# gregspangenberg/shoulder

Measured on AMD Instinct MI355X. Metric: humerus meshes/s end-to-end (all 4 landmarks), higher is better.
Workload: dtype f64 geometry + bf16 UNet

## Files before the change

shoulder_amd/csrc/k_groove.h:

```cpp
#pragma once
#include "k_stages.h"

namespace sh {

#define SH_GSLOTS (SH_GROOVE_NROWS * SH_MAXPEAK)

__global__ void k_groove_rows(const double* __restrict__ itr_cs , const double* __restrict__ prox_zs,
                              const double* __restrict__ canal_axis_ct, int row0,
                              double* __restrict__ xraw, double* __restrict__ ptheta, int* __restrict__ npk,
                              double* __restrict__ r0, int* __restrict__ err, int B) {
  __shared__ double s_bufA[SH_MPROX], s_bufB[SH_MPROX];
  double* const s_r = s_bufA; double* const s_filt = s_bufA;
  double* const s_neg = s_bufB; double* const s_roll = s_bufB;
  __shared__ int s_cand[SH_PEAK_CAP];
  __shared__ Peak s_pk[SH_PEAK_CAP];
  __shared__ int s_pass[SH_PEAK_CAP];
  __shared__ int s_ncand;
  const int M = SH_MPROX;
  const int gid = blockIdx.x, lane = threadIdx.x;
  const int b = gid / SH_GROOVE_NROWS, i = gid % SH_GROOVE_NROWS;
  const double* row = itr_cs + ((size_t)b * SH_NPROX + row0 + i) * 2 * M;
  const double* zs = prox_zs + (size_t)b * SH_NPROX + row0;
  for (int k = lane; k < M; k += 64) s_r[k] = row[M + k];
  if (lane == 0) s_ncand = 0;
  __syncthreads();
  double acc = 0.0;
  if (lane < 32) {
    const int leaf = lane >> 3, k = lane & 7;
    acc = s_r[128 * leaf + k];
    for (int q = 1; q < 16; ++q) acc += s_r[128 * leaf + 8 * q + k];
  }
  acc = acc + __shfl_down(acc, 1);
  acc = acc + __shfl_down(acc, 2);
  acc = acc + __shfl_down(acc, 4);
  acc = acc + __shfl_down(acc, 8);
  acc = acc + __shfl_down(acc, 16);
  const double mean = __shfl(acc, 0) / (double)M;
  for (int k = lane; k < M; k += 64) s_neg[k] = -1.0 * (s_r[k] - mean);
  __syncthreads();
  for (int k = 5 + lane; k < M - 5; k += 64) s_filt[k] = savgol10_1_at(s_neg, k);
  if (lane == 0) savgol10_1_edges(s_neg, M, s_filt);
  __syncthreads();
  double bv = 1e300;
  int bi = 0x7fffffff;
  for (int k = lane; k < M; k += 64) if (s_filt[k] < bv) { bv = s_filt[k]; bi = k; }
  for (int off = 32; off > 0; off >>= 1) {
    double ov = __shfl_down(bv, off);
    int oi = __shfl_down(bi, off);
    if (ov < bv || (ov == bv && oi < bi)) { bv = ov; bi = oi; }
  }
  const int amin = __shfl(bi, 0);
  double* r0row = r0 + (size_t)gid * M;
  for (int k = lane; k < M; k += 64) r0row[k] = -s_neg[k];
  __syncthreads();
  for (int k = lane; k < M; k += 64) { int src = k + amin; if (src >= M) src -= M; s_roll[k] = s_filt[src]; }
  __syncthreads();
  for (int k = 1 + lane; k < M - 1; k += 64)
    if (s_roll[k - 1] < s_roll[k]) {
      int resume;
      int pk = local_maximum_at(s_roll, M, k, &resume);
      if (pk >= 0) { int s = atomicAdd(&s_ncand, 1); if (s < SH_PEAK_CAP) s_cand[s] = pk; }
    }
  __syncthreads();
  int nc = s_ncand < SH_PEAK_CAP ? s_ncand : SH_PEAK_CAP;
  if (lane == 0)
    for (int a = 1; a < nc; ++a) { int v = s_cand[a]; int q = a - 1; while (q >= 0 && s_cand[q] > v) { s_cand[q + 1] = s_cand[q]; --q; } s_cand[q + 1] = v; }
  __syncthreads();
  static_assert(SH_MPROX == 512, "8 samples per lane");
  __shared__ int s_lb[SH_PEAK_CAP], s_rb[SH_PEAK_CAP];
  __shared__ double s_lmin[SH_PEAK_CAP], s_rmin[SH_PEAK_CAP];
  {
    double xr[8];
#pragma unroll
    for (int q = 0; q < 8; ++q) xr[q] = s_roll[8 * lane + q];
    for (int cnd = 0; cnd < nc; ++cnd) {
      const int pk = s_cand[cnd];
      const double v = s_roll[pk];
      int L = -1, R = M;
#pragma unroll
      for (int q = 0; q < 8; ++q) { const int k = 8 * lane + q; if (k < pk && xr[q] > v) L = k; }
#pragma unroll
      for (int q = 7; q >= 0; --q) { const int k = 8 * lane + q; if (k > pk && xr[q] > v) R = k; }
      for (int off = 32; off > 0; off >>= 1) { L = max(L, __shfl_xor(L, off)); R = min(R, __shfl_xor(R, off)); }
      double lm = v, rm = v;
#pragma unroll
      for (int q = 0; q < 8; ++q) {
        const int k = 8 * lane + q;
        if (k > L && k <= pk) lm = fmin(lm, xr[q]);
        if (k >= pk && k < R) rm = fmin(rm, xr[q]);
      }
      for (int off = 32; off > 0; off >>= 1) { lm = fmin(lm, __shfl_xor(lm, off)); rm = fmin(rm, __shfl_xor(rm, off)); }
      int lb = -1, rb = M;
#pragma unroll
      for (int q = 0; q < 8; ++q) { const int k = 8 * lane + q; if (k > L && k <= pk && xr[q] == lm) lb = k; }
#pragma unroll
      for (int q = 7; q >= 0; --q) { const int k = 8 * lane + q; if (k >= pk && k < R && xr[q] == rm) rb = k; }
      for (int off = 32; off > 0; off >>= 1) { lb = max(lb, __shfl_xor(lb, off)); rb = min(rb, __shfl_xor(rb, off)); }
      if (lane == 0) { s_lb[cnd] = lb; s_rb[cnd] = rb; s_lmin[cnd] = lm; s_rmin[cnd] = rm; }
    }
  }
  __syncthreads();
  if (lane < nc) {
    const double* x = s_roll;
    const int pk = s_cand[lane], lb = s_lb[lane], rb = s_rb[lane];
    const double left_min = s_lmin[lane], right_min = s_rmin[lane];
    bool ok = x[pk] >= -10.0;
    const double prom = x[pk] - (left_min > right_min ? left_min : right_min);
    ok = ok && prom >= 0.6;
    if (ok) {
      const double h = x[pk] - prom * 0.5;
      int k = pk;
      while (lb < k && h < x[k]) --k;
      double lip = (double)k;
      if (x[k] < h) lip += (h - x[k]) / (x[k + 1] - x[k]);
      k = pk;
      while (k < rb && h < x[k]) ++k;
      double rip = (double)k;
      if (x[k] < h) rip -= (h - x[k]) / (x[k - 1] - x[k]);
      const double w = rip - lip;
      ok = w >= 0.1;
      if (ok) { s_pk[lane].idx = pk; s_pk[lane].prominence = prom; s_pk[lane].width = w; s_pk[lane].width_height = h; }
    }
    s_pass[lane] = ok ? 1 : 0;
  }
  __syncthreads();
  __shared__ int s_np;
  __shared__ double s_th[SH_MAXPEAK], s_d[SH_MAXPEAK][SH_MAXPEAK];
  __shared__ int s_pidx[SH_MAXPEAK];
  if (lane == 0) {
    int np_ = 0;
    for (int a = 0; a < nc; ++a) if (s_pass[a]) s_pk[np_++] = s_pk[a];
    if (np_ > SH_MAXPEAK) {
      bool keep[SH_PEAK_CAP];
      for (int k = 0; k < np_; ++k) keep[k] = false;
      for (int q = 0; q < SH_MAXPEAK; ++q) {
        int bq = -1;
        for (int k = 0; k < np_; ++k)
          if (!keep[k] && (bq < 0 || s_pk[k].prominence > s_pk[bq].prominence)) bq = k;
        keep[bq] = true;
      }
      int w = 0;
      for (int k = 0; k < np_; ++k) if (keep[k]) s_pk[w++] = s_pk[k];
      np_ = SH_MAXPEAK;
    }
    s_np = np_;
  }
  __syncthreads();
  const int np_ = s_np;
  if (lane < np_) {
    const int idx = (s_pk[lane].idx + amin) % M;
    s_pidx[lane] = idx;
    s_th[lane] = row[idx];
  }
  double zmax = -1e300, zmin = 1e300;
  for (int k = lane; k < SH_GROOVE_NROWS; k += 64) { zmax = fmax(zmax, zs[k]); zmin = fmin(zmin, zs[k]); }
  for (int off = 32; off > 0; off >>= 1) { zmax = fmax(zmax, __shfl_xor(zmax, off)); zmin = fmin(zmin, __shfl_xor(zmin, off)); }
  __syncthreads();
  {
    const int k = lane >> 3, j = lane & 7;
    if (k < np_ && j < np_) s_d[k][j] = wrapped_abs_diff(s_th[k], s_th[j]);
  }
  __syncthreads();
  if (lane < np_) {
    const int k = lane;
    double near = 0.0, next = 0.0;
    if (np_ > 1) {
      double a[SH_MAXPEAK];
      int na = 0;
      for (int j = 0; j < np_; ++j) {
        double d = s_d[k][j];
        if (rint(d * 100.0) / 100.0 != 0.0) a[na++] = d;
      }
      for (int p = 1; p < na; ++p) { double v = a[p]; int q = p - 1; while (q >= 0 && a[q] > v) { a[q + 1] = a[q]; --q; } a[q + 1] = v; }
      near = na > 0 ? a[0] : nan("");
      if (np_ > 2) next = na > 1 ? a[1] : nan("");
    }
    double rng = zmax - zmin;
    if (rng == 0.0) rng = 1.0;
    const double sc = 1.0 / rng;
    const double z_scaled = zs[i] * sc + (0.0 - zmin * sc);
    const double* ax = canal_axis_ct + 6 * b;
    double cu[3] = {ax[0] - ax[3], ax[1] - ax[4], ax[2] - ax[5]};
    const double n = norm3(cu);
    cu[0] /= n; cu[1] /= n; cu[2] /= n;
    const double z = zs[i], th = s_th[k];
    const double rad = row[M + s_pidx[k]];
    const double px = rad * cos(th), py = rad * sin(th);
    const double dx = px - cu[0] * z, dy = py - cu[1] * z;
    double* X = xraw + ((size_t)b * SH_GSLOTS + (size_t)i * SH_MAXPEAK + k) * 9;
    X[0] = rad; X[1] = near; X[2] = next; X[3] = z_scaled; X[4] = s_pk[k].prominence; X[5] = s_pk[k].width;
    X[6] = s_pk[k].width_height; X[7] = sqrt(dx * dx + dy * dy); X[8] = (double)np_ / 7.0;
    ptheta[(size_t)b * SH_GSLOTS + (size_t)i * SH_MAXPEAK + k] = th;
    for (int q = 0; q < 9; ++q) if (X[q] != X[q]) atomicCAS(&err[b], 0, SH_ERR_GEOMETRY_DEV);
  }
  if (lane == 0) npk[gid] = np_;
  (void)B;
}

__global__ void __launch_bounds__(256)
k_groove_scale(const double* __restrict__ xraw, const int* __restrict__ npk, double* __restrict__ stats, int B,
               int* __restrict__ slots_out , int* __restrict__ nslot_out ,
               float* __restrict__ proba ) {
  __shared__ double col[5][SH_GSLOTS];
  __shared__ int slot[SH_GSLOTS];
  __shared__ int P_s;
  const int b = blockIdx.x, tid = threadIdx.x;
  const double* X = xraw + (size_t)b * SH_GSLOTS * 9;
  const int* np_ = npk + (size_t)b * SH_GROOVE_NROWS;
  __shared__ int s_cnt[SH_GROOVE_NROWS];
  for (int i = tid; i < SH_GROOVE_NROWS; i += 256) s_cnt[i] = np_[i];
  __syncthreads();
  for (int i = tid; i < SH_GROOVE_NROWS; i += 256) {
    int off = 0;
    for (int j = 0; j < i; ++j) off += s_cnt[j];
    const int n = s_cnt[i];
    for (int k = 0; k < n; ++k) slot[off + k] = i * SH_MAXPEAK + k;
    if (i == SH_GROOVE_NROWS - 1) P_s = off + n;
  }
  __syncthreads();
  const int P = P_s;
  for (int p = tid; p < P; p += 256) slots_out[(size_t)b * SH_GSLOTS + p] = slot[p];
  if (tid == 0) nslot_out[b] = P;
  for (int s = tid; s < SH_GSLOTS; s += 256)
    if (s % SH_MAXPEAK >= s_cnt[s / SH_MAXPEAK]) proba[(size_t)b * SH_GSLOTS + s] = -1.0f;
  for (int f0 = 0; f0 < 9; f0 += 5) {
    const int nf = f0 + 5 <= 9 ? 5 : 9 - f0;
    for (int q = tid; q < P * nf; q += 256) { const int p = q / nf, f = q - p * nf; col[f][p] = X[(size_t)slot[p] * 9 + f0 + f]; }
    __syncthreads();
    if (tid < nf) {
      const double* c = col[tid];
      double s = 0.0;
      int p = 0;
      for (; p + 8 <= P; p += 8) {
        double t8[8];
#pragma unroll
        for (int u = 0; u < 8; ++u) t8[u] = c[p + u];
#pragma unroll
        for (int u = 0; u < 8; ++u) s += t8[u];
      }
      for (; p < P; ++p) s += c[p];
      const double mean = P ? s / (double)P : 0.0;
      double v = 0.0;
      p = 0;
      for (; p + 8 <= P; p += 8) {
        double t8[8];
#pragma unroll
        for (int u = 0; u < 8; ++u) t8[u] = c[p + u];
#pragma unroll
        for (int u = 0; u < 8; ++u) { const double d = t8[u] - mean; v += d * d; }
      }
      for (; p < P; ++p) { double d = c[p] - mean; v += d * d; }
      const double var = P ? v / (double)P : 0.0;
      const double eps_ = 2.220446049250313e-16, nn = (double)P;
      const double ub = nn * eps_ * var + (nn * mean * eps_) * (nn * mean * eps_);
      double scale = var <= ub ? 1.0 : sqrt(var);
      stats[(size_t)b * 18 + f0 + tid] = mean;
      stats[(size_t)b * 18 + 9 + f0 + tid] = scale;
    }
    __syncthreads();
  }
}

__global__ void k_rfc_pack(const int* __restrict__ feat, const float* __restrict__ thr, const int* __restrict__ ti, const int* __restrict__ fi,
                           const float* __restrict__ lw, int4* __restrict__ nodes, int N) {
  const int i = blockIdx.x * blockDim.x + threadIdx.x;
  if (i >= N) return;
  const bool leaf = ti[i] < 0;
  nodes[i] = make_int4(feat[i], __float_as_int(leaf ? lw[i] : thr[i]), ti[i], fi[i]);
}

__global__ void __launch_bounds__(64)
k_groove_rfc(const double* __restrict__ xraw, const int* __restrict__ slots , const int* __restrict__ nslot , const double* __restrict__ stats,
             const int4* __restrict__ nodes, const int* __restrict__ roots, int n_trees,
             double* __restrict__ xs , float* __restrict__ proba, int B) {
  __shared__ double sx[9][64];
  const int tid = threadIdx.x;
  constexpr int WPB = (SH_GSLOTS + 63) / 64;
  const int b = blockIdx.x / WPB, p = (blockIdx.x - b * WPB) * 64 + tid;
  if (b >= B || p >= nslot[b]) return;
  const int gid = b * SH_GSLOTS + slots[(size_t)b * SH_GSLOTS + p];
  for (int f = 0; f < 9; ++f) {
    const double v = (xraw[(size_t)gid * 9 + f] - stats[(size_t)b * 18 + f]) / stats[(size_t)b * 18 + 9 + f];
    xs[(size_t)gid * 9 + f] = v;
    sx[f][tid] = v;
  }
  double acc = 0.0;
  for (int t = 0; t < n_trees; ++t) {
    int4 nd = nodes[roots[t]];
    while (nd.z >= 0) nd = nodes[(sx[nd.x][tid] <= (double)__int_as_float(nd.y)) ? nd.z : nd.w];
    acc += (double)__int_as_float(nd.y);
  }
  proba[gid] = (float)acc;
}

#define SH_KDE_TIE 1e-9
__device__ inline double groove_kde_wg(const double* __restrict__ ptheta, const float* __restrict__ proba, double* __restrict__ bg_theta,
                                       int* __restrict__ err, int b) {
  __shared__ double sel[SH_GSLOTS];
  __shared__ double dens[1024];
  __shared__ int nsel;
  __shared__ double wv[4];
  __shared__ int wi[4];
  __shared__ double s_bg;
  int tid = threadIdx.x;
  __shared__ int s_wc[4];
  if (tid == 0) nsel = 0;
  __syncthreads();
  for (int s0 = 0; s0 < SH_GSLOTS; s0 += 256) {
    const int s = s0 + tid;
    const bool keep = s < SH_GSLOTS && proba[(size_t)b * SH_GSLOTS + s] > 0.4f;
    const double val = keep ? ptheta[(size_t)b * SH_GSLOTS + s] : 0.0;
    const unsigned long long m = __ballot(keep);
    if ((tid & 63) == 0) s_wc[tid >> 6] = __popcll(m);
    __syncthreads();
    int pos = nsel + __popcll(m & ((1ull << (tid & 63)) - 1ull));
    for (int w = 0; w < (tid >> 6); ++w) pos += s_wc[w];
    if (keep) sel[pos] = val;
    __syncthreads();
    if (tid == 0) nsel += s_wc[0] + s_wc[1] + s_wc[2] + s_wc[3];
    __syncthreads();
  }
  const int n = nsel;
  if (n == 0) { if (tid == 0) { atomicCAS(&err[b], 0, SH_ERR_GEOMETRY_DEV); bg_theta[b] = 0.0; } return 0.0; }
  double best = -1.0;
  for (int j = tid; j < 1024; j += blockDim.x) {
    double t = linspace_at(-1.0 * M_PI, M_PI, 1024, j);
    double acc = 0.0;
    for (int i = 0; i < n; ++i) {
      double d = 1.0 - fabs(t - sel[i]);
      if (d > 0.0) acc += d;
    }
    dens[j] = acc;
    best = fmax(best, acc);
  }
  for (int off = 32; off > 0; off >>= 1) best = fmax(best, __shfl_down(best, off));
  if ((tid & 63) == 0) wv[tid >> 6] = best;
  __syncthreads();
  best = wv[0];
  for (int w = 1; w < (int)(blockDim.x >> 6); ++w) best = fmax(best, wv[w]);
  const double thr = best * (1.0 - SH_KDE_TIE);
  int bi = 0x7fffffff;
  for (int j = tid; j < 1024; j += blockDim.x)
    if (dens[j] >= thr) bi = min(bi, j);
  for (int off = 32; off > 0; off >>= 1) bi = min(bi, __shfl_down(bi, off));
  if ((tid & 63) == 0) wi[tid >> 6] = bi;
  __syncthreads();
  if (tid == 0) {
    for (int w = 1; w < (int)(blockDim.x >> 6); ++w) bi = min(bi, wi[w]);
    s_bg = linspace_at(-1.0 * M_PI, M_PI, 1024, bi);
    bg_theta[b] = s_bg;
  }
  __syncthreads();
  return s_bg;
}

__device__ inline void groove_localmin_row(const double* __restrict__ itr_cs, const double* __restrict__ r0, const double* __restrict__ prox_zs,
                                           const double* __restrict__ prox_centroids, double bg, int row0, double deg_window,
                                           int* __restrict__ local_idx, double* pts_obb, int b, int i) {
  const int gid = b * SH_GROOVE_NROWS + i;
  const double* row = itr_cs + ((size_t)b * SH_NPROX + row0 + i) * 2 * SH_MPROX;
  int ivar = (int)rint(deg_window / (360.0 / (double)SH_MPROX));
  if (ivar < 1) ivar = 1;
  int loc = groove_local_min(row, r0 + (size_t)gid * SH_MPROX, SH_MPROX, bg, ivar);
  local_idx[gid] = loc;
  int k = loc < 0 ? loc + SH_MPROX : loc;
  k = k < 0 ? 0 : (k >= SH_MPROX ? SH_MPROX - 1 : k);
  double t = row[k], r = row[SH_MPROX + k];
  const double* c = prox_centroids + 2 * ((size_t)b * SH_NPROX + row0 + i);
  double* p = pts_obb + (size_t)gid * 3;
  p[0] = r * cos(t) + c[0];
  p[1] = r * sin(t) + c[1];
  p[2] = prox_zs[(size_t)b * SH_NPROX + row0 + i] + 0.0;
}

__device__ inline void groove_axis_wave(const double* pts_obb, const double* __restrict__ T_obb, double* __restrict__ axis_ct,
                                        double* __restrict__ pts_ct, int b) {
  int lane = threadIdx.x & 63;
  const double* P = pts_obb + (size_t)b * SH_GROOVE_NROWS * 3;
  double mean[3], d[3];
  wave_line_fit(P, SH_GROOVE_NROWS, 3, mean, d);
  double zmin = 1e300, zmax = -1e300;
  for (int i = lane; i < SH_GROOVE_NROWS; i += 64) { zmin = fmin(zmin, P[3 * i + 2]); zmax = fmax(zmax, P[3 * i + 2]); }
  for (int off = 32; off > 0; off >>= 1) { zmin = fmin(zmin, __shfl_down(zmin, off)); zmax = fmax(zmax, __shfl_down(zmax, off)); }
  zmin = __shfl(zmin, 0); zmax = __shfl(zmax, 0);
  double Ti[16];
  inv_transform(T_obb + 16 * b, Ti);
  for (int i = lane; i < SH_GROOVE_NROWS; i += 64) xform_pt(Ti, P[3 * i], P[3 * i + 1], P[3 * i + 2], pts_ct + ((size_t)b * SH_GROOVE_NROWS + i) * 3);
  if (lane == 0) {
    if (d[2] < 0) { d[0] = -d[0]; d[1] = -d[1]; d[2] = -d[2]; }
    double h = (zmax - zmin) / 2.0;
    xform_pt(Ti, mean[0] + d[0] * h, mean[1] + d[1] * h, mean[2] + d[2] * h, axis_ct + 6 * b);
    xform_pt(Ti, mean[0] - d[0] * h, mean[1] - d[1] * h, mean[2] - d[2] * h, axis_ct + 6 * b + 3);
  }
}

__global__ void __launch_bounds__(256)
k_groove_tail(const double* __restrict__ ptheta, const float* __restrict__ proba, double* __restrict__ bg_theta, int* __restrict__ err,
              const double* __restrict__ itr_cs, const double* __restrict__ r0, const double* __restrict__ prox_zs, const double* __restrict__ prox_centroids,
              int row0, double deg_window, int* __restrict__ local_idx, double* pts_obb, const double* __restrict__ T_obb,
              double* __restrict__ axis_ct, double* __restrict__ pts_ct) {
  const int b = blockIdx.x, tid = threadIdx.x;
  const double bg = groove_kde_wg(ptheta, proba, bg_theta, err, b);
  for (int i = tid; i < SH_GROOVE_NROWS; i += 256) groove_localmin_row(itr_cs, r0, prox_zs, prox_centroids, bg, row0, deg_window, local_idx, pts_obb, b, i);
  __syncthreads();
  if (tid < 64) groove_axis_wave(pts_obb, T_obb, axis_ct, pts_ct, b);
}

}
```

shoulder_amd/csrc/k_ovf.h:

```cpp
#pragma once
#include "k_slices.h"

namespace sh {

struct OvfPools {
  Seg* segs; double* ring; unsigned char* work;
  unsigned long long seg_cap, ring_cap, work_cap;
  unsigned long long* ctr;
  int open_mode;
};
__host__ __device__ inline int ovf_nodes(int cnt, int open_mode) { return open_mode ? 2 * cnt : cnt; }

struct OvfSet { long long* soff; long long* roff; long long* woff; int* fill; int* list; int* nlist ; int* list2; };

__host__ __device__ inline unsigned ovf_hash_size(int n) { unsigned h = 64; while (h < 2u * (unsigned)n) h <<= 1; return h; }
__host__ __device__ inline unsigned long long ovf_work_bytes(int n) {
  unsigned long long b = (unsigned long long)n * 8ull * 5ull + (unsigned long long)ovf_hash_size(n) * 4ull + (unsigned long long)n * 4ull * 6ull + 64ull;
  const unsigned long long te = (unsigned long long)(n + 1) * 8ull * 7ull + 64ull;
  if (te > b) b = te;
  return (b + 15ull) & ~15ull;
}

__global__ void k_ovf_plan(int N, int nplanes, const int* __restrict__ seg_count, OvfPools P, OvfSet S, int* __restrict__ err) {
  const int pl = blockIdx.x * blockDim.x + threadIdx.x;
  if (pl >= nplanes) return;
  const int cnt = seg_count[pl];
  S.soff[pl] = -1; S.roff[pl] = -1; S.woff[pl] = -1; S.fill[pl] = 0;
  if (cnt <= SH_MAXSEG) return;
  const int nn = ovf_nodes(cnt, P.open_mode);
  const unsigned long long wb = ovf_work_bytes(nn);
  const unsigned long long s = atomicAdd(&P.ctr[0], (unsigned long long)cnt);
  const unsigned long long r = atomicAdd(&P.ctr[1], (unsigned long long)nn + 1ull);
  const unsigned long long w = atomicAdd(&P.ctr[2], wb);
  atomicMax(&P.ctr[3], s + cnt); atomicMax(&P.ctr[4], r + nn + 1ull); atomicMax(&P.ctr[5], w + wb);
  if (s + cnt > P.seg_cap || r + nn + 1ull > P.ring_cap || w + wb > P.work_cap) { atomicExch(&err[pl / N], SH_ERR_CAPACITY_DEV); return; }
  S.soff[pl] = (long long)s; S.roff[pl] = (long long)r; S.woff[pl] = (long long)w;
  S.list[atomicAdd(S.nlist, 1)] = pl;
}

__global__ void __launch_bounds__(256)
k_slice_emit_ovf(const double* __restrict__ vobb, const int* __restrict__ faces, const long long* __restrict__ voff, const long long* __restrict__ foff,
                 const double* __restrict__ zeff, int N, OvfPools P, OvfSet S) {
  if (*S.nlist == 0) return;
  const int b = blockIdx.y;
  const long long f0 = foff[b], nf = foff[b + 1] - f0;
  const double* vb = vobb + 3 * voff[b];
  const double* zp = zeff + (size_t)b * N;
  const double z_first = zp[0], z_last = zp[N - 1];
  const double inv_step = (double)(N - 1) / (z_last - z_first);
  for (long long fi = blockIdx.x * (long long)blockDim.x + threadIdx.x; fi < nf; fi += (long long)gridDim.x * blockDim.x) {
    const int* f = faces + 3 * (f0 + fi);
    const int id[3] = {f[0], f[1], f[2]};
    double Z[3];
    for (int k = 0; k < 3; ++k) Z[k] = vb[3 * (size_t)id[k] + 2];
    const double fzmin = fmin(Z[0], fmin(Z[1], Z[2])), fzmax = fmax(Z[0], fmax(Z[1], Z[2]));
    const double ka = (fzmin - z_first) * inv_step, kb = (fzmax - z_first) * inv_step;
    const double klo = fmin(ka, kb), khi = fmax(ka, kb);
    if (khi < -1.0 || klo > (double)N) continue;
    int lo = (int)floor(fmax(klo, 0.0)) - 1, hi = (int)ceil(fmin(khi, (double)(N - 1))) + 1;
    lo = lo < 0 ? 0 : lo;
    hi = hi > N - 1 ? N - 1 : hi;
    if (N == 1) { lo = 0; hi = 0; }
    for (int k = lo; k <= hi; ++k) {
      const long long so = S.soff[(size_t)b * N + k];
      if (so < 0) continue;
      const double z = zp[k];
      double d[3];
      int s[3];
      for (int j = 0; j < 3; ++j) { d[j] = Z[j] - z; s[j] = d[j] < -SH_SECTION_TOL ? -1 : 1; }
      if (s[0] == s[1] && s[1] == s[2]) continue;
      const int slot = atomicAdd(&S.fill[(size_t)b * N + k], 1);
      int up = 0, dn = 0;
      for (int j = 0; j < 3; ++j) {
        const int jn = (j + 1) % 3;
        if (s[j] == -1 && s[jn] == 1) up = j;
        if (s[j] == 1 && s[jn] == -1) dn = j;
      }
      Seg sg;
      {
        const int a = dn, c = (dn + 1) % 3;
        const int l = id[a] < id[c] ? a : c, h = id[a] < id[c] ? c : a;
        sg.s_lo = (uint32_t)id[l]; sg.s_hi = (uint32_t)id[h];
      }
      {
        const int a = up, c = (up + 1) % 3;
        const int l = id[a] < id[c] ? a : c, h = id[a] < id[c] ? c : a;
        sg.e_lo = (uint32_t)id[l]; sg.e_hi = (uint32_t)id[h];
      }
      P.segs[so + slot] = sg;
    }
  }
}

__global__ void __launch_bounds__(256)
k_ovf_plan_loops(int N, const int* __restrict__ seg_count, const Seg* __restrict__ segs , OvfPools P, OvfSet S, int* __restrict__ err) {
  __shared__ long long so, ro, wo;
  const int n2 = S.nlist[1];
  for (int i = blockIdx.x; i < n2; i += gridDim.x) {
    const int pl = S.list2[i];
    const int cnt = seg_count[pl];
    if (threadIdx.x == 0) {
      const int nn = ovf_nodes(cnt, P.open_mode);
      const unsigned long long wb = ovf_work_bytes(nn);
      const unsigned long long s = atomicAdd(&P.ctr[0], (unsigned long long)cnt);
      const unsigned long long r = atomicAdd(&P.ctr[1], (unsigned long long)nn + 1ull);
      const unsigned long long w = atomicAdd(&P.ctr[2], wb);
      atomicMax(&P.ctr[3], s + cnt); atomicMax(&P.ctr[4], r + nn + 1ull); atomicMax(&P.ctr[5], w + wb);
      if (s + cnt > P.seg_cap || r + nn + 1ull > P.ring_cap || w + wb > P.work_cap) { atomicExch(&err[pl / N], SH_ERR_CAPACITY_DEV); so = -1; }
      else { so = (long long)s; ro = (long long)r; wo = (long long)w; }
    }
    __syncthreads();
    if (so >= 0) {
      const Seg* src = segs + (size_t)pl * SH_MAXSEG;
      for (int j = threadIdx.x; j < cnt; j += 256) P.segs[so + j] = src[j];
      if (threadIdx.x == 0) { S.soff[pl] = so; S.roff[pl] = ro; S.woff[pl] = wo; S.fill[pl] = cnt; S.list[atomicAdd(&S.nlist[0], 1)] = pl; }
    }
    __syncthreads();
  }
}

#define SH_HUGE_THREADS 1024
#define SH_MAXLOOPS_G 1024

template <bool OPEN>
__device__ inline void slice_link_plane_g(const int pl, int N, const int* __restrict__ seg_count, const Seg* __restrict__ sp, const double* __restrict__ vb ,
             const double zpl , unsigned char* __restrict__ wk,
             double* __restrict__ centroids, double* __restrict__ areas, int* __restrict__ nloops, int* __restrict__ ring_n, double* __restrict__ ring_out ,
             int select, int* __restrict__ err, double* __restrict__ areas_total, const OpenCfg oc) {
  constexpr int T = SH_HUGE_THREADS;
  __shared__ unsigned long long l_key[SH_MAXLOOPS_G];
  __shared__ int l_start[SH_MAXLOOPS_G], l_len[SH_MAXLOOPS_G], l_off[SH_MAXLOOPS_G];
  __shared__ double l_area[SH_MAXLOOPS_G], l_sel[SH_MAXLOOPS_G];
  __shared__ int n_loops, bad, octl[4];
  __shared__ double bbw[T / 64][4];
  const int b = pl / N, tid = threadIdx.x;
  const int n = seg_count[pl];
  const int cap = ovf_nodes(n, OPEN ? oc.mode : 0);
  const unsigned HASH = ovf_hash_size(cap);
  unsigned long long* skey = (unsigned long long*)wk;
  unsigned long long* bufA = skey + cap;
  unsigned long long* bufB = bufA + cap;
  double* rx = (double*)(bufB + cap);
  double* ry = rx + cap;
  int* table = (int*)(ry + cap);
  int* nxt = table + HASH;
  int* jmpA = nxt + cap; int* jmpB = jmpA + cap; int* offA = jmpB + cap; int* offB = offA + cap; int* posv = offB + cap;
  if (tid == 0) { n_loops = 0; bad = 0; }
  for (unsigned i = tid; i < HASH; i += T) table[i] = -1;
  for (int i = tid; i < n; i += T) {
    const Seg s = sp[i];
    skey[i] = ((unsigned long long)s.s_lo << 32) | s.s_hi;
    bufA[i] = ((unsigned long long)s.e_lo << 32) | s.e_hi;
  }
  __syncthreads();
  for (int i = tid; i < n; i += T) {
    uint32_t h = hash_key64(skey[i]) & (HASH - 1);
    while (atomicCAS(&table[h], -1, i) != -1) h = (h + 1) & (HASH - 1);
  }
  __syncthreads();
  for (int i = tid; i < n; i += T) {
    const unsigned long long k = bufA[i];
    uint32_t h = hash_key64(k) & (HASH - 1);
    int t, found = -1;
    while ((t = table[h]) != -1) {
      if (skey[t] == k) { found = t; break; }
      h = (h + 1) & (HASH - 1);
    }
    if (found < 0) { found = i; bad = 1; }
    nxt[i] = found;
  }
  __syncthreads();
  const bool bridging = OPEN && (bad || n < 3);
  int n2 = n;
  if (bridging) {
    n2 = bridge_open_chains<T>(n, cap, n, skey, bufA, nxt, offB, octl, jmpA, jmpB, offA, posv, table, table + cap, rx, ry,
                               (double*)bufB, (double*)bufB + n, vb, zpl, oc.max_gap);
    if (tid == 0) bad = 0;
  }
  unsigned long long* labA = bufA;
  unsigned long long* labB = bufB;
  int* ja = jmpA; int* jb = jmpB;
  int* ra = offA; int* rb = offB;
  for (int i = tid; i < n2; i += T) { labA[i] = skey[i]; ja[i] = nxt[i]; ra[i] = 0; }
  __syncthreads();
  for (int span = 1; span < n2; span <<= 1) {
    for (int i = tid; i < n2; i += T) {
      const int j = ja[i];
      const unsigned long long a = labA[i], c = labA[j];
      const bool own = a <= c;
      labB[i] = own ? a : c;
      rb[i] = own ? ra[i] : span + ra[j];
      jb[i] = ja[j];
    }
    __syncthreads();
    unsigned long long* tl = labA; labA = labB; labB = tl;
    int* tj = ja; ja = jb; jb = tj;
    int* tr = ra; ra = rb; rb = tr;
  }
  for (int i = tid; i < n2; i += T)
    if (ra[i] == 0 && (!bridging || (nxt[ja[i]] != ja[i] && ra[nxt[i]] >= 2))) {
      const int l = atomicAdd(&n_loops, 1);
      if (l < SH_MAXLOOPS_G) l_start[l] = i;
    }
  __syncthreads();
  const int nl = n_loops > SH_MAXLOOPS_G ? SH_MAXLOOPS_G : n_loops;
  if (tid == 0) {
    if (n_loops > SH_MAXLOOPS_G) atomicExch(&err[b], SH_ERR_CAPACITY_DEV);
    for (int a = 1; a < nl; ++a) {
      const int v = l_start[a]; int c = a - 1;
      while (c >= 0 && skey[l_start[c]] > skey[v]) { l_start[c + 1] = l_start[c]; --c; }
      l_start[c + 1] = v;
    }
    int off = 0;
    for (int l = 0; l < nl; ++l) {
      const int s = l_start[l];
      const int L = ra[nxt[s]] + 1;
      l_len[l] = L; l_off[l] = off; off += L;
      l_key[l] = skey[s];
    }
    if (off != n && !bridging) bad = 1;
  }
  __syncthreads();
  if (bridging && oc.stats)
    for (int i = tid; i < n; i += T)
      if (nxt[i] == i || nxt[i] >= n) {
        bool kept = false;
        for (int q = 0; q < nl; ++q) kept |= l_key[q] == labA[i];
        atomicAdd(&oc.stats[2 * b + (kept ? 0 : 1)], 1);
      }
  for (int i = tid; i < n2; i += T) {
    const unsigned long long key = labA[i];
    int l = -1;
    for (int q = 0; q < nl; ++q) if (l_key[q] == key) { l = q; break; }
    const int L = l >= 0 ? l_len[l] : 1;
    const int r = ra[i];
    const int pos = r == 0 ? 0 : L - r;
    posv[i] = l < 0 ? -1 : l_off[l] + pos;
  }
  __syncthreads();
  for (int i = tid; i < n2; i += T)
    if (posv[i] >= 0 && posv[i] < n2) {
      if (!OPEN || i < n) { const Seg sg = sp[i]; seg_start_point(vb, sg.s_lo, sg.s_hi, zpl, &rx[posv[i]], &ry[posv[i]]); }
      else { const unsigned long long kv = skey[i]; seg_start_point(vb, (uint32_t)(kv >> 32), (uint32_t)kv, zpl, &rx[posv[i]], &ry[posv[i]]); }
    }
  __syncthreads();
  const int lane = tid & 63, wave = tid >> 6;
  {
    const int nv = bridging ? (nl > 0 ? l_off[nl - 1] + l_len[nl - 1] : 0) : n;
    double x0 = 1e300, x1 = -1e300, y0 = 1e300, y1 = -1e300;
    for (int i = tid; i < nv; i += T) {
      const double qx = rx[i], qy = ry[i];
      x0 = fmin(x0, qx); x1 = fmax(x1, qx); y0 = fmin(y0, qy); y1 = fmax(y1, qy);
    }
    for (int off = 32; off > 0; off >>= 1) {
      x0 = fmin(x0, __shfl_down(x0, off)); x1 = fmax(x1, __shfl_down(x1, off));
      y0 = fmin(y0, __shfl_down(y0, off)); y1 = fmax(y1, __shfl_down(y1, off));
    }
    if (lane == 0) { bbw[wave][0] = x0; bbw[wave][1] = x1; bbw[wave][2] = y0; bbw[wave][3] = y1; }
  }
  for (int l = wave; l < nl; l += T / 64) {
    const int o = l_off[l], L = l_len[l];
    double a2 = 0.0, mx = 0.0, my = 0.0;
    for (int q = lane; q < L; q += 64) {
      const int qn = q + 1 == L ? 0 : q + 1;
      a2 += rx[o + q] * ry[o + qn] - rx[o + qn] * ry[o + q];
      mx += rx[o + q]; my += ry[o + q];
    }
    for (int off = 32; off > 0; off >>= 1) { a2 += __shfl_down(a2, off); mx += __shfl_down(mx, off); my += __shfl_down(my, off); }
    if (lane == 0) {
      l_area[l] = 0.5 * a2;
      mx = (mx + rx[o]) / (double)(L + 1); my = (my + ry[o]) / (double)(L + 1);
      l_sel[l] = fabs(mx) + fabs(my);
    }
  }
  __syncthreads();
  int best = 0;
  for (int l = 1; l < nl; ++l) {
    if (select == 0) { if (fabs(l_area[l]) > fabs(l_area[best])) best = l; }
    else { if (l_sel[l] < l_sel[best]) best = l; }
  }
  if (tid == 0) {
    double x0 = bbw[0][0], x1 = bbw[0][1], y0 = bbw[0][2], y1 = bbw[0][3];
    for (int w = 1; w < T / 64; ++w) { x0 = fmin(x0, bbw[w][0]); x1 = fmax(x1, bbw[w][1]); y0 = fmin(y0, bbw[w][2]); y1 = fmax(y1, bbw[w][3]); }
    centroids[2 * (size_t)pl] = 0.5 * (x0 + x1);
    centroids[2 * (size_t)pl + 1] = 0.5 * (y0 + y1);
    int amax = 0;
    for (int l = 1; l < nl; ++l) if (fabs(l_area[l]) > fabs(l_area[amax])) amax = l;
    areas[pl] = nl > 0 ? fabs(l_area[amax]) : 0.0;
    if (areas_total) {
      double tot = 0.0;
      for (int l = 0; l < nl; ++l) tot += l_area[l];
      areas_total[pl] = fabs(tot);
    }
    nloops[pl] = nl;
    ring_n[pl] = nl > 0 ? l_len[best] : 0;
    if (bad || (nl == 0 && !(bridging && areas_total))) atomicCAS(&err[b], 0, SH_ERR_GEOMETRY_DEV);
  }
  if (ring_out && nl > 0) {
    const int l = best, o = l_off[l], L = l_len[l];
    const bool rev = l_area[l] < 0;
    for (int q = tid; q <= L; q += T) {
      const int qq = q == L ? 0 : q;
      const int src = rev ? (qq == 0 ? 0 : L - qq) : qq;
      ring_out[2 * q] = rx[o + src];
      ring_out[2 * q + 1] = ry[o + src];
    }
  }
  __syncthreads();
}

template <bool OPEN>
__global__ void __launch_bounds__(SH_HUGE_THREADS)
k_slice_link_huge(int N, const int* __restrict__ seg_count, OvfPools P, OvfSet S, double* __restrict__ centroids, double* __restrict__ areas,
                  int* __restrict__ nloops, int* __restrict__ ring_n, int want_ring, int select, int* __restrict__ err, double* __restrict__ areas_total,
                  const double* __restrict__ vobb, const long long* __restrict__ voff, const double* __restrict__ zeff, const OpenCfg oc) {
  const int nl = *S.nlist;
  for (int i = blockIdx.x; i < nl; i += gridDim.x) {
    const int pl = S.list[i];
    slice_link_plane_g<OPEN>(pl, N, seg_count, P.segs + S.soff[pl], vobb + 3 * voff[pl / N], zeff[pl], P.work + S.woff[pl], centroids, areas, nloops, ring_n,
                       want_ring ? P.ring + 2 * S.roff[pl] : (double*)nullptr, select, err, areas_total, oc);
  }
}

__global__ void __launch_bounds__(SH_RS_THREADS)
k_resample_polar_huge(int N, int M, const int* __restrict__ ring_n, OvfPools P, OvfSet S, const double* __restrict__ centroids,
                      double* __restrict__ ixy, double* __restrict__ itr_start, double* __restrict__ itr_cs, const RsWant W) {
  constexpr int NS = SH_MPROX / SH_RS_THREADS;
  __shared__ int amin_idx;
  __shared__ double wmin[SH_RS_THREADS / 64];
  __shared__ int widx[SH_RS_THREADS / 64];
  const int nlist = *S.nlist, tid = threadIdx.x;
  for (int it = blockIdx.x; it < nlist; it += gridDim.x) {
    const int pl = S.list[it];
    const int kpl = pl % N;
    const bool want_st = W.keep_all || kpl >= W.st_lo, want_cs = W.keep_all || (kpl >= W.cs_lo && kpl < W.cs_hi);
    if (!want_st && !want_cs) continue;
    const int L = ring_n[pl];
    const double* rp = P.ring + 2 * S.roff[pl];
    double* d = (double*)(P.work + S.woff[pl]);
    for (int q = 1 + tid; q <= L; q += SH_RS_THREADS) {
      const double dx = rp[2 * q] - rp[2 * (q - 1)], dy = rp[2 * q + 1] - rp[2 * (q - 1) + 1];
      d[q] = sqrt(dx * dx + dy * dy);
    }
    __syncthreads();
    if (tid == 0) {
      double acc = 0.0;
      d[0] = 0.0;
      for (int q = 1; q <= L; ++q) { acc += d[q]; d[q] = acc; }
    }
    __syncthreads();
    const double dmax = d[L];
    double sx[NS], sy[NS];
#pragma unroll
    for (int u = 0; u < NS; ++u) {
      const int j = tid + u * SH_RS_THREADS;
      const double t = linspace_at(0.0, dmax, M, j);
      const int n = L + 1;
      if (t < d[0]) { sx[u] = rp[0]; sy[u] = rp[1]; }
      else if (!(t < d[n - 1])) { sx[u] = rp[2 * (n - 1)]; sy[u] = rp[2 * (n - 1) + 1]; }
      else {
        int lo = 0, hi = n - 1;
        while (hi - lo > 1) { const int mid = (lo + hi) >> 1; if (t >= d[mid]) lo = mid; else hi = mid; }
        const double x0 = d[lo], fx = rp[2 * lo], fy = rp[2 * lo + 1];
        if (x0 == t) { sx[u] = fx; sy[u] = fy; }
        else {
          const double den = d[lo + 1] - x0;
          sx[u] = (rp[2 * (lo + 1)] - fx) / den * (t - x0) + fx;
          sy[u] = (rp[2 * (lo + 1) + 1] - fy) / den * (t - x0) + fy;
        }
      }
    }
    if (W.keep_all) {
      double* oxy = ixy + (size_t)pl * 2 * M;
#pragma unroll
      for (int u = 0; u < NS; ++u) { const int j = tid + u * SH_RS_THREADS; oxy[j] = sx[u]; oxy[M + j] = sy[u]; }
    }
    const double cx = centroids[2 * (size_t)pl], cy = centroids[2 * (size_t)pl + 1];
    for (int pass = 0; pass < 2; ++pass) {
      if (pass == 0 ? !want_st : !want_cs) continue;
      const double ox = pass ? cx : 0.0, oy = pass ? cy : 0.0;
      double best = 1e300;
      int bi = 0x7fffffff;
      double th[NS], rr[NS];
#pragma unroll
      for (int u = 0; u < NS; ++u) {
        const int j = tid + u * SH_RS_THREADS;
        const double x = sx[u] - ox, y = sy[u] - oy;
        th[u] = atan2(y, x);
        rr[u] = sqrt(x * x + y * y);
        if (th[u] < best || (th[u] == best && j < bi)) { best = th[u]; bi = j; }
      }
      for (int off = 32; off > 0; off >>= 1) {
        const double ob = __shfl_down(best, off);
        const int oi = __shfl_down(bi, off);
        if (ob < best || (ob == best && oi < bi)) { best = ob; bi = oi; }
      }
      if ((tid & 63) == 0) { wmin[tid >> 6] = best; widx[tid >> 6] = bi; }
      __syncthreads();
      if (tid == 0) {
        double bv = wmin[0]; int bx = widx[0];
        for (int w = 1; w < SH_RS_THREADS / 64; ++w)
          if (wmin[w] < bv || (wmin[w] == bv && widx[w] < bx)) { bv = wmin[w]; bx = widx[w]; }
        amin_idx = bx;
      }
      __syncthreads();
      const int k0 = amin_idx;
      double* o = (pass ? itr_cs : itr_start) + (size_t)pl * 2 * M;
#pragma unroll
      for (int u = 0; u < NS; ++u) {
        int dst = tid + u * SH_RS_THREADS - k0; if (dst < 0) dst += M;
        o[dst] = th[u];
        o[M + dst] = rr[u];
      }
      __syncthreads();
    }
  }
}

}
```

shoulder_amd/csrc/k_slices.h:

```cpp
#pragma once
#include "sh_scalar.h"

namespace sh {

struct __attribute__((aligned(16))) Seg {
  uint32_t s_lo, s_hi, e_lo, e_hi;
};
static_assert(sizeof(Seg) == 16, "Seg must be 16 bytes");
__device__ inline void seg_start_point(const double* __restrict__ vb , uint32_t lo, uint32_t hi, double z, double* x, double* y) {
  const double* pl = vb + 3 * (size_t)lo;
  const double* ph = vb + 3 * (size_t)hi;
  const double dl = pl[2] - z, dh = ph[2] - z;
  const double t = dl / (dl - dh);
  *x = pl[0] + t * (ph[0] - pl[0]);
  *y = pl[1] + t * (ph[1] - pl[1]);
}

__device__ inline unsigned long long enc_f64(double v) {
  unsigned long long b = (unsigned long long)__double_as_longlong(v);
  return (b & 0x8000000000000000ull) ? ~b : (b | 0x8000000000000000ull);
}
__device__ inline double dec_f64(unsigned long long e) {
  unsigned long long b = (e & 0x8000000000000000ull) ? (e & 0x7FFFFFFFFFFFFFFFull) : ~e;
  return __longlong_as_double((long long)b);
}

__global__ void k_transform_verts(const float* __restrict__ verts, const long long* __restrict__ voff,
                                  const double* __restrict__ T, double* __restrict__ vobb,
                                  unsigned long long* __restrict__ zb_enc ) {
  int b = blockIdx.y;
  long long v0 = voff[b], nv = voff[b + 1] - v0;
  const double* Tb = T + 16 * b;
  double zmin = 1e300, zmax = -1e300;
  for (long long i = blockIdx.x * (long long)blockDim.x + threadIdx.x; i < nv; i += (long long)gridDim.x * blockDim.x) {
    const float* p = verts + 3 * (v0 + i);
    double o[3];
    xform_pt(Tb, (double)p[0], (double)p[1], (double)p[2], o);
    double* q = vobb + 3 * (v0 + i);
    q[0] = o[0]; q[1] = o[1]; q[2] = o[2];
    zmin = fmin(zmin, o[2]); zmax = fmax(zmax, o[2]);
  }
  for (int off = 32; off > 0; off >>= 1) {
    zmin = fmin(zmin, __shfl_down(zmin, off));
    zmax = fmax(zmax, __shfl_down(zmax, off));
  }
  if ((threadIdx.x & 63) == 0) {
    atomicMin(&zb_enc[2 * b], enc_f64(zmin));
    atomicMin(&zb_enc[2 * b + 1], ~enc_f64(zmax));
  }
}

__global__ void k_decode_bounds(const unsigned long long* zb_enc, double* zb, int B) {
  int i = blockIdx.x * blockDim.x + threadIdx.x;
  if (i < 2 * B) zb[i] = dec_f64((i & 1) ? ~zb_enc[i] : zb_enc[i]);
}

__device__ inline double np_pairwise_sum(const double* a, int n) {
  if (n < 8) {
    double r = 0.0;
    for (int i = 0; i < n; ++i) r += a[i];
    return r;
  } else if (n <= 128) {
    double r[8];
    for (int k = 0; k < 8; ++k) r[k] = a[k];
    int i;
    for (i = 8; i < n - (n % 8); i += 8)
      for (int k = 0; k < 8; ++k) r[k] += a[i + k];
    double res = ((r[0] + r[1]) + (r[2] + r[3])) + ((r[4] + r[5]) + (r[6] + r[7]));
    for (; i < n; ++i) res += a[i];
    return res;
  } else {
    int n2 = n / 2;
    n2 -= n2 % 8;
    return np_pairwise_sum(a, n2) + np_pairwise_sum(a + n2, n - n2);
  }
}

struct PlaneAux {
  const unsigned long long* zb_enc; double* zb_out;
  int* seg_count; int* nlarge;
  int* ovf_nlist; unsigned long long* ovf_ctr;
};
struct ManyLoops { int* list; int* n; unsigned long long* missed; };
struct SliceSetDev {
  int N, kind, select;
  const double* zb;
  double* zs; double* zeff;
  int* seg_count; Seg* segs;
  double* centroids; double* areas; int* nloops; int* ring_n; double* ring ; double* areas_total ;
  int* nlarge; ManyLoops many; unsigned long long* ovf_missed;
  PlaneAux aux;
};
struct OpenCfg { int mode; double max_gap; int* stats; };

struct SliceSets { SliceSetDev s[2]; int n; const double* vobb; const long long* voff; OpenCfg open; };

__global__ void k_make_planes(SliceSets sets, const double* __restrict__ neck_z, int B) {
  const SliceSetDev& S = sets.s[blockIdx.y];
  const int kind = S.kind, N = S.N;
  const double* zb = S.zb;
  double* zs = S.zs; double* zeff = S.zeff;
  const PlaneAux A = S.aux;
  int b = blockIdx.x;
  if (b >= B) return;
  for (int k = threadIdx.x; k < N; k += blockDim.x) A.seg_count[(size_t)b * N + k] = 0;
  if (b == 0 && threadIdx.x == 0) {
    *A.nlarge = 0;
    if (A.ovf_nlist) { A.ovf_nlist[0] = 0; A.ovf_nlist[1] = 0 ; if (A.ovf_ctr) { A.ovf_ctr[0] = 0ull; A.ovf_ctr[2] = 0ull; } }
  }
  if (kind == 3) {
    if (threadIdx.x == 0) { zs[b] = neck_z[b]; zeff[b] = neck_z[b]; }
    return;
  }
  double zmin, zmax;
  if (A.zb_enc) {
    zmin = dec_f64(A.zb_enc[2 * b]); zmax = dec_f64(~A.zb_enc[2 * b + 1]);
    if (threadIdx.x == 0) { A.zb_out[2 * b] = zmin; A.zb_out[2 * b + 1] = zmax; }
  } else { zmin = zb[2 * b]; zmax = zb[2 * b + 1]; }
  double a, e;
  if (kind == 4) {
    for (int k = threadIdx.x; k < N; k += blockDim.x) { double z = linspace_at(zmin * 0.99, zmax * 0.99, N, k); zs[(size_t)b * N + k] = z; zeff[(size_t)b * N + k] = z; }
    return;
  }
  if (kind == 0) { a = 0.99 * zmax; e = 0.99 * zmin; }
  else if (kind == 1) { a = 0.99 * zmax; e = neck_z[b]; }
  else { a = 0.99 * zmin; e = 0.0; }
  double* z = zs + (size_t)b * N;
  for (int k = threadIdx.x; k < N; k += blockDim.x) z[k] = linspace_at(a, e, N, k);
  __syncthreads();
  __shared__ double z_orig;
  if (threadIdx.x == 0) z_orig = np_pairwise_sum(z, N) / (double)N;
  __syncthreads();
  for (int k = threadIdx.x; k < N; k += blockDim.x) zeff[(size_t)b * N + k] = z_orig + (z[k] - z_orig);
}

#define SH_EMIT_MAXN 640
__global__ void __launch_bounds__(256)
k_slice_emit(const double* __restrict__ vobb, const int* __restrict__ faces,
             const long long* __restrict__ voff, const long long* __restrict__ foff, SliceSets sets) {
  __shared__ int hist[SH_EMIT_MAXN];
  int b = blockIdx.y;
  long long f0 = foff[b], nf = foff[b + 1] - f0;
  const double* vb = vobb + 3 * voff[b];
  const int nsets = sets.n, Ntot = sets.s[0].N + (nsets > 1 ? sets.s[1].N : 0);
  for (long long f_base = blockIdx.x * (long long)blockDim.x; f_base < nf; f_base += (long long)gridDim.x * blockDim.x) {
    for (int k = threadIdx.x; k < Ntot; k += blockDim.x) hist[k] = 0;
    const long long fi = f_base + threadIdx.x;
    const bool live = fi < nf;
    const int* f = faces + 3 * (f0 + (live ? fi : 0));
    int id[3] = {f[0], f[1], f[2]};
    double Z[3];
    for (int k = 0; k < 3; ++k) Z[k] = vb[3 * (size_t)id[k] + 2];
    double fzmin = fmin(Z[0], fmin(Z[1], Z[2])), fzmax = fmax(Z[0], fmax(Z[1], Z[2]));
    int lo_[2] = {1, 1}, hi_[2] = {0, 0};
    for (int si = 0; si < nsets; ++si) {
      const int N = sets.s[si].N;
      const double* zp = sets.s[si].zeff + (size_t)b * N;
      const double z_first = zp[0], z_last = zp[N - 1];
      const double inv_step = (double)(N - 1) / (z_last - z_first);
      double ka = (fzmin - z_first) * inv_step, kb = (fzmax - z_first) * inv_step;
      double klo = fmin(ka, kb), khi = fmax(ka, kb);
      int lo = 1, hi = 0;
      if (live && !(khi < -1.0 || klo > (double)N)) {
        lo = (int)floor(fmax(klo, 0.0)) - 1; hi = (int)ceil(fmin(khi, (double)(N - 1))) + 1;
        lo = lo < 0 ? 0 : lo;
        hi = hi > N - 1 ? N - 1 : hi;
      }
      if (live && N == 1) { lo = 0; hi = 0; }
      lo_[si] = lo; hi_[si] = hi;
    }
    __syncthreads();
    for (int si = 0; si < nsets; ++si) {
      const int N = sets.s[si].N, hoff = si ? sets.s[0].N : 0;
      const double* zp = sets.s[si].zeff + (size_t)b * N;
      for (int k = lo_[si]; k <= hi_[si]; ++k) {
        const double z = zp[k];
        const int s0 = Z[0] - z < -SH_SECTION_TOL ? -1 : 1, s1 = Z[1] - z < -SH_SECTION_TOL ? -1 : 1, s2 = Z[2] - z < -SH_SECTION_TOL ? -1 : 1;
        if (!(s0 == s1 && s1 == s2)) atomicAdd(&hist[hoff + k], 1);
      }
    }
    __syncthreads();
    for (int k = threadIdx.x; k < Ntot; k += blockDim.x) {
      const int n = hist[k];
      if (n > 0) {
        const int si = k >= sets.s[0].N ? 1 : 0, kk = si ? k - sets.s[0].N : k;
        hist[k] = atomicAdd(&sets.s[si].seg_count[(size_t)b * sets.s[si].N + kk], n);
      }
    }
    __syncthreads();
    for (int si = 0; si < nsets; ++si) {
      const int N = sets.s[si].N, hoff = si ? sets.s[0].N : 0;
      const double* zp = sets.s[si].zeff + (size_t)b * N;
      Seg* segs = sets.s[si].segs;
      for (int k = lo_[si]; k <= hi_[si]; ++k) {
        const double z = zp[k];
        double d[3];
        int s[3];
        for (int j = 0; j < 3; ++j) { d[j] = Z[j] - z; s[j] = d[j] < -SH_SECTION_TOL ? -1 : 1; }
        if (s[0] == s[1] && s[1] == s[2]) continue;
        const int slot = atomicAdd(&hist[hoff + k], 1);
        int up = 0, dn = 0;
        for (int j = 0; j < 3; ++j) {
          int jn = (j + 1) % 3;
          if (s[j] == -1 && s[jn] == 1) up = j;
          if (s[j] == 1 && s[jn] == -1) dn = j;
        }
        Seg sg;
        {
          int a = dn, c = (dn + 1) % 3;
          int l = id[a] < id[c] ? a : c, h = id[a] < id[c] ? c : a;
          sg.s_lo = (uint32_t)id[l]; sg.s_hi = (uint32_t)id[h];
        }
        {
          int a = up, c = (up + 1) % 3;
          int l = id[a] < id[c] ? a : c, h = id[a] < id[c] ? c : a;
          sg.e_lo = (uint32_t)id[l]; sg.e_hi = (uint32_t)id[h];
        }
        if (slot < SH_MAXSEG) segs[((size_t)b * N + k) * SH_MAXSEG + slot] = sg;
      }
    }
    __syncthreads();
  }
}

#define SH_LINK_THREADS 256
#define SH_MAXLOOPS 32
#define SH_SMALLSEG 384

__device__ inline uint32_t hash_key64(unsigned long long k) {
  k ^= k >> 33; k *= 0xff51afd7ed558ccdull; k ^= k >> 33;
  return (uint32_t)k;
}

template <int T>
__device__ inline int bridge_open_chains(const int n, const int cap, const int maxe, unsigned long long* __restrict__ skey,
                                         const unsigned long long* __restrict__ ekey, int* __restrict__ nxt, int* __restrict__ pred,
                                         int* __restrict__ ctl, int* tl, int* hd, int* bt, int* bh, int* mt, int* mh,
                                         double* tx, double* ty, double* hx, double* hy,
                                         const double* __restrict__ vb, const double z, const double max_gap) {
  const int tid = threadIdx.x;
  for (int i = tid; i < n; i += T) pred[i] = 0;
  if (tid < 4) ctl[tid] = 0;
  __syncthreads();
  for (int i = tid; i < n; i += T) if (nxt[i] != i) atomicAdd(&pred[nxt[i]], 1);
  __syncthreads();
  for (int i = tid; i < n; i += T) {
    if (nxt[i] == i) { const int q = atomicAdd(&ctl[0], 1); if (q < maxe) tl[q] = i; }
    if (pred[i] == 0) { const int q = atomicAdd(&ctl[1], 1); if (q < maxe) hd[q] = i; }
  }
  __syncthreads();
  const int nt = ctl[0], nh = ctl[1];
  if (nt > maxe || nh > maxe) return -1;
  for (int q = tid; q < nt; q += T) { const unsigned long long k = ekey[tl[q]]; seg_start_point(vb, (uint32_t)(k >> 32), (uint32_t)k, z, &tx[q], &ty[q]); mt[q] = -1; }
  for (int q = tid; q < nh; q += T) { const unsigned long long k = skey[hd[q]]; seg_start_point(vb, (uint32_t)(k >> 32), (uint32_t)k, z, &hx[q], &hy[q]); mh[q] = -1; }
  for (;;) {
    __syncthreads();
    if (tid == 0) ctl[2] = 0;
    for (int q = tid; q < nt; q += T) {
      int best = -1; double bd = 0.0; unsigned long long bk = 0;
      if (mt[q] < 0)
        for (int h = 0; h < nh; ++h) {
          if (mh[h] >= 0) continue;
          const double dx = tx[q] - hx[h], dy = ty[q] - hy[h];
          const double d = sqrt(dx * dx + dy * dy);
          if (!(d <= max_gap)) continue;
          const unsigned long long k = skey[hd[h]];
          if (best < 0 || d < bd || (d == bd && k < bk)) { best = h; bd = d; bk = k; }
        }
      bt[q] = best;
    }
    for (int q = tid; q < nh; q += T) {
      int best = -1; double bd = 0.0; unsigned long long bk = 0;
      if (mh[q] < 0)
        for (int t = 0; t < nt; ++t) {
          if (mt[t] >= 0) continue;
          const double dx = tx[t] - hx[q], dy = ty[t] - hy[q];
          const double d = sqrt(dx * dx + dy * dy);
          if (!(d <= max_gap)) continue;
          const unsigned long long k = ekey[tl[t]];
          if (best < 0 || d < bd || (d == bd && k < bk)) { best = t; bd = d; bk = k; }
        }
      bh[q] = best;
    }
    __syncthreads();
    for (int q = tid; q < nt; q += T) {
      const int h = bt[q];
      if (h >= 0 && bh[h] == q) { mt[q] = h; mh[h] = q; ctl[2] = 1; }
    }
    __syncthreads();
    if (ctl[2] == 0) break;
  }
  for (int q = tid; q < nt; q += T)
    if (mt[q] >= 0) {
      const int v = n + atomicAdd(&ctl[3], 1);
      if (v < cap) { skey[v] = ekey[tl[q]]; nxt[v] = hd[mt[q]]; nxt[tl[q]] = v; }
    }
  __syncthreads();
  const int nb = ctl[3];
  return n + nb > cap ? -1 : n + nb;
}


template <int CAP, bool OPEN>
__device__ inline void slice_link_plane(const int pl, int N, const int* __restrict__ seg_count, const Seg* __restrict__ segs,
             const double* __restrict__ vobb, const long long* __restrict__ voff, const double* __restrict__ zeff,
             double* __restrict__ centroids, double* __restrict__ areas, int* __restrict__ nloops,
             int* __restrict__ ring_n, double* __restrict__ ring , int select, int* __restrict__ err,
             double* __restrict__ areas_total , ManyLoops many, const OpenCfg oc,
             int* __restrict__ nlarge = nullptr) {
  constexpr int HASH = CAP <= 384 ? 512 : 2048;
  static_assert(HASH * 4 <= CAP * 8 && HASH > CAP, "the hash table lives in bufB");
  __shared__ unsigned long long skey[CAP];
  __shared__ unsigned long long bufA[CAP];
  __shared__ unsigned long long bufB[CAP];
  __shared__ int nxt[CAP], jmpA[CAP], jmpB[CAP], offA[CAP], offB[CAP];
  int* const table = (int*)bufB;
  __shared__ unsigned long long l_key[SH_MAXLOOPS];
  __shared__ int l_start[SH_MAXLOOPS], l_len[SH_MAXLOOPS], l_off[SH_MAXLOOPS];
  __shared__ double l_area[SH_MAXLOOPS], l_sel[SH_MAXLOOPS];
  __shared__ int n_loops, bad;
  __shared__ double bbv[4];

  const int b = pl / N;
  const int tid = threadIdx.x;
  int cnt = seg_count[pl];
  if (CAP == SH_SMALLSEG ? cnt > SH_SMALLSEG : cnt <= SH_SMALLSEG) {
    if (CAP == SH_SMALLSEG && nlarge && tid == 0) atomicAdd(nlarge, 1);
    return;
  }
  if (cnt > SH_MAXSEG) return;
  const int n = cnt;
  if (tid == 0) { n_loops = 0; bad = 0; }
  for (int i = tid; i < HASH; i += SH_LINK_THREADS) table[i] = -1;
  const Seg* sp = segs + (size_t)pl * SH_MAXSEG;
  const double* vb = vobb + 3 * voff[b];
  const double zpl = zeff[pl];
  for (int i = tid; i < n; i += SH_LINK_THREADS) {
    Seg s = sp[i];
    skey[i] = ((unsigned long long)s.s_lo << 32) | s.s_hi;
    bufA[i] = ((unsigned long long)s.e_lo << 32) | s.e_hi;
  }
  __syncthreads();
  if (n < 3 && !(OPEN && n > 0)) {
    if (tid == 0) {
      centroids[2 * (size_t)pl] = 0; centroids[2 * (size_t)pl + 1] = 0; areas[pl] = 0; nloops[pl] = 0; ring_n[pl] = 0;
      if (areas_total) areas_total[pl] = 0;
      else atomicCAS(&err[b], 0, SH_ERR_GEOMETRY_DEV);
    }
    return;
  }
  for (int i = tid; i < n; i += SH_LINK_THREADS) {
    uint32_t h = hash_key64(skey[i]) & (HASH - 1);
    while (atomicCAS(&table[h], -1, i) != -1) h = (h + 1) & (HASH - 1);
  }
  __syncthreads();
  for (int i = tid; i < n; i += SH_LINK_THREADS) {
    unsigned long long k = bufA[i];
    uint32_t h = hash_key64(k) & (HASH - 1);
    int t, found = -1;
    while ((t = table[h]) != -1) {
      if (skey[t] == k) { found = t; break; }
      h = (h + 1) & (HASH - 1);
    }
    if (found < 0) { found = i; bad = 1; }
    nxt[i] = found;
  }
  __syncthreads();
  const bool bridging = OPEN && (bad || n < 3);
  int n2 = n;
  if (bridging) {
    constexpr int E = SH_MAXLOOPS;
    double* pts = (double*)bufB;
    n2 = bridge_open_chains<SH_LINK_THREADS>(n, CAP, E, skey, bufA, nxt, offB, jmpB, jmpA, jmpA + E, jmpA + 2 * E, jmpA + 3 * E, jmpA + 4 * E,
                                             jmpA + 5 * E, pts, pts + E, pts + 2 * E, pts + 3 * E, vb, zpl, oc.max_gap);
    if (n2 < 0) {
      if (tid == 0) {
        if (many.list) many.list[atomicAdd(many.n, 1)] = pl;
        else if (many.missed) atomicExch(many.missed, 1ull);
        else atomicExch(&err[b], SH_ERR_CAPACITY_DEV);
      }
      return;
    }
    if (tid == 0) bad = 0;
  }
  unsigned long long* labA = bufA;
  unsigned long long* labB = bufB;
  int* ja = jmpA; int* jb = jmpB;
  int* ra = offA; int* rb = offB;
  for (int i = tid; i < n2; i += SH_LINK_THREADS) { labA[i] = skey[i]; ja[i] = nxt[i]; ra[i] = 0; }
  __syncthreads();
  for (int span = 1; span < n2; span <<= 1) {
    for (int i = tid; i < n2; i += SH_LINK_THREADS) {
      const int j = ja[i];
      const unsigned long long a = labA[i], c = labA[j];
      const bool own = a <= c;
      labB[i] = own ? a : c;
      rb[i] = own ? ra[i] : span + ra[j];
      jb[i] = ja[j];
    }
    __syncthreads();
    unsigned long long* tl = labA; labA = labB; labB = tl;
    int* tj = ja; ja = jb; jb = tj;
    int* tr = ra; ra = rb; rb = tr;
  }
  for (int i = tid; i < n2; i += SH_LINK_THREADS)
    if (ra[i] == 0 && (!bridging || (nxt[ja[i]] != ja[i] && ra[nxt[i]] >= 2))) {
      int l = atomicAdd(&n_loops, 1);
      if (l < SH_MAXLOOPS) l_start[l] = i;
    }
  __syncthreads();
  if (n_loops > SH_MAXLOOPS) {
    if (tid == 0) {
      if (many.list) many.list[atomicAdd(many.n, 1)] = pl;
      else if (many.missed) atomicExch(many.missed, 1ull);
      else atomicExch(&err[b], SH_ERR_CAPACITY_DEV);
    }
    return;
  }
  const int nl = n_loops;
  if (tid == 0) {
    for (int a = 1; a < nl; ++a) {
      int v = l_start[a]; int c = a - 1;
      while (c >= 0 && skey[l_start[c]] > skey[v]) { l_start[c + 1] = l_start[c]; --c; }
      l_start[c + 1] = v;
    }
    int off = 0;
    for (int l = 0; l < nl; ++l) {
      int s = l_start[l];
      int L = ra[nxt[s]] + 1;
      l_len[l] = L; l_off[l] = off; off += L;
      l_key[l] = skey[s];
    }
    if (off != n && !bridging) bad = 1;
  }
  __syncthreads();
  if (bridging) {
    if (oc.stats)
      for (int i = tid; i < n; i += SH_LINK_THREADS)
        if (nxt[i] == i || nxt[i] >= n) {
          bool kept = false;
          for (int q = 0; q < nl; ++q) kept |= l_key[q] == labA[i];
          atomicAdd(&oc.stats[2 * b + (kept ? 0 : 1)], 1);
        }
    if (nl == 0) {
      if (tid == 0) {
        centroids[2 * (size_t)pl] = 0; centroids[2 * (size_t)pl + 1] = 0; areas[pl] = 0; nloops[pl] = 0; ring_n[pl] = 0;
        if (areas_total) areas_total[pl] = 0;
        else atomicCAS(&err[b], 0, SH_ERR_GEOMETRY_DEV);
      }
      return;
    }
    __syncthreads();
  }
  double* rx = (double*)bufA;
  double* ry = (double*)bufB;
  int my_pos[(CAP + SH_LINK_THREADS - 1) / SH_LINK_THREADS];
  {
    int c = 0;
    for (int i = tid; i < n2; i += SH_LINK_THREADS, ++c) {
      const unsigned long long key = labA[i];
      int l = -1;
      for (int q = 0; q < nl; ++q) if (l_key[q] == key) { l = q; break; }
      const int L = l >= 0 ? l_len[l] : 1;
      const int r = ra[i];
      const int pos = r == 0 ? 0 : L - r;
      my_pos[c] = l < 0 ? -1 : l_off[l] + pos;
    }
  }
  __syncthreads();
  {
    int c = 0;
    for (int i = tid; i < n2; i += SH_LINK_THREADS, ++c)
      if (my_pos[c] >= 0 && my_pos[c] < n2) {
        if (!OPEN || i < n) { const Seg sg = sp[i]; seg_start_point(vb, sg.s_lo, sg.s_hi, zpl, &rx[my_pos[c]], &ry[my_pos[c]]); }
        else { const unsigned long long kv = skey[i]; seg_start_point(vb, (uint32_t)(kv >> 32), (uint32_t)kv, zpl, &rx[my_pos[c]], &ry[my_pos[c]]); }
      }
  }
  __syncthreads();
  const int lane = tid & 63, wave = tid >> 6;
  const int nv = bridging ? l_off[nl - 1] + l_len[nl - 1] : n;
  if (wave == SH_LINK_THREADS / 64 - 1) {
    double x0 = 1e300, x1 = -1e300, y0 = 1e300, y1 = -1e300;
    for (int i = lane; i < nv; i += 64) {
      const double qx = rx[i], qy = ry[i];
      x0 = fmin(x0, qx); x1 = fmax(x1, qx); y0 = fmin(y0, qy); y1 = fmax(y1, qy);
    }
    for (int off = 32; off > 0; off >>= 1) {
      x0 = fmin(x0, __shfl_down(x0, off)); x1 = fmax(x1, __shfl_down(x1, off));
      y0 = fmin(y0, __shfl_down(y0, off)); y1 = fmax(y1, __shfl_down(y1, off));
    }
    if (lane == 0) { bbv[0] = x0; bbv[1] = x1; bbv[2] = y0; bbv[3] = y1; }
  } else {
    for (int l = wave; l < nl; l += SH_LINK_THREADS / 64 - 1) {
      const int o = l_off[l], L = l_len[l];
      double a2 = 0.0, mx = 0.0, my = 0.0;
      for (int q = lane; q < L; q += 64) {
        const int qn = q + 1 == L ? 0 : q + 1;
        a2 += rx[o + q] * ry[o + qn] - rx[o + qn] * ry[o + q];
        mx += rx[o + q]; my += ry[o + q];
      }
      for (int off = 32; off > 0; off >>= 1) { a2 += __shfl_down(a2, off); mx += __shfl_down(mx, off); my += __shfl_down(my, off); }
      if (lane == 0) {
        l_area[l] = 0.5 * a2;
        mx = (mx + rx[o]) / (double)(L + 1); my = (my + ry[o]) / (double)(L + 1);
        l_sel[l] = fabs(mx) + fabs(my);
      }
    }
  }
  __syncthreads();
  int best = 0;
  for (int l = 1; l < nl; ++l) {
    if (select == 0) { if (fabs(l_area[l]) > fabs(l_area[best])) best = l; }
    else { if (l_sel[l] < l_sel[best]) best = l; }
  }
  if (tid == 0) {
    double x0 = bbv[0], x1 = bbv[1], y0 = bbv[2], y1 = bbv[3];
    centroids[2 * (size_t)pl] = 0.5 * (x0 + x1);
    centroids[2 * (size_t)pl + 1] = 0.5 * (y0 + y1);
    int amax = 0;
    for (int l = 1; l < nl; ++l) if (fabs(l_area[l]) > fabs(l_area[amax])) amax = l;
    areas[pl] = fabs(l_area[amax]);
    if (areas_total) {
      double tot = 0.0;
      for (int l = 0; l < nl; ++l) tot += l_area[l];
      areas_total[pl] = fabs(tot);
    }
    nloops[pl] = nl;
    ring_n[pl] = l_len[best];
    if (bad) atomicCAS(&err[b], 0, SH_ERR_GEOMETRY_DEV);
  }
  if (ring) {
    int l = best, o = l_off[l], L = l_len[l];
    bool rev = l_area[l] < 0;
    double* out = ring + (size_t)pl * (SH_MAXSEG + 1) * 2;
    for (int q = tid; q <= L; q += SH_LINK_THREADS) {
      int qq = q == L ? 0 : q;
      int src = rev ? (qq == 0 ? 0 : L - qq) : qq;
      out[2 * q] = rx[o + src];
      out[2 * q + 1] = ry[o + src];
    }
  }
}

template <bool OPEN>
__global__ void __launch_bounds__(SH_LINK_THREADS)
k_slice_link(SliceSets sets, int B, int* __restrict__ err) {
  const int ntot = sets.s[0].N + (sets.n > 1 ? sets.s[1].N : 0);
  int id = (int)blockIdx.x;
  if (B % 8 == 0) { const int x = id & 7, j = id >> 3; id = (x + 8 * (j / ntot)) * ntot + j % ntot; }
  const int b = id / ntot, kk = id - b * ntot;
  const int si = kk >= sets.s[0].N ? 1 : 0;
  const SliceSetDev& S = sets.s[si];
  slice_link_plane<SH_SMALLSEG, OPEN>(b * S.N + (kk - (si ? sets.s[0].N : 0)), S.N, S.seg_count, S.segs, sets.vobb, sets.voff, S.zeff, S.centroids, S.areas, S.nloops, S.ring_n,
                                S.ring, S.select, err, S.areas_total, S.many, sets.open, S.nlarge);
}
template <bool OPEN>
__global__ void __launch_bounds__(SH_LINK_THREADS)
k_slice_link_large(SliceSets sets, int B, int* __restrict__ err) {
  for (int si = 0; si < sets.n; ++si) {
    const SliceSetDev& S = sets.s[si];
    if (*S.nlarge == 0) continue;
    const int nplanes = B * S.N;
    for (int pl = blockIdx.x; pl < nplanes; pl += gridDim.x) {
      const int cnt = S.seg_count[pl];
      if (cnt > SH_MAXSEG && S.ovf_missed && threadIdx.x == 0) atomicExch(S.ovf_missed, 1ull);
      if (cnt <= SH_SMALLSEG || cnt > SH_MAXSEG) continue;
      slice_link_plane<SH_MAXSEG, OPEN>(pl, S.N, S.seg_count, S.segs, sets.vobb, sets.voff, S.zeff, S.centroids, S.areas, S.nloops, S.ring_n, S.ring, S.select, err, S.areas_total, S.many, sets.open);
      __syncthreads();
    }
  }
}

#define SH_RS_THREADS 128
struct RsWant { int keep_all, st_lo, cs_lo, cs_hi; };
template <int CAP>
__device__ inline void resample_polar_plane(const int pl, int N, int M, const int* __restrict__ ring_n, const double* __restrict__ ring,
                 const double* __restrict__ centroids, double* __restrict__ ixy,
                 double* __restrict__ itr_start, double* __restrict__ itr_cs, const long long* __restrict__ ovf_roff, const RsWant W) {
  static_assert(SH_MPROX % SH_RS_THREADS == 0, "whole samples per lane");
  constexpr int NS = SH_MPROX / SH_RS_THREADS;
  __shared__ double rx[CAP + 1], ry[CAP + 1], d[CAP + 1];
  __shared__ int amin_idx;
  __shared__ double wmin[SH_RS_THREADS / 64];
  __shared__ int widx[SH_RS_THREADS / 64];
  const int tid = threadIdx.x;
  const int L = ring_n[pl];
  if (CAP == SH_SMALLSEG ? L > SH_SMALLSEG : L <= SH_SMALLSEG) return;
  if (ovf_roff[pl] >= 0) return;
  const int kpl = pl % N;
  const bool want_st = W.keep_all || kpl >= W.st_lo, want_cs = W.keep_all || (kpl >= W.cs_lo && kpl < W.cs_hi);
  if (!want_st && !want_cs) return;
  const double* rp = ring + (size_t)pl * (SH_MAXSEG + 1) * 2;
  for (int q = tid; q <= L; q += SH_RS_THREADS) { rx[q] = rp[2 * q]; ry[q] = rp[2 * q + 1]; }
  __syncthreads();
  for (int q = 1 + tid; q <= L; q += SH_RS_THREADS) {
    double dx = rx[q] - rx[q - 1], dy = ry[q] - ry[q - 1];
    d[q] = sqrt(dx * dx + dy * dy);
  }
  __syncthreads();
  if (tid == 0) {
    double acc = 0.0;
    d[0] = 0.0;
    int q = 1;
    for (; q + 8 <= L + 1; q += 8) {
      double v[8];
#pragma unroll
      for (int u = 0; u < 8; ++u) v[u] = d[q + u];
#pragma unroll
      for (int u = 0; u < 8; ++u) { acc += v[u]; v[u] = acc; }
#pragma unroll
      for (int u = 0; u < 8; ++u) d[q + u] = v[u];
    }
    for (; q <= L; ++q) { acc += d[q]; d[q] = acc; }
  }
  __syncthreads();
  const double dmax = d[L];
  double sx[NS], sy[NS];
#pragma unroll
  for (int u = 0; u < NS; ++u) {
    const int j = tid + u * SH_RS_THREADS;
    const double t = linspace_at(0.0, dmax, M, j);
    const int n = L + 1;
    if (t < d[0]) { sx[u] = rx[0]; sy[u] = ry[0]; }
    else if (!(t < d[n - 1])) { sx[u] = rx[n - 1]; sy[u] = ry[n - 1]; }
    else {
      int lo = 0, hi = n - 1;
      while (hi - lo > 1) { const int mid = (lo + hi) >> 1; if (t >= d[mid]) lo = mid; else hi = mid; }
      const double x0 = d[lo], fx = rx[lo], fy = ry[lo];
      if (x0 == t) { sx[u] = fx; sy[u] = fy; }
      else {
        const double den = d[lo + 1] - x0;
        sx[u] = (rx[lo + 1] - fx) / den * (t - x0) + fx;
        sy[u] = (ry[lo + 1] - fy) / den * (t - x0) + fy;
      }
    }
  }
  if (W.keep_all) {
    double* oxy = ixy + (size_t)pl * 2 * M;
#pragma unroll
    for (int u = 0; u < NS; ++u) { const int j = tid + u * SH_RS_THREADS; oxy[j] = sx[u]; oxy[M + j] = sy[u]; }
  }
  const double cx = centroids[2 * (size_t)pl], cy = centroids[2 * (size_t)pl + 1];
  for (int pass = 0; pass < 2; ++pass) {
    if (pass == 0 ? !want_st : !want_cs) continue;
    const double ox = pass ? cx : 0.0, oy = pass ? cy : 0.0;
    double best = 1e300;
    int bi = 0x7fffffff;
    double th[NS], rr[NS];
#pragma unroll
    for (int u = 0; u < NS; ++u) {
      const int j = tid + u * SH_RS_THREADS;
      const double x = sx[u] - ox, y = sy[u] - oy;
      th[u] = atan2(y, x);
      rr[u] = sqrt(x * x + y * y);
      if (th[u] < best || (th[u] == best && j < bi)) { best = th[u]; bi = j; }
    }
    for (int off = 32; off > 0; off >>= 1) {
      double ob = __shfl_down(best, off);
      int oi = __shfl_down(bi, off);
      if (ob < best || (ob == best && oi < bi)) { best = ob; bi = oi; }
    }
    if ((tid & 63) == 0) { wmin[tid >> 6] = best; widx[tid >> 6] = bi; }
    __syncthreads();
    if (tid == 0) {
      double bv = wmin[0]; int bx = widx[0];
      for (int w = 1; w < SH_RS_THREADS / 64; ++w)
        if (wmin[w] < bv || (wmin[w] == bv && widx[w] < bx)) { bv = wmin[w]; bx = widx[w]; }
      amin_idx = bx;
    }
    __syncthreads();
    const int k0 = amin_idx;
    double* o = (pass ? itr_cs : itr_start) + (size_t)pl * 2 * M;
#pragma unroll
    for (int u = 0; u < NS; ++u) {
      int dst = tid + u * SH_RS_THREADS - k0; if (dst < 0) dst += M;
      o[dst] = th[u];
      o[M + dst] = rr[u];
    }
    __syncthreads();
  }
}

__global__ void __launch_bounds__(SH_RS_THREADS)
k_resample_polar(int N, int M, const int* __restrict__ ring_n, const double* __restrict__ ring, const double* __restrict__ centroids,
                 double* __restrict__ ixy, double* __restrict__ itr_start, double* __restrict__ itr_cs, const long long* __restrict__ ovf_roff, const RsWant W) {
  resample_polar_plane<SH_SMALLSEG>(blockIdx.x, N, M, ring_n, ring, centroids, ixy, itr_start, itr_cs, ovf_roff, W);
}
__global__ void __launch_bounds__(SH_RS_THREADS)
k_resample_polar_large(int nplanes, int N, int M, const int* __restrict__ ring_n, const double* __restrict__ ring, const double* __restrict__ centroids,
                       double* __restrict__ ixy, double* __restrict__ itr_start, double* __restrict__ itr_cs, const int* __restrict__ nlarge,
                       const long long* __restrict__ ovf_roff, const RsWant W) {
  if (*nlarge == 0) return;
  for (int pl = blockIdx.x; pl < nplanes; pl += gridDim.x) {
    if (ring_n[pl] <= SH_SMALLSEG || ovf_roff[pl] >= 0) continue;
    resample_polar_plane<SH_MAXSEG>(pl, N, M, ring_n, ring, centroids, ixy, itr_start, itr_cs, ovf_roff, W);
    __syncthreads();
  }
}

}
```

shoulder_amd/csrc/shoulder_hip.hip:

```cpp
#include "../../include/shoulder_hip.h"

#include <hip/hip_runtime.h>

#include <algorithm>
#include <cstdio>
#include <cstring>
#include <map>
#include <tuple>
#include <mutex>
#include <string>
#include <vector>

#include "k_slices.h"
#include "k_ovf.h"
#include "k_open.h"
#include "k_stages.h"
#include "k_groove.h"
#include "k_anp.h"
#include "k_unet.h"
#include "k_unet_bf16.h"
#include "k_unet16_ldr.h"
#include "k_unet_x3.h"
#include "k_unet16_up.h"
#include "unet16_pp.h"
// ... 1150 lines not shown
    h /= 2; w /= 2;
    std::string na = i < D ? "enc" + std::to_string(i) + "a" : "bota", nb = i < D ? "enc" + std::to_string(i) + "b" : "botb";
    if ((rc = conv_layer(c, ("unet." + na).c_str(), L(na), A, nullptr, ch, 0, Bq, h, w, nimg, 1)) != SH_OK) return rc;
    ch *= 2;
    float* dst = i < D ? skip[i] : A;
    if ((rc = conv_layer(c, ("unet." + nb).c_str(), L(nb), Bq, nullptr, ch, 0, dst, h, w, nimg, 1, (x3 && i < D) ? UF_POOL : 0, A)) != SH_OK) return rc;
  }
  float* x = A; float* y = Bq;
  for (int i = D - 1; i >= 0; --i) {
    std::string nu = "up" + std::to_string(i), na = "dec" + std::to_string(i) + "a", nb = "dec" + std::to_string(i) + "b";
    if ((rc = conv_layer(c, ("unet." + nu).c_str(), L(nu), x, nullptr, ch, 0, y, h, w, nimg, 0)) != SH_OK) return rc;
    h *= 2; w *= 2; ch /= 2;
    if ((rc = conv_layer(c, ("unet." + na).c_str(), L(na), skip[i], y, ch, ch, x, h, w, nimg, 1)) != SH_OK) return rc;
    if ((rc = conv_layer(c, ("unet." + nb).c_str(), L(nb), x, nullptr, ch, 0, y, h, w, nimg, 1)) != SH_OK) return rc;
    std::swap(x, y);
  }
  {
    const sh_ctx::ULayer& l = L("head");
    size_t npx = (size_t)nimg * H * W;
    if (l.cin <= 32) { LAUNCH(c, "unet.head", k_head<32>, dim3((unsigned)std::min<size_t>((npx + 255) / 256, 16384)), dim3(256), x, P + l.w_off, P + l.b_off, logits, l.cin, npx); }
    else { LAUNCH(c, "unet.head", k_head<64>, dim3((unsigned)std::min<size_t>((npx + 255) / 256, 8192)), dim3(256), x, P + l.w_off, P + l.b_off, logits, l.cin, npx); }
  }
  return SH_OK;
}

}

#define SH_UNET_TICKETS 64
#define SH_UNET_TKTAB (1 << 18)
static int persistent_grid(sh_ctx* c) {
  constexpr int cu_reserve = 32;
  if (c->num_cus <= 0) { int v = 0; if (hipDeviceGetAttribute(&v, hipDeviceAttributeMultiprocessorCount, c->device) != hipSuccess) v = 0; c->num_cus = v > 0 ? v : 256; }
  return c->unet_turn ? std::max(8, c->num_cus - cu_reserve) : c->num_cus;
}

static int unet_tickets(sh_ctx* c, int total, int nwg, int ngrp, unsigned** tk, const int** tk_tab, int* ntk) {
  const auto key = std::make_tuple(total, nwg, ngrp);
  auto it = c->tk_tabs.find(key);
  if (it == c->tk_tabs.end()) {
    std::vector<int> tab;
    int pos = 0;
    while (pos < total) {
      int sz = std::max(1, (int)std::ceil((total - pos) / (3.0 * (double)nwg)));
      if (sz >= ngrp) sz = sz / ngrp * ngrp;
      tab.push_back(pos);
      pos += std::min(sz, total - pos);
    }
    tab.push_back(total);
    if ((int)tab.size() > SH_UNET_TKTAB) return fail(c, SH_ERR_CAPACITY, "unet: ticket table larger than its buffer");
    if (c->tk_tab_used + (int)tab.size() > SH_UNET_TKTAB) {
      HIPCHK(c, hipStreamSynchronize(c->stream));
      c->tk_tabs.clear();
      c->tk_tab_used = 0;
    }
    HIPCHK(c, hipMemcpyAsync(buf<int>(c, "unet16.tk_tab") + c->tk_tab_used, tab.data(), tab.size() * 4, hipMemcpyHostToDevice, c->stream));
    HIPCHK(c, hipStreamSynchronize(c->stream));
    it = c->tk_tabs.emplace(key, std::make_pair(c->tk_tab_used, (int)tab.size() - 1)).first;
    c->tk_tab_used += (int)tab.size();
  }
  if (c->ticket_next >= SH_UNET_TICKETS) return fail(c, SH_ERR_CAPACITY, "unet: out of work counters");
  *tk = buf<unsigned>(c, "unet16.tickets") + c->ticket_next++;
  *tk_tab = buf<int>(c, "unet16.tk_tab") + it->second.first;
  *ntk = it->second.second;
  return SH_OK;
}

template <int EK>
static int conv_layer16(sh_ctx* c, const char* lname, const sh_ctx::ULayer& L, const u16* src0, const u16* src1, int C0, int C1,
                           u16* dst, int H, int W, int nimg, int relu, int fuse = 0, ConvFuse fz = ConvFuse{}) {
  if (H % UN_TH || W % UN_TW) return fail(c, SH_ERR_ARG, "unet: feature map is not a multiple of 16");
  const u16* w = buf<u16>(c, "params_bf16") + L.w_off;
  const float* b = buf<float>(c, "params") + L.b_off;
  const int tiles = (H / UN_TH) * (W / UN_TW);
  const dim3 blk(UN_THREADS);
  const bool ldr = !c->unet_reference && L.taps == 9 && L.cout % 64 == 0 && L.cout <= 512 && W % 32 == 0 && H % 16 == 0 && C0 % 32 == 0 && C1 % 32 == 0 &&
                   (fuse == 0 || (fuse == UF_POOL && relu));
  if (ldr) {
    int rc0;
    if ((rc0 = ensure(c, "unet16.zero", 256, 2)) != SH_OK) return rc0;
    if (!c->zero_page_ready) { HIPCHK(c, hipMemsetAsync(buf<char>(c, "unet16.zero"), 0, 256, c->stream)); c->zero_page_ready = true; }
    const int total = nimg * (W / 32) * (H / 16) * (L.cout / 64);
    const dim3 g((unsigned)std::min(total, persistent_grid(c)));
    unsigned* tk = nullptr; const int* tk_tab = nullptr; int ntk = 0;
    if ((rc0 = unet_tickets(c, total, (int)g.x, L.cout / 64, &tk, &tk_tab, &ntk)) != SH_OK) return rc0;
    const u16* zp = (const u16*)c->bufs["unet16.zero"].p;
    u16* pl = fuse == UF_POOL ? (u16*)fz.pooled : (u16*)nullptr;
    const bool wres = L.cout == 64 && ((C0 + C1) / 32) * 64 <= 128;
    if (fuse == UF_POOL && wres) { LAUNCH(c, lname, (k_conv3_ldr16<EK, UF_POOL, 1>), g, dim3(UD_THREADS), src0, src1, C0, C1, w, b, dst, H, W, L.cout, relu, nimg, zp, pl, tk, tk_tab, ntk); }
    else if (fuse == UF_POOL) { LAUNCH(c, lname, (k_conv3_ldr16<EK, UF_POOL, 0>), g, dim3(UD_THREADS), src0, src1, C0, C1, w, b, dst, H, W, L.cout, relu, nimg, zp, pl, tk, tk_tab, ntk); }
    else if (wres) { LAUNCH(c, lname, (k_conv3_ldr16<EK, 0, 1>), g, dim3(UD_THREADS), src0, src1, C0, C1, w, b, dst, H, W, L.cout, relu, nimg, zp, pl, tk, tk_tab, ntk); }
    else { LAUNCH(c, lname, (k_conv3_ldr16<EK, 0, 0>), g, dim3(UD_THREADS), src0, src1, C0, C1, w, b, dst, H, W, L.cout, relu, nimg, zp, pl, tk, tk_tab, ntk); }
  } else if (L.taps == 9 && L.cout % 64 == 0) {
    const dim3 g(tiles, L.cout / 64, nimg);
    if (fuse == 0) { LAUNCH(c, lname, (k_conv_mfma16<EK, 9, 4, 0>), g, blk, src0, src1, C0, C1, w, b, dst, H, W, L.cout, relu, fz); }
    else if (fuse == UF_POOL) { LAUNCH(c, lname, (k_conv_mfma16<EK, 9, 4, UF_POOL>), g, blk, src0, src1, C0, C1, w, b, dst, H, W, L.cout, relu, fz); }
    else return fail(c, SH_ERR_ARG, "unet: unsupported fusion");
  } else if (L.taps == 9) {
    const dim3 g(tiles, L.cout / 32, nimg);
    if (fuse == 0) { LAUNCH(c, lname, (k_conv_mfma16<EK, 9, 2, 0>), g, blk, src0, src1, C0, C1, w, b, dst, H, W, L.cout, relu, fz); }
    else return fail(c, SH_ERR_ARG, "unet: unsupported fusion");
  } else if (!c->unet_reference && L.cout % 32 == 0 && C1 == 0 && C0 % 32 == 0) {
    const bool upg = W % 32 == 0 && H % 16 == 0 && (C0 == 128 || C0 == 256 || C0 == 512) && L.cout <= 512;
    if (upg) {
      const int mt = C0 == 128 ? 4 : 2, nitems = (W / 32) * (H / (4 * mt)) * nimg;
      const int grid = C0 == 512 ? nitems : std::min(nitems, persistent_grid(c));
      unsigned* tk = nullptr; const int* tk_tab = nullptr; int ntk = 0;
      if (C0 != 512) { const int trc = unet_tickets(c, nitems, grid, 1, &tk, &tk_tab, &ntk); if (trc != SH_OK) return trc; }
      if (C0 == 128) { LAUNCH(c, lname, (k_upconv16g<EK, 4, 4, 4, true>), dim3((unsigned)grid), dim3(UPR_THREADS), src0, w, b, dst, H, W, L.cout, nimg, tk, tk_tab, ntk); }
      else if (C0 == 256) { LAUNCH(c, lname, (k_upconv16g<EK, 8, 2, 4, true>), dim3((unsigned)grid), dim3(UPR_THREADS), src0, w, b, dst, H, W, L.cout, nimg, tk, tk_tab, ntk); }
      else { LAUNCH(c, lname, (k_upconv16g<EK, 16, 2, 2, false>), dim3((unsigned)grid), dim3(UPR_THREADS), src0, w, b, dst, H, W, L.cout, nimg, tk, tk_tab, ntk); }
    }
    else { LAUNCH(c, lname, (k_upconv16<EK>), dim3(tiles, L.cout / 32, nimg * 2), dim3(UPC_THREADS), src0, C0, w, b, dst, H, W, L.cout); }
  } else if (L.cout % 64 == 0) {
    LAUNCH(c, lname, (k_conv_mfma16<EK, 1, 4, 0>), dim3(tiles, L.cout / 64, nimg * 4), blk, src0, src1, C0, C1, w, b, dst, H, W, L.cout, 0, fz);
  } else {
    LAUNCH(c, lname, (k_conv_mfma16<EK, 1, 2, 0>), dim3(tiles, L.cout / 32, nimg * 4), blk, src0, src1, C0, C1, w, b, dst, H, W, L.cout, 0, fz);
  }
  return SH_OK;
}

static bool unet16_level0_fused(const sh_ctx* c, int H, int W) {
  return !c->unet_reference && c->unet_base == 32 && c->unet_depth >= 1 && W % 32 == 0 && H % 16 == 0 && (H >> c->unet_depth) % 16 == 0 && (W >> c->unet_depth) % 16 == 0;
}
static bool unet16_starts_fused(const sh_ctx* c, int H, int W) { return unet16_level0_fused(c, H, W); }

template <int EK>
static int unet_forward16(sh_ctx* c, const float* image, float* logits, int nimg, int H, int W) {
  const int D = c->unet_depth, base = c->unet_base;
  if ((H >> D) % 16 || (W >> D) % 16) return fail(c, SH_ERR_ARG, "unet: input size must be a multiple of 16 << depth");
  int rc;
  if ((rc = ensure(c, "params_bf16", c->unet_floats * 2, 2)) != SH_OK) return rc;
  const float* P = buf<float>(c, "params");
  u16* PW = buf<u16>(c, "params_bf16");
  if (c->packed_kind != EK) {
    std::vector<PackEntry> tab;
    long long total = 0;
    for (auto& kv : c->ulayers) {
      const sh_ctx::ULayer& l = kv.second;
      if (l.cin < 32 || l.cout < 32) continue;
      tab.push_back(PackEntry{total, (long long)l.w_off, l.taps, l.cin, l.cout, 0});
      total += (long long)l.taps * l.cin * l.cout;
    }
    if ((rc = ensure(c, "unet16.packtab", tab.size() * sizeof(PackEntry), 8)) != SH_OK) return rc;
    if (!c->packtab_ready) {
      HIPCHK(c, hipMemcpyAsync(c->bufs["unet16.packtab"].p, tab.data(), tab.size() * sizeof(PackEntry), hipMemcpyHostToDevice, c->stream));
      HIPCHK(c, hipStreamSynchronize(c->stream));
      c->packtab_ready = true;
    }
    LAUNCH(c, "k_pack_w_bf16", k_pack_w16_all<EK>, dim3(2048), dim3(256), P, PW, (const PackEntry*)c->bufs["unet16.packtab"].p, (int)tab.size(), total);
    c->packed_kind = EK;
  }
  if ((rc = ensure(c, "unet16.tickets", SH_UNET_TICKETS * 4, 4)) != SH_OK) return rc;
  if ((rc = ensure(c, "unet16.tk_tab", SH_UNET_TKTAB * 4, 4)) != SH_OK) return rc;
  FILL(c, {buf<unsigned>(c, "unet16.tickets"), (size_t)SH_UNET_TICKETS * 4, 0});
  c->ticket_next = 0;
  const bool fused = unet16_level0_fused(c, H, W);
  const size_t full = (size_t)nimg * H * W * base * 2;
  if ((rc = ensure(c, "unet16.a", full, 2)) != SH_OK) return rc;
  if ((rc = ensure(c, "unet16.b", full, 2)) != SH_OK) return rc;
  std::vector<u16*> skip(D);
  for (int i = 0; i < D; ++i) {
    std::string nm = "unet16.skip" + std::to_string(i);
    if ((rc = ensure(c, nm.c_str(), full >> i, 2)) != SH_OK) return rc;
    skip[i] = buf<u16>(c, nm.c_str());
  }
  u16* A = buf<u16>(c, "unet16.a");
  u16* Bq = buf<u16>(c, "unet16.b");
  auto L = [&](const std::string& n) -> const sh_ctx::ULayer& { return c->ulayers[n]; };
  if ((rc = ensure(c, "unet16.zero", 256, 2)) != SH_OK) return rc;
  if (!c->zero_page_ready) { HIPCHK(c, hipMemsetAsync(buf<char>(c, "unet16.zero"), 0, 256, c->stream)); c->zero_page_ready = true; }
  const u16* zp = (const u16*)c->bufs["unet16.zero"].p;
  int h = H, w = W;
  if (fused) {
    const sh_ctx::ULayer& la = L("enc0a");
    const sh_ctx::ULayer& lb = L("enc0b");
    const int total = nimg * (w / 32) * (h / 16);
    const unsigned grid = (unsigned)std::min(total, persistent_grid(c));
    unsigned* tk = nullptr; const int* tk_tab = nullptr; int ntk = 0;
    if ((rc = unet_tickets(c, total, (int)grid, 1, &tk, &tk_tab, &ntk)) != SH_OK) return rc;
    LAUNCH_FN(c, "unet.enc0b", launch_enc0_pp(EK, grid, c->stream, image, P + la.w_off, P + la.b_off, PW + lb.w_off, P + lb.b_off, skip[0], A, h, w, nimg,
                                              c->unet_raw, c->unet_mm, tk, tk_tab, ntk));
  } else {
    const sh_ctx::ULayer& l = L("enc0a");
    size_t npx = (size_t)nimg * h * w;
    LAUNCH(c, "unet.enc0a", k_conv_first16<EK>, dim3((unsigned)std::min<size_t>((npx + 255) / 256, 8192)), dim3(256), image, P + l.w_off, P + l.b_off, A, h, w, l.cout, nimg);
    if ((rc = conv_layer16<EK>(c, "unet.enc0b", L("enc0b"), A, nullptr, base, 0, skip[0], h, w, nimg, 1)) != SH_OK) return rc;
  }
  int ch = base;
  for (int i = 1; i <= D; ++i) {
    if (!fused) {
      size_t e = (size_t)nimg * (h / 2) * (w / 2) * (ch / 8);
      LAUNCH(c, "unet.pool", k_maxpool2_16<EK>, dim3((unsigned)std::min<size_t>((e + 255) / 256, 8192)), dim3(256), skip[i - 1], A, h, w, ch, nimg);
    }
    h /= 2; w /= 2;
    std::string na = i < D ? "enc" + std::to_string(i) + "a" : "bota", nb = i < D ? "enc" + std::to_string(i) + "b" : "botb";
    if ((rc = conv_layer16<EK>(c, ("unet." + na).c_str(), L(na), A, nullptr, ch, 0, Bq, h, w, nimg, 1)) != SH_OK) return rc;
    ch *= 2;
    u16* dst = i < D ? skip[i] : A;
    ConvFuse fz{};
    fz.pooled = A;
    if ((rc = conv_layer16<EK>(c, ("unet." + nb).c_str(), L(nb), Bq, nullptr, ch, 0, dst, h, w, nimg, 1, (fused && i < D) ? UF_POOL : 0, fz)) != SH_OK) return rc;
  }
  u16* x = A; u16* y = Bq;
  for (int i = D - 1; i >= 0; --i) {
    std::string nu = "up" + std::to_string(i), na = "dec" + std::to_string(i) + "a", nb = "dec" + std::to_string(i) + "b";
    if (fused && i == 0) {
      h *= 2; w *= 2; ch /= 2;
      const sh_ctx::ULayer& lu = L(nu);
      const sh_ctx::ULayer& la = L(na);
      const sh_ctx::ULayer& lb = L(nb);
      const sh_ctx::ULayer& lh = L("head");
      {
        const int total = nimg * (w / 32) * (h / 8);
        const unsigned grid = (unsigned)std::min(total, persistent_grid(c));
        unsigned* tk = nullptr; const int* tk_tab = nullptr; int ntk = 0;
        if ((rc = unet_tickets(c, total, (int)grid, 1, &tk, &tk_tab, &ntk)) != SH_OK) return rc;
        LAUNCH_FN(c, "unet.dec0a", launch_dec0a_up_pp(EK, grid, c->stream, skip[0], x, PW + la.w_off, P + la.b_off, PW + lu.w_off, P + lu.b_off, y, h, w, nimg,
                                                      zp, tk, tk_tab, ntk));
      }
      {
        const int total = nimg * (w / 32) * (h / 16);
        const unsigned grid = (unsigned)std::min(total, persistent_grid(c));
        unsigned* tk = nullptr; const int* tk_tab = nullptr; int ntk = 0;
        if ((rc = unet_tickets(c, total, (int)grid, 1, &tk, &tk_tab, &ntk)) != SH_OK) return rc;
        LAUNCH_FN(c, "unet.dec0b", launch_dec0b_head_pp(EK, grid, c->stream, y, PW + lb.w_off, P + lb.b_off, P + lh.w_off, P + lh.b_off, logits, h, w, nimg,
                                                        zp, tk, tk_tab, ntk));
      }
      return SH_OK;
    }
    if ((rc = conv_layer16<EK>(c, ("unet." + nu).c_str(), L(nu), x, nullptr, ch, 0, y, h, w, nimg, 0)) != SH_OK) return rc;
    h *= 2; w *= 2; ch /= 2;
    if ((rc = conv_layer16<EK>(c, ("unet." + na).c_str(), L(na), skip[i], y, ch, ch, x, h, w, nimg, 1)) != SH_OK) return rc;
    if ((rc = conv_layer16<EK>(c, ("unet." + nb).c_str(), L(nb), x, nullptr, ch, 0, y, h, w, nimg, 1)) != SH_OK) return rc;
    std::swap(x, y);
  }
  {
    const sh_ctx::ULayer& l = L("head");
    size_t npx = (size_t)nimg * H * W;
    LAUNCH(c, "unet.head", k_head16<EK>, dim3((unsigned)std::min<size_t>((npx + 255) / 256, 8192)), dim3(256), x, P + l.w_off, P + l.b_off, logits, l.cin, npx, (size_t)H * W);
  }
  return SH_OK;
}

static int unet_dispatch(sh_ctx* c, const float* image, float* logits, int nimg, int H, int W) {
  switch (c->params.unet_dtype) {
    case SH_UNET_BF16: return unet_forward16<0>(c, image, logits, nimg, H, W);
    case SH_UNET_F16: return unet_forward16<1>(c, image, logits, nimg, H, W);
    default: return unet_forward(c, image, logits, nimg, H, W);
  }
}

extern "C" {

int sh_unet_infer(sh_ctx* c, const float* images, int n, int H, int W, float* logits) {
  if (!c || !images || !logits || n <= 0 || H <= 0 || W <= 0) return fail(c, SH_ERR_ARG, "sh_unet_infer: bad argument");
  if (c->ulayers.empty()) return fail(c, SH_ERR_STATE, "sh_unet_infer: no UNet weights loaded");
  HIPCHK(c, hipSetDevice(c->device));
  const size_t bytes = (size_t)n * H * W * 4;
  int rc;
  if ((rc = ensure(c, "infer.image", bytes, 4)) != SH_OK) return rc;
  if ((rc = ensure(c, "infer.logits", bytes, 4)) != SH_OK) return rc;
  const int b0 = c->b0; c->b0 = 0;
  HIPCHK(c, hipMemcpyAsync(buf<float>(c, "infer.image"), images, bytes, hipMemcpyHostToDevice, c->stream));
  rc = unet_dispatch(c, buf<float>(c, "infer.image"), buf<float>(c, "infer.logits"), n, H, W);
  c->b0 = b0;
  if (rc != SH_OK) { (void)hipStreamSynchronize(c->stream); return rc; }
  HIPCHK(c, hipMemcpyAsync(logits, buf<float>(c, "infer.logits"), bytes, hipMemcpyDeviceToHost, c->stream));
  HIPCHK(c, hipStreamSynchronize(c->stream));
  return SH_OK;
}

static int ovf_pools(sh_ctx* c, OvfPools* P) {
  int rc;
  if ((rc = ensure(c, "ovf.segs", c->ovf_seg_cap * sizeof(Seg), 1)) != SH_OK) return rc;
  if ((rc = ensure(c, "ovf.ring", c->ovf_ring_cap * 16, 8)) != SH_OK) return rc;
  if ((rc = ensure(c, "ovf.work", c->ovf_work_cap, 1)) != SH_OK) return rc;
  if ((rc = ensure(c, "ovf.ctr", 128, 8)) != SH_OK) return rc;
  for (const char* n : {"ovf.segs", "ovf.ring", "ovf.work", "ovf.ctr"}) c->bufs[n].per_mesh = 0;
  P->segs = (Seg*)c->bufs["ovf.segs"].p; P->ring = (double*)c->bufs["ovf.ring"].p; P->work = (unsigned char*)c->bufs["ovf.work"].p;
  P->seg_cap = c->ovf_seg_cap; P->ring_cap = c->ovf_ring_cap; P->work_cap = c->ovf_work_cap;
  P->ctr = (unsigned long long*)c->bufs["ovf.ctr"].p;
  P->open_mode = c->open_mode;
  return SH_OK;
}
static int ovf_set(sh_ctx* c, const std::string& pfx, int N, OvfSet* S) {
  const size_t B = (size_t)c->B;
  int rc;
  struct A { const char* suffix; size_t elem; } arr[6] = {{".ovf_soff", 8}, {".ovf_roff", 8}, {".ovf_woff", 8}, {".ovf_fill", 4}, {".ovf_list", 4}, {".ovf_list2", 4}};
  for (const A& a : arr) {
    const std::string nm = pfx + a.suffix;
    const bool fresh = c->bufs.find(nm) == c->bufs.end() || c->bufs[nm].bytes < B * N * a.elem;
    if ((rc = ensure(c, nm.c_str(), B * N * a.elem, (int)a.elem)) != SH_OK) return rc;
    c->bufs[nm].per_mesh = (size_t)N * a.elem;
    if (fresh) HIPCHK(c, hipMemsetAsync(c->bufs[nm].p, 0xFF, B * N * a.elem, c->stream));
  }
  if ((rc = ensure(c, (pfx + ".ovf_nlist").c_str(), 16, 4)) != SH_OK) return rc;
  c->bufs[pfx + ".ovf_nlist"].per_mesh = 0;
  S->soff = buf<long long>(c, (pfx + ".ovf_soff").c_str()); S->roff = buf<long long>(c, (pfx + ".ovf_roff").c_str());
  S->woff = buf<long long>(c, (pfx + ".ovf_woff").c_str()); S->fill = buf<int>(c, (pfx + ".ovf_fill").c_str());
  S->list = buf<int>(c, (pfx + ".ovf_list").c_str()); S->nlist = (int*)c->bufs[pfx + ".ovf_nlist"].p; S->list2 = buf<int>(c, (pfx + ".ovf_list2").c_str());
  return SH_OK;
}

struct SliceSpec { const char* pfx; int kind, N; bool ring, resample; int select; bool total_area, decode_bounds; };
static int run_slice_sets(sh_ctx* c, const SliceSpec* specs, int nspec) {
  const int B = c->Bwin;
  if (nspec < 1 || nspec > 2) return fail(c, SH_ERR_STATE, "run_slice_sets: one or two sets");
  int ntot = 0;
  for (int i = 0; i < nspec; ++i) ntot += specs[i].N;
  if (ntot > SH_EMIT_MAXN) return fail(c, SH_ERR_CAPACITY, "slice sets have more planes than k_slice_emit's LDS histogram");
  OvfPools OP; OvfSet OS[2];
  { int orc; if ((orc = ovf_pools(c, &OP)) != SH_OK) return orc; }
  const bool ovf_on = c->ovf_none_gen != c->batch_gen;
  SliceSets sets{};
  sets.n = nspec;
  sets.vobb = buf<double>(c, "verts_obb"); sets.voff = buf<long long>(c, "voff");
  sets.open = OpenCfg{c->open_mode, c->open_gap, c->open_mode ? buf<int>(c, "open.stats") : (int*)nullptr};
  for (int i = 0; i < nspec; ++i) {
    const SliceSpec& sp = specs[i];
    const std::string p = sp.pfx;
    { int orc; if ((orc = ovf_set(c, p, sp.N, &OS[i])) != SH_OK) return orc; }
    SliceSetDev& S = sets.s[i];
    S.N = sp.N; S.kind = sp.kind; S.select = sp.select;
    S.zb = buf<double>(c, sp.kind == 4 ? "obb.zb_pre" : "z_bounds");
    S.zs = buf<double>(c, (p + ".zs").c_str()); S.zeff = buf<double>(c, (p + ".zeff").c_str());
    S.seg_count = buf<int>(c, (p + ".seg_count").c_str()); S.segs = buf<Seg>(c, (p + ".segs").c_str());
    S.centroids = buf<double>(c, (p + ".centroids").c_str()); S.areas = buf<double>(c, (p + ".areas").c_str()); S.nloops = buf<int>(c, (p + ".nloops").c_str());
    S.ring_n = buf<int>(c, (p + ".ring_n").c_str());
    S.ring = sp.ring ? buf<double>(c, (p + ".ring").c_str()) : (double*)nullptr;
    S.areas_total = sp.total_area ? buf<double>(c, (p + ".area_total").c_str()) : (double*)nullptr;
    S.nlarge = (int*)c->bufs["slices.nlarge"].p + (sp.kind & 7);
    S.many = ManyLoops{ovf_on ? OS[i].list2 : (int*)nullptr, ovf_on ? OS[i].nlist + 1 : (int*)nullptr, ovf_on ? (unsigned long long*)nullptr : OP.ctr + 6};
    S.ovf_missed = ovf_on ? (unsigned long long*)nullptr : OP.ctr + 6;
    S.aux = PlaneAux{sp.decode_bounds ? (const unsigned long long*)buf<unsigned long long>(c, "zb_enc") : (const unsigned long long*)nullptr, buf<double>(c, "z_bounds"), S.seg_count, S.nlarge,
                     ovf_on ? OS[i].nlist : (int*)nullptr, i == 0 ? OP.ctr : (unsigned long long*)nullptr};
  }
  LAUNCH(c, "k_make_planes", k_make_planes, dim3(B, nspec), dim3(256), sets, (const double*)buf<double>(c, "neck_z"), B);
  dim3 g((unsigned)std::min<long long>((c->maxF + 255) / 256, 4096), (unsigned)B);
  LAUNCH(c, "k_slice_emit", k_slice_emit, g, dim3(256), buf<double>(c, "verts_obb"), buf<int>(c, "faces"), buf<long long>(c, "voff"), buf<long long>(c, "foff"), sets);
  if (ovf_on)
    for (int i = 0; i < nspec; ++i) {
      const SliceSetDev& S = sets.s[i];
      LAUNCH(c, "k_ovf_plan", k_ovf_plan, dim3((unsigned)((B * S.N + 255) / 256)), dim3(256), S.N, B * S.N, (const int*)S.seg_count, OP, OS[i], buf<int>(c, "err"));
      LAUNCH(c, "k_slice_emit_ovf", k_slice_emit_ovf, g, dim3(256), buf<double>(c, "verts_obb"), buf<int>(c, "faces"), buf<long long>(c, "voff"),
             buf<long long>(c, "foff"), (const double*)S.zeff, S.N, OP, OS[i]);
    }
  if (c->open_mode != SH_OPEN_ERROR) {
    LAUNCH(c, "k_slice_link", k_slice_link<true>, dim3(B * ntot), dim3(SH_LINK_THREADS), sets, B, buf<int>(c, "err"));
    LAUNCH(c, "k_slice_link_large", k_slice_link_large<true>, dim3(std::min(B * ntot, 512)), dim3(SH_LINK_THREADS), sets, B, buf<int>(c, "err"));
  } else {
    LAUNCH(c, "k_slice_link", k_slice_link<false>, dim3(B * ntot), dim3(SH_LINK_THREADS), sets, B, buf<int>(c, "err"));
    LAUNCH(c, "k_slice_link_large", k_slice_link_large<false>, dim3(std::min(B * ntot, 512)), dim3(SH_LINK_THREADS), sets, B, buf<int>(c, "err"));
  }
  for (int i = 0; i < nspec; ++i) {
    const SliceSpec& sp = specs[i];
    const SliceSetDev& S = sets.s[i];
    if (ovf_on) {
      LAUNCH(c, "k_ovf_plan_loops", k_ovf_plan_loops, dim3(16), dim3(256), S.N, (const int*)S.seg_count, (const Seg*)S.segs, OP, OS[i], buf<int>(c, "err"));
      if (c->open_mode != SH_OPEN_ERROR)
        LAUNCH(c, "k_slice_link_huge", k_slice_link_huge<true>, dim3(64), dim3(SH_HUGE_THREADS), S.N, (const int*)S.seg_count, OP, OS[i], S.centroids, S.areas, S.nloops, S.ring_n,
             sp.ring ? 1 : 0, S.select, buf<int>(c, "err"), S.areas_total, (const double*)buf<double>(c, "verts_obb"), (const long long*)buf<long long>(c, "voff"), (const double*)S.zeff, sets.open);
      else
        LAUNCH(c, "k_slice_link_huge", k_slice_link_huge<false>, dim3(64), dim3(SH_HUGE_THREADS), S.N, (const int*)S.seg_count, OP, OS[i], S.centroids, S.areas, S.nloops, S.ring_n,
             sp.ring ? 1 : 0, S.select, buf<int>(c, "err"), S.areas_total, (const double*)buf<double>(c, "verts_obb"), (const long long*)buf<long long>(c, "voff"), (const double*)S.zeff, sets.open);
    }
    if (sp.resample) {
      RsWant want{c->keep_products ? 1 : 0, SH_ANP_ROW0, 0, 0};
      cutoff_range(SH_NPROX, c->params.groove_cutoff[0], c->params.groove_cutoff[1], &want.cs_lo, &want.cs_hi);
      if (c->b0 == 0) { c->rs_cs_lo = want.cs_lo; c->rs_cs_hi = want.cs_hi; c->rs_all = c->keep_products; c->rs_gen = c->batch_gen; }
      LAUNCH(c, "k_resample_polar", k_resample_polar, dim3(B * S.N), dim3(SH_RS_THREADS), S.N, SH_MPROX, S.ring_n, S.ring,
             S.centroids, buf<double>(c, "prox.ixy"), buf<double>(c, "prox.itr_start"), buf<double>(c, "prox.itr_centered_start"), (const long long*)OS[i].roff, want);
      LAUNCH(c, "k_resample_polar_large", k_resample_polar_large, dim3(std::min(B * S.N, 512)), dim3(SH_RS_THREADS), B * S.N, S.N, SH_MPROX, S.ring_n, S.ring,
             S.centroids, buf<double>(c, "prox.ixy"), buf<double>(c, "prox.itr_start"), buf<double>(c, "prox.itr_centered_start"), (const int*)S.nlarge, (const long long*)OS[i].roff, want);
      if (ovf_on) {
        LAUNCH(c, "k_resample_polar_huge", k_resample_polar_huge, dim3(64), dim3(SH_RS_THREADS), S.N, SH_MPROX, (const int*)S.ring_n, OP, OS[i],
               S.centroids, buf<double>(c, "prox.ixy"), buf<double>(c, "prox.itr_start"), buf<double>(c, "prox.itr_centered_start"), want);
      }
    }
  }
  return SH_OK;
}
static int run_slice_set(sh_ctx* c, const char* pfx, int kind, int N, bool ring, bool resample, int select = 0, bool total_area = false, bool decode_bounds = false) {
  const SliceSpec sp{pfx, kind, N, ring, resample, select, total_area, decode_bounds};
  return run_slice_sets(c, &sp, 1);
}

struct HullPre { const float* verts; const long long* voff; int* ext; double* planes; int* npl; float* kept; int* nkept; long long* koff; double* pval; int* pidx; int* pcnt; long long* poff; };
static HullPre hullpre_ptrs(sh_ctx* c) {
  return HullPre{(const float*)c->bufs["verts"].p, (const long long*)c->bufs["voff"].p, (int*)c->bufs["hullpre.ext"].p, (double*)c->bufs["hullpre.planes"].p,
                 (int*)c->bufs["hullpre.npl"].p, (float*)c->bufs["hullpre.kept"].p, (int*)c->bufs["hullpre.nkept"].p, (long long*)c->bufs["hullpre.koff"].p,
                 (double*)c->bufs["hullpre.pval"].p, (int*)c->bufs["hullpre.pidx"].p, (int*)c->bufs["hullpre.pcnt"].p, (long long*)c->bufs["hullpre.poff"].p};
}
static void launch_prefilter(const HullPre& hp, int B, hipStream_t st) {
  hipLaunchKernelGGL(k_hullpre_extremes, dim3(SH_HP_PARTS, B), dim3(256), 0, st, hp.verts, hp.voff, hp.pval, hp.pidx);
  hipLaunchKernelGGL(k_hullpre_polytope, dim3(B), dim3(256), 0, st, hp.verts, hp.voff, (const double*)hp.pval, (const int*)hp.pidx, hp.ext, hp.planes, hp.npl);
  hipLaunchKernelGGL(k_hullpre_filter<false>, dim3(SH_HP_PARTS, B), dim3(256), 0, st, hp.verts, hp.voff, (const double*)hp.planes, (const int*)hp.npl,
                     (const long long*)hp.poff, hp.kept, hp.pcnt);
  hipLaunchKernelGGL(k_hullpre_offsets, dim3(1), dim3(64), 0, st, (const int*)hp.pcnt, hp.koff, hp.poff, hp.nkept, B);
  hipLaunchKernelGGL(k_hullpre_filter<true>, dim3(SH_HP_PARTS, B), dim3(256), 0, st, hp.verts, hp.voff, (const double*)hp.planes, (const int*)hp.npl,
                     (const long long*)hp.poff, hp.kept, hp.pcnt);
}

static hipError_t fetch_prefiltered(const HullPre& hp, int B, long long sumV, long long* h_koff, float* h_kept, sh_ctx::HullPts* out, hipStream_t st) {
  hipError_t e;
  launch_prefilter(hp, B, st);
  if ((e = hipGetLastError()) != hipSuccess) return e;
  if ((e = hipMemcpyAsync(h_koff, hp.koff, (size_t)(B + 1) * 8, hipMemcpyDeviceToHost, st)) != hipSuccess) return e;
  if ((e = hipStreamSynchronize(st)) != hipSuccess) return e;
  const long long total = h_koff[B];
  if (total < 0 || total > sumV) return hipErrorUnknown;
  if (total > 0 && (e = hipMemcpyAsync(h_kept, hp.kept, (size_t)total * 12, hipMemcpyDeviceToHost, st)) != hipSuccess) return e;
  if ((e = hipStreamSynchronize(st)) != hipSuccess) return e;
  out->off.resize(B); out->cnt.resize(B);
  for (int b = 0; b < B; ++b) { out->off[b] = h_koff[b]; out->cnt[b] = (int)(h_koff[b + 1] - h_koff[b]); }
  out->src = h_kept;
  return hipSuccess;
}

static hipError_t fetch_hull_points(sh_ctx* c, const HullPre& hp, hipStream_t st) {
  const int B = c->B;
  sh_ctx::HullPts& in = c->hull_in;
  in.cnt.resize(B);
  if (c->h_verts_valid) {
    in.off.assign(c->h_voff.begin(), c->h_voff.begin() + B);
    for (int b = 0; b < B; ++b) in.cnt[b] = (int)(c->h_voff[b + 1] - c->h_voff[b]);
    in.src = c->h_verts.data();
    return hipSuccess;
  }
  hipError_t e;
  if (!c->sw.hull_prefilter || !hp.kept) {
    c->h_verts.resize(3 * (size_t)c->sumV);
    if ((e = hipMemcpyAsync(c->h_verts.data(), hp.verts, c->sumV * 3 * 4, hipMemcpyDeviceToHost, st)) != hipSuccess) return e;
    if ((e = hipStreamSynchronize(st)) != hipSuccess) return e;
    in.off.assign(c->h_voff.begin(), c->h_voff.begin() + B);
    for (int b = 0; b < B; ++b) in.cnt[b] = (int)(c->h_voff[b + 1] - c->h_voff[b]);
    in.src = c->h_verts.data();
    return hipSuccess;
  }
  return fetch_prefiltered(hp, B, c->sumV, c->h_koff, c->h_kept, &in, st);
}

class HullPool {
 public:
  static HullPool& instance() { static HullPool p; return p; }
  static unsigned thread_count() {
    unsigned nt = std::min(threads_per_local_rank(false), 32u);
    if (const char* e = getenv("SHOULDER_HULL_THREADS")) { int v = atoi(e); if (v > 0) nt = (unsigned)v; }
    return nt;
  }
  void run(const std::function<void()>& fn, int items) {
    Job job;
    job.fn = fn;
    job.want = (int)std::min<unsigned>(std::max(1, items), (unsigned)workers_.size() + 1) - 1;
    if (job.want > 0) {
      { std::lock_guard<std::mutex> lk(mu_); queue_.push_back(&job); }
      cv_.notify_all();
    }
    fn();
    if (job.want > 0) {
      std::unique_lock<std::mutex> lk(mu_);
      auto it = std::find(queue_.begin(), queue_.end(), &job);
      if (it != queue_.end()) queue_.erase(it);
      done_cv_.wait(lk, [&] { return job.active == 0; });
    }
  }

 private:
  struct Job { std::function<void()> fn; int want = 0, taken = 0, active = 0; };
  HullPool() {
    const unsigned nt = thread_count();
    for (unsigned t = 1; t < nt; ++t) workers_.emplace_back([this] { loop(); });
  }
  ~HullPool() {
    { std::lock_guard<std::mutex> lk(mu_); stop_ = true; }
    cv_.notify_all();
    for (auto& t : workers_) t.join();
  }
  void loop() {
    std::unique_lock<std::mutex> lk(mu_);
    for (;;) {
      cv_.wait(lk, [&] { return stop_ || !queue_.empty(); });
      if (stop_) return;
      Job* j = queue_.front();
      ++j->taken; ++j->active;
      if (j->taken >= j->want) queue_.pop_front();
      lk.unlock();
      j->fn();
      lk.lock();
      if (--j->active == 0) done_cv_.notify_all();
    }
  }
  std::mutex mu_;
  std::condition_variable cv_, done_cv_;
  std::deque<Job*> queue_;
  std::vector<std::thread> workers_;
  bool stop_ = false;
};

struct HullPhaseGate {
  std::mutex m; std::condition_variable cv; bool busy = false; std::atomic<int> fg_waiting{0};
  void enter(bool background) {
    std::unique_lock<std::mutex> l(m);
    if (!background) ++fg_waiting;
    cv.wait(l, [&] { return !busy && (!background || fg_waiting.load() == 0); });
    if (!background) --fg_waiting;
    busy = true;
  }
  bool foreground_waits() const { return fg_waiting.load(std::memory_order_relaxed) > 0; }
  void leave() { { std::lock_guard<std::mutex> l(m); busy = false; } cv.notify_all(); }
  static HullPhaseGate& instance() { static HullPhaseGate g; return g; }
};

static int hull_host_phase(sh_ctx* c, const sh_ctx::HullPts& in, int slot, int b0, int B, int* bad_mesh, double* ms, std::string* errtxt, bool background = false) {
  auto t0 = std::chrono::steady_clock::now();
  sh_ctx::HullStage& hs = c->hstage[slot];
#define HULLCHK(call) do { hipError_t e_ = (call); if (e_ != hipSuccess) { *errtxt = std::string(#call) + ": " + hipGetErrorString(e_); return SH_ERR_HIP; } } while (0)
  bool grown = false;
again:
  if (hs.cap < B || grown) {
    if (hs.hv) { (void)hipHostFree(hs.hv); (void)hipHostFree(hs.nr); (void)hipHostFree(hs.ed); (void)hipHostFree(hs.cnt); }
    hs.hv = nullptr; hs.cap = 0;
    HULLCHK(hipHostMalloc((void**)&hs.hv, (size_t)B * hs.pv * 3 * 8));
    HULLCHK(hipHostMalloc((void**)&hs.nr, (size_t)B * hs.pf * 3 * 8));
    HULLCHK(hipHostMalloc((void**)&hs.ed, (size_t)B * hs.pe * 4 * 4));
    HULLCHK(hipHostMalloc((void**)&hs.cnt, (size_t)B * 3 * 4));
    hs.cap = B;
  }
  if (!hs.ev) HULLCHK(hipEventCreateWithFlags(&hs.ev, hipEventDisableTiming));
  if (hs.used) HULLCHK(hipEventSynchronize(hs.ev));
  {
    sh_ctx::HullStage& ho = c->hstage[slot ^ 1];
    if (!ho.hv && !grown) {
      ho.pv = hs.pv; ho.pf = hs.pf; ho.pe = hs.pe;
      HULLCHK(hipHostMalloc((void**)&ho.hv, (size_t)B * ho.pv * 3 * 8));
      HULLCHK(hipHostMalloc((void**)&ho.nr, (size_t)B * ho.pf * 3 * 8));
      HULLCHK(hipHostMalloc((void**)&ho.ed, (size_t)B * ho.pe * 4 * 4));
      HULLCHK(hipHostMalloc((void**)&ho.cnt, (size_t)B * 3 * 4));
      ho.cap = B;
    }
  }
#undef HULLCHK
  double* hv = hs.hv; double* nr = hs.nr; int* ed = hs.ed; int* counts = hs.cnt;
  std::vector<int> status(B, 0);
  std::vector<int> demand(3 * (size_t)B, 0);
  std::atomic<int> next(0);
  auto work = [&]() {
    std::vector<double> P;
    shhull::Hull H;
    for (;;) {
      if (background && HullPhaseGate::instance().foreground_waits()) break;
      int b = next.fetch_add(1);
      if (b >= B) break;
      counts[b] = counts[B + b] = counts[2 * B + b] = 0;
      long long v0 = in.off[b0 + b], nv = in.cnt[b0 + b];
      P.resize(3 * (size_t)nv);
      const float* src = in.src + 3 * v0;
      for (long long i = 0; i < 3 * nv; ++i) P[i] = (double)src[i];
      if (!shhull::convex_hull(P.data(), (int)nv, H)) { status[b] = SH_ERR_GEOMETRY; continue; }
      int hn = (int)H.vert_ids.size(), fn = (int)H.tris.size() / 3, en = (int)H.edges.size() / 4;
      if (hn > hs.pv || fn > hs.pf || en > hs.pe) { status[b] = 1; demand[3 * (size_t)b] = hn; demand[3 * (size_t)b + 1] = fn; demand[3 * (size_t)b + 2] = en; continue; }
      for (int i = 0; i < hn; ++i)
        for (int k = 0; k < 3; ++k) hv[((size_t)b * hs.pv + i) * 3 + k] = P[3 * (size_t)H.vert_ids[i] + k];
      std::copy(H.normals.begin(), H.normals.end(), nr + (size_t)b * hs.pf * 3);
      std::copy(H.edges.begin(), H.edges.end(), ed + (size_t)b * hs.pe * 4);
      counts[b] = hn; counts[B + b] = fn; counts[2 * B + b] = en;
    }
  };
  do {
    HullPhaseGate::instance().enter(background);
    HullPool::instance().run(work, B);
    HullPhaseGate::instance().leave();
  } while (next.load() < B);
  if (!grown && std::find(status.begin(), status.end(), 1) != status.end()) {
    int dv = SH_HV, df = SH_HF, de = SH_HE;
    for (int b = 0; b < B; ++b) { dv = std::max(dv, demand[3 * (size_t)b]); df = std::max(df, demand[3 * (size_t)b + 1]); de = std::max(de, demand[3 * (size_t)b + 2]); }
    auto up = [](int x) { return (x + 1023) / 1024 * 1024; };
    hs.pv = up(dv); hs.pf = up(df); hs.pe = up(de);
    grown = true;
    std::fill(status.begin(), status.end(), 0);
    next = 0;
    goto again;
  }
  *ms = std::chrono::duration<double, std::milli>(std::chrono::steady_clock::now() - t0).count();
  for (int b = 0; b < B; ++b)
    if (status[b] != 0) { *bad_mesh = b0 + b; return status[b] == 1 ? SH_ERR_CAPACITY : status[b]; }
  return SH_OK;
}

static bool hull_fits(const sh_ctx* c, int slot, int B, int* need ) {
  const int* counts = c->hstage[slot].cnt;
  int nvmax = 1, nfmax = 1, nemax = 1;
  for (int b = 0; b < B; ++b) { nvmax = std::max(nvmax, counts[b]); nfmax = std::max(nfmax, counts[B + b]); nemax = std::max(nemax, counts[2 * B + b]); }
  if (need) { need[0] = nvmax; need[1] = nfmax; need[2] = nemax; }
  return nvmax <= c->hcap.v && nfmax <= c->hcap.f && nemax <= c->hcap.e;
}
static int grow_hull_records(sh_ctx* c, int nv, int nf, int ne) {
  auto up = [](int x) { return (x + x / 8 + 1023) / 1024 * 1024; };
  HIPCHK(c, hipStreamSynchronize(c->stream));
  if (nv > c->hcap.v) c->hcap.v = up(nv);
  if (nf > c->hcap.f) c->hcap.f = up(nf);
  if (ne > c->hcap.e) c->hcap.e = up(ne);
  const size_t B = (size_t)c->B;
  const struct { const char* n; size_t per; int elem; } arr[] = {
      {"hull.hv", (size_t)c->hcap.v * 24, 8}, {"hull.normals", (size_t)c->hcap.f * 24, 8}, {"hull.edges", (size_t)c->hcap.e * 16, 4},
      {"obb.cand_vol", (size_t)c->hcap.f * 8, 8}, {"obb.cand_edge", (size_t)c->hcap.f * 4, 4}, {"obb.area2", (size_t)c->hcap.f * 8, 8},
      {"obb.lb", (size_t)c->hcap.f * 8, 8}, {"obb.dir_list", (size_t)c->hcap.f * 4, 4}, {"obb.seeded", (size_t)c->hcap.f, 1}};
  for (const auto& a : arr) {
    if (int e = ensure(c, a.n, B * a.per, a.elem)) return e;
    c->bufs[a.n].per_mesh = a.per;
  }
  if (c->sw.debug) fprintf(stderr, "[sh] hull record grown to %d vertices / %d faces / %d edges per humerus\n", c->hcap.v, c->hcap.f, c->hcap.e);
  return SH_OK;
}
static hipError_t hull_upload(sh_ctx* c, int slot, int B, void* const dst[6], hipStream_t st) {
  sh_ctx::HullStage& hs = c->hstage[slot];
  const int* counts = hs.cnt;
  int nvmax = 1, nfmax = 1, nemax = 1;
  for (int b = 0; b < B; ++b) { nvmax = std::max(nvmax, counts[b]); nfmax = std::max(nfmax, counts[B + b]); nemax = std::max(nemax, counts[2 * B + b]); }
  if (nvmax > c->hcap.v || nfmax > c->hcap.f || nemax > c->hcap.e) return hipErrorInvalidValue;
  hipError_t e;
  if ((e = hipMemcpy2DAsync(dst[0], (size_t)c->hcap.v * 24, hs.hv, (size_t)hs.pv * 24, (size_t)nvmax * 24, B, hipMemcpyHostToDevice, st)) != hipSuccess) return e;
  if ((e = hipMemcpy2DAsync(dst[1], (size_t)c->hcap.f * 24, hs.nr, (size_t)hs.pf * 24, (size_t)nfmax * 24, B, hipMemcpyHostToDevice, st)) != hipSuccess) return e;
  if ((e = hipMemcpy2DAsync(dst[2], (size_t)c->hcap.e * 16, hs.ed, (size_t)hs.pe * 16, (size_t)nemax * 16, B, hipMemcpyHostToDevice, st)) != hipSuccess) return e;
  if ((e = hipMemcpyAsync(dst[3], counts, (size_t)B * 4, hipMemcpyHostToDevice, st)) != hipSuccess) return e;
  if ((e = hipMemcpyAsync(dst[4], counts + B, (size_t)B * 4, hipMemcpyHostToDevice, st)) != hipSuccess) return e;
  if ((e = hipMemcpyAsync(dst[5], counts + 2 * B, (size_t)B * 4, hipMemcpyHostToDevice, st)) != hipSuccess) return e;
  if ((e = hipEventRecord(hs.ev, st)) != hipSuccess) return e;
  hs.used = true;
  return hipSuccess;
}

static bool device_hull_now(const sh_ctx* c) { return c->hull_mode == 1 && !(c->hull_force_host && c->obb_gen == c->batch_gen); }

static int run_obb(sh_ctx* c, int prepared_slot) {
  const int B = c->Bwin, b0 = c->b0;
  int nfmax = 1;
  if (c->obb_gen != c->batch_gen) { c->obb_gen = c->batch_gen; c->obb_sil_need = 0; c->obb_nf_over = false; c->hull_force_host = false; }
  if (c->redo_records) {
    nfmax = std::max(1, c->redo_nf);
  } else if (device_hull_now(c)) {
    { int arc = alloc_hulld(c); if (arc != SH_OK) return arc; }
    launch_prefilter(hullpre_ptrs(c), B, c->stream);
    HIPCHK(c, hipGetLastError());
    HullScratch hs{buf<int>(c, "hulld.fv"), buf<int>(c, "hulld.vis"), buf<int>(c, "hulld.ev"), buf<int>(c, "hulld.hor"), buf<int>(c, "hulld.newslot"),
                   buf<int>(c, "hulld.freestack"), buf<unsigned long long>(c, "hulld.tkeys"), buf<unsigned>(c, "hulld.tvals")};
    LAUNCH(c, "k_hull_rounds", k_hull_rounds, dim3(B), dim3(HD_THREADS), (const float*)c->bufs["hullpre.kept"].p, (const long long*)c->bufs["hullpre.koff"].p, hs,
           buf<double>(c, "hull.hv"), buf<double>(c, "hull.normals"), buf<int>(c, "hull.edges"), buf<int>(c, "hull.nv"), buf<int>(c, "hull.nf"), buf<int>(c, "hull.ne"),
           buf<int>(c, "hulld.fail"), buf<int>(c, "hulld.rounds"), (const int*)buf<int>(c, "hulld.skip"), c->hcap);
    LAUNCH(c, "k_hull_flag", k_hull_flag, dim3((B + 63) / 64), dim3(64), buf<int>(c, "hulld.fail"), buf<int>(c, "err"), B);
    nfmax = std::max((int)HD_SLOTS, c->skip_nfmax);
  } else {
  int slot = prepared_slot;
  if (slot < 0) {
    slot = c->hslot; c->hslot ^= 1;
    int bad = -1; double ms = 0; std::string et;
    int hrc = hull_host_phase(c, c->hull_in, slot, b0, B, &bad, &ms, &et);
    if (c->sw.debug) fprintf(stderr, "[sh] run_obb: foreground hull phase %.2f ms\n", ms);
    if (c->timing) { KTimer& h = c->timers["host.hull"]; h.ms += ms; h.n += 1; }
    if (hrc == SH_ERR_HIP) { c->err = et; return hrc; }
    if (hrc != SH_OK) { char m[96]; snprintf(m, sizeof m, "mesh %d: convex hull failed (%d)", bad, hrc); return fail(c, hrc, m); }
  }
  const int* counts = c->hstage[slot].cnt;
  for (int b = 0; b < B; ++b) nfmax = std::max(nfmax, counts[B + b]);
  {
    int need[3];
    if (!hull_fits(c, slot, B, need)) {
      int grc = grow_hull_records(c, need[0], need[1], need[2]);
      if (grc != SH_OK) return grc;
    }
  }
  if (!(prepared_slot >= 0 && c->prep.uploaded)) {
    void* const dst[6] = {buf<double>(c, "hull.hv"), buf<double>(c, "hull.normals"), buf<int>(c, "hull.edges"), buf<int>(c, "hull.nv"), buf<int>(c, "hull.nf"), buf<int>(c, "hull.ne")};
    HIPCHK(c, hull_upload(c, slot, B, dst, c->stream));
  }
  }
  const int* cnt_nv = buf<int>(c, "hull.nv");
  const int* cnt_nf = buf<int>(c, "hull.nf");
  const int* cnt_ne = buf<int>(c, "hull.ne");
  {
    FILL(c, {buf<unsigned long long>(c, "obb.best_enc"), (size_t)B * 8, 0xFF} , {buf<unsigned long long>(c, "obb.lbmin_enc"), (size_t)B * 8, 0xFF},
         {buf<double>(c, "obb.area2"), (size_t)B * c->hcap.f * 8, 0}, {buf<int>(c, "obb.endcnt"), (size_t)B * 2 * 4, 0},
         {buf<unsigned long long>(c, "zb_enc"), (size_t)B * 16, 0xFF} , {buf<unsigned long long>(c, "anp.mm_enc"), (size_t)B * 16, 0xFF});
    c->bounds_cleared = true;
    const int nemax = 3 * nfmax / 2 + 3;
    const HullCap hc = c->hcap;
    LAUNCH(c, "k_obb_face_area2", k_obb_face_area2, dim3((unsigned)((std::min(nemax, hc.e) + 255) / 256), (unsigned)B), dim3(256), buf<double>(c, "hull.hv"),
           buf<double>(c, "hull.normals"), buf<int>(c, "hull.edges"), cnt_ne, buf<double>(c, "obb.area2"), hc);
    const int bnd_tiles = (nfmax + SH_OBB_BND_DIRS - 1) / SH_OBB_BND_DIRS;
    LAUNCH(c, "k_obb_bounds", k_obb_bounds, dim3((unsigned)(bnd_tiles * ((B + 7) / 8) * 8)), dim3(SH_OBB_BND_THREADS),
           buf<double>(c, "hull.hv"), cnt_nv, buf<double>(c, "hull.normals"), cnt_nf, buf<double>(c, "obb.area2"), buf<double>(c, "obb.lb"),
           buf<unsigned long long>(c, "obb.lbmin_enc"), buf<double>(c, "obb.cand_vol"), buf<int>(c, "obb.cand_edge"), bnd_tiles, B, hc);
    const bool huge = nfmax > 32768 || c->obb_sil_need > 2048 || c->obb_nf_over;
    const bool big = !huge && (nfmax > 8192 || c->obb_sil_need > 512);
    const int TT = (big || huge) ? 8 : SH_OBB_TILE;
    const int ntiles = (nfmax + TT - 1) / TT;
    ObbWs ws{};
    ws.need = (unsigned long long*)c->bufs["ovf.ctr"].p + 8;
    if (huge) {
      ws.nwg = 256;
      ws.silcap = std::max(hc.v + 64, c->obb_sil_need + c->obb_sil_need / 8);
      int wrc;
      if ((wrc = ensure(c, "obb.ws_fmask", (size_t)ws.nwg * hc.f, 1)) != SH_OK || (wrc = ensure(c, "obb.ws_lists", (size_t)ws.nwg * 8 * ws.silcap * 4, 4)) != SH_OK ||
          (wrc = ensure(c, "obb.ws_sxy", (size_t)ws.nwg * ws.silcap * 16, 8)) != SH_OK || (wrc = ensure(c, "obb.ws_area", (size_t)ws.nwg * ws.silcap * 8, 8)) != SH_OK) return wrc;
      for (const char* n : {"obb.ws_fmask", "obb.ws_lists", "obb.ws_sxy", "obb.ws_area"}) c->bufs[n].per_mesh = 0;
      ws.fmask = (unsigned char*)c->bufs["obb.ws_fmask"].p; ws.lists = (unsigned*)c->bufs["obb.ws_lists"].p;
      ws.sxy = (double2*)c->bufs["obb.ws_sxy"].p; ws.area = (double*)c->bufs["obb.ws_area"].p;
    }
    const bool prune = c->sw.obb_prune;
    for (int pass = 0; pass < 2; ++pass) {
      LAUNCH(c, "k_obb_select", k_obb_select, dim3(B), dim3(256), buf<double>(c, "obb.lb"), cnt_nf, buf<unsigned long long>(c, "obb.lbmin_enc"),
             buf<unsigned long long>(c, "obb.best_enc"), (prune || pass == 0) ? pass : 2, buf<int>(c, "obb.dir_list"), buf<int>(c, "obb.dir_count"), buf<unsigned char>(c, "obb.seeded"), hc);
      const int nt_pass = pass == 0 ? SH_OBB_TILE / TT : ntiles;
      const dim3 cg((unsigned)(nt_pass * ((B + 7) / 8) * 8));
      if (huge) {
        LAUNCH(c, pass == 0 ? "k_obb_seed" : "k_obb_candidates", (k_obb_candidates<8, 1, 0, 0, unsigned, true>), dim3((unsigned)std::min<unsigned>(cg.x, (unsigned)ws.nwg)), dim3(SH_OBB_THREADS),
               buf<double>(c, "hull.hv"), cnt_nv, buf<double>(c, "hull.normals"), cnt_nf, buf<int>(c, "hull.edges"), cnt_ne, buf<double>(c, "obb.cand_vol"),
               buf<int>(c, "obb.cand_edge"), buf<int>(c, "err"), buf<unsigned long long>(c, "obb.best_enc"), buf<int>(c, "obb.dir_list"), buf<int>(c, "obb.dir_count"),
               nt_pass, B, prune ? 1 : 0, hc, ws);
      } else if (big) {
        LAUNCH(c, pass == 0 ? "k_obb_seed" : "k_obb_candidates", (k_obb_candidates<8, 1, 2048, 32768, unsigned>), cg, dim3(SH_OBB_THREADS),
               buf<double>(c, "hull.hv"), cnt_nv, buf<double>(c, "hull.normals"), cnt_nf, buf<int>(c, "hull.edges"), cnt_ne, buf<double>(c, "obb.cand_vol"),
               buf<int>(c, "obb.cand_edge"), buf<int>(c, "err"), buf<unsigned long long>(c, "obb.best_enc"), buf<int>(c, "obb.dir_list"), buf<int>(c, "obb.dir_count"),
               nt_pass, B, prune ? 1 : 0, hc, ws);
      } else {
        LAUNCH(c, pass == 0 ? "k_obb_seed" : "k_obb_candidates", (k_obb_candidates<SH_OBB_TILE, SH_OBB_GROUP, 512, 8192, unsigned short>), cg, dim3(SH_OBB_THREADS),
               buf<double>(c, "hull.hv"), cnt_nv, buf<double>(c, "hull.normals"), cnt_nf, buf<int>(c, "hull.edges"), cnt_ne, buf<double>(c, "obb.cand_vol"),
               buf<int>(c, "obb.cand_edge"), buf<int>(c, "err"), buf<unsigned long long>(c, "obb.best_enc"), buf<int>(c, "obb.dir_list"), buf<int>(c, "obb.dir_count"),
               nt_pass, B, prune ? 1 : 0, hc, ws);
      }
    }
  }
  LAUNCH(c, "k_obb_pick", k_obb_pick, dim3(B), dim3(256), buf<double>(c, "hull.hv"), buf<double>(c, "hull.normals"), cnt_nf, buf<int>(c, "hull.edges"),
         buf<double>(c, "obb.cand_vol"), buf<int>(c, "obb.cand_edge"), buf<float>(c, "verts"), buf<long long>(c, "voff"), buf<double>(c, "obb.T_pre"),
         buf<double>(c, "obb.zb_pre"), buf<int>(c, "err"), c->hcap);
  if (!c->obb_done_ev) HIPCHK(c, hipEventCreateWithFlags(&c->obb_done_ev, hipEventDisableTiming));
  HIPCHK(c, hipEventRecord(c->obb_done_ev, c->stream));
  if (c->params.bone_kind == SH_BONE_PROXIMAL) {
    dim3 gv((unsigned)std::min<long long>((c->maxV + 255) / 256, 1024), (unsigned)B);
    LAUNCH(c, "k_transform_verts", k_transform_verts, gv, dim3(256), buf<float>(c, "verts"), buf<long long>(c, "voff"),
           buf<double>(c, "obb.T_pre"), buf<double>(c, "verts_obb"), buf<unsigned long long>(c, "zb_enc"));
    c->bounds_cleared = false;
    int rc2;
    if ((rc2 = run_slice_set(c, "pobb", 4, SH_NPSCAN, false, false, 0, true)) != SH_OK) return rc2;
    LAUNCH(c, "k_prox_obb", k_prox_obb, dim3((B + 63) / 64), dim3(64), buf<double>(c, "pobb.area_total"), buf<double>(c, "pobb.zs"), buf<double>(c, "obb.T_pre"),
           buf<double>(c, "obb_transform"), buf<int>(c, "flipped"), buf<double>(c, "pobb.cutoff"), buf<int>(c, "pobb.cutoff_idx"), buf<int>(c, "err"), B);
    c->obb_injected = true;
    return SH_OK;
  }
  dim3 g((unsigned)std::min<long long>((c->maxF + 255) / 256, 1024), (unsigned)B);
  LAUNCH(c, "k_obb_end_points", k_obb_end_points, g, dim3(256), buf<float>(c, "verts"), buf<int>(c, "faces"), buf<long long>(c, "voff"),
         buf<long long>(c, "foff"), buf<double>(c, "obb.T_pre"), buf<double>(c, "obb.zb_pre"), buf<double>(c, "obb.endpts"), buf<int>(c, "obb.endcnt"), c->end_cap);
  LAUNCH(c, "k_obb_ends", k_obb_ends, dim3(B), dim3(128), buf<double>(c, "obb.endpts"), buf<int>(c, "obb.endcnt"),
         buf<double>(c, "obb.T_pre"), buf<double>(c, "obb.resid"), buf<double>(c, "obb_transform"), buf<int>(c, "flipped"), buf<int>(c, "err"), B, c->end_cap,
         (unsigned long long*)c->bufs["ovf.ctr"].p + 7);
  c->obb_injected = true;
  return SH_OK;
}

static int run_te_rows(sh_ctx* c) {
  const int B = c->Bwin;
  OvfPools OP; OvfSet OS;
  { int orc; if ((orc = ovf_pools(c, &OP)) != SH_OK || (orc = ovf_set(c, "distal", SH_NDIST, &OS)) != SH_OK) return orc; }
  LAUNCH(c, "k_te_rows", k_te_rows<SH_SMALLSEG>, dim3(B * SH_TE_NROWS), dim3(64), buf<double>(c, "distal.ring"), buf<int>(c, "distal.ring_n"),
         buf<double>(c, "te.rects"), B, (const long long*)OS.roff);
  LAUNCH(c, "k_te_rows_large", k_te_rows<SH_MAXSEG>, dim3(B * SH_TE_NROWS), dim3(64), buf<double>(c, "distal.ring"), buf<int>(c, "distal.ring_n"),
         buf<double>(c, "te.rects"), B, (const long long*)OS.roff);
  if (c->ovf_none_gen != c->batch_gen) {
    LAUNCH(c, "k_te_rows_huge", k_te_rows_huge, dim3(64), dim3(64), OP, OS, (const int*)buf<int>(c, "distal.ring_n"), buf<double>(c, "te.rects"));
  }
  LAUNCH(c, "k_te_ends", k_te_ends, dim3(B), dim3(64), buf<double>(c, "distal.ring"), buf<int>(c, "distal.ring_n"), buf<double>(c, "te.rects"),
         buf<double>(c, "distal.zs"), buf<double>(c, "obb_transform"), buf<double>(c, "te.ends_ct"), buf<int>(c, "te.row"), buf<int>(c, "err"), B, OP, OS);
  return SH_OK;
}

static int run_window(sh_ctx* c, uint32_t mask, int prepared_slot) {
  const int B = c->Bwin;
  int rc;
  c->bounds_cleared = false;
  if (mask & SH_STAGE_OBB)
    if ((rc = run_obb(c, prepared_slot)) != SH_OK) return rc;
  if (!c->bounds_cleared && (mask & (SH_STAGE_OBB | SH_STAGE_FULL | SH_STAGE_ANP)))
    FILL(c, {buf<unsigned long long>(c, "zb_enc"), (size_t)B * 16, 0xFF}, {buf<unsigned long long>(c, "anp.mm_enc"), (size_t)B * 16, 0xFF});
  const bool transformed = (mask & (SH_STAGE_OBB | SH_STAGE_FULL)) != 0;
  if (transformed) {
    dim3 g((unsigned)std::min<long long>((c->maxV + 255) / 256, 1024), (unsigned)B);
    LAUNCH(c, "k_transform_verts", k_transform_verts, g, dim3(256), buf<float>(c, "verts"), buf<long long>(c, "voff"),
           buf<double>(c, "obb_transform"), buf<double>(c, "verts_obb"), buf<unsigned long long>(c, "zb_enc"));
    if (!(mask & SH_STAGE_FULL))
      LAUNCH(c, "k_decode_bounds", k_decode_bounds, dim3((2 * B + 63) / 64), dim3(64), buf<unsigned long long>(c, "zb_enc"), buf<double>(c, "z_bounds"), B);
  }
  const bool merge_env = c->sw.slice_merge;
  const bool can_fork = (mask & SH_STAGE_DISTAL) && c->ovf_none_gen == c->batch_gen && c->timing != 1 && !c->redo_records;
  const bool side = can_fork && B <= 16;
  bool te_rows_done = false;
  c->side_pending = false;
  const bool merge_fd = merge_env && (mask & SH_STAGE_FULL) && (mask & SH_STAGE_DISTAL) && !side;
  if (merge_fd) {
    const SliceSpec sp[2] = {{"full", 0, SH_NFULL, false, false, 0, false, transformed}, {"distal", 2, SH_NDIST, true, false, 0, false, transformed}};
    if ((rc = run_slice_sets(c, sp, 2)) != SH_OK) return rc;
  } else if (mask & SH_STAGE_FULL) {
    if ((rc = run_slice_set(c, "full", 0, SH_NFULL, false, false, 0, false, transformed)) != SH_OK) return rc;
  }
  if (mask & SH_STAGE_DISTAL) {
    hipStream_t main_stream = c->stream;
    if (side) {
      if (!c->side_stream) HIPCHK(c, hipStreamCreateWithFlags(&c->side_stream, hipStreamNonBlocking));
      if (!c->side_fork_ev) { HIPCHK(c, hipEventCreateWithFlags(&c->side_fork_ev, hipEventDisableTiming)); HIPCHK(c, hipEventCreateWithFlags(&c->side_join_ev, hipEventDisableTiming)); }
      HIPCHK(c, hipEventRecord(c->side_fork_ev, main_stream));
      HIPCHK(c, hipStreamWaitEvent(c->side_stream, c->side_fork_ev, 0));
      c->stream = c->side_stream;
    }
    rc = merge_fd ? SH_OK : run_slice_set(c, "distal", 2, SH_NDIST, true, false);
    const bool te_inline = !side && (mask & SH_STAGE_ANP);
    if (rc == SH_OK && (side || te_inline) && (mask & SH_STAGE_TE)) { rc = run_te_rows(c); te_rows_done = rc == SH_OK; }
    if (side) {
      c->stream = main_stream;
      if (rc == SH_OK) { HIPCHK(c, hipEventRecord(c->side_join_ev, c->side_stream)); c->side_pending = true; }
    }
    if (rc != SH_OK) return rc;
  }
  if (mask & SH_STAGE_NECK) {
    const bool prox = c->params.bone_kind == SH_BONE_PROXIMAL;
    if (prox) {
      LAUNCH(c, "k_neck", k_neck<true>, dim3(B), dim3(64), buf<double>(c, "full.areas"), buf<double>(c, "full.zs"),
             buf<double>(c, "neck_z"), buf<int>(c, "neck_index"), B, 0.2, 0.99, buf<double>(c, "neck.gram"));
    } else {
      LAUNCH(c, "k_neck", k_neck<false>, dim3(B), dim3(64), buf<double>(c, "full.areas"), buf<double>(c, "full.zs"),
             buf<double>(c, "neck_z"), buf<int>(c, "neck_index"), B, 0.70, 0.99, (double*)nullptr);
    }
    if (merge_env && (mask & SH_STAGE_PROXIMAL)) {
      const SliceSpec sp[2] = {{"neckc", 3, 1, true, false, 1, false, false}, {"prox", 1, SH_NPROX, true, true, 0, false, false}};
      if ((rc = run_slice_sets(c, sp, 2)) != SH_OK) return rc;
    } else if ((rc = run_slice_set(c, "neckc", 3, 1, true, false, 1)) != SH_OK) return rc;
  }
  if (mask & SH_STAGE_CANAL) {
    LAUNCH(c, "k_canal", k_canal, dim3(B), dim3(64), buf<double>(c, "full.centroids"), buf<double>(c, "full.zs"),
           buf<double>(c, "z_bounds"), buf<double>(c, "obb_transform"), c->params.canal_cutoff[0], c->params.canal_cutoff[1],
           c->params.bone_kind == SH_BONE_PROXIMAL ? buf<double>(c, "pobb.cutoff") : (const double*)nullptr,
           buf<double>(c, "canal.points_obb"), buf<double>(c, "canal.axis_obb"), buf<double>(c, "canal.axis_ct"), buf<int>(c, "err"));
  }
  if ((mask & SH_STAGE_PROXIMAL) && !(merge_env && (mask & SH_STAGE_NECK)))
    if ((rc = run_slice_set(c, "prox", 1, SH_NPROX, true, true)) != SH_OK) return rc;
  if (mask & SH_STAGE_GROOVE) {
    if (!c->have_rfc) return fail(c, SH_ERR_STATE, "sh_run: groove stage needs sh_load_rfc first");
    int ga, gb;
    cutoff_range(SH_NPROX, c->params.groove_cutoff[0], c->params.groove_cutoff[1], &ga, &gb);
    if (!(mask & SH_STAGE_PROXIMAL) && !(c->rs_gen == c->batch_gen && (c->rs_all || (ga >= c->rs_cs_lo && gb <= c->rs_cs_hi))))
      return fail(c, SH_ERR_STATE, "sh_run: SH_STAGE_GROOVE without SH_STAGE_PROXIMAL, and the proximal slices of this batch were not made for this groove_cutoff (run SH_STAGE_PROXIMAL again)");
    const char* pp = buf<char>(c, "params") + c->unet_floats * 4;
    const size_t N = c->h_feat.size();
    const int* feat = (const int*)pp; const float* thr = (const float*)(pp + N * 4); const int* ti = (const int*)(pp + N * 8);
    const int* fi = (const int*)(pp + N * 12); const float* lw = (const float*)(pp + N * 16); const int* roots = (const int*)(pp + N * 20);
    const int rows = B * SH_GROOVE_NROWS;
    LAUNCH(c, "k_groove_rows", k_groove_rows, dim3(rows), dim3(64), buf<double>(c, "prox.itr_centered_start"),
           buf<double>(c, "prox.zs"), buf<double>(c, "canal.axis_ct"), ga, buf<double>(c, "groove.xraw"),
           buf<double>(c, "groove.ptheta"), buf<int>(c, "groove.npk"), buf<double>(c, "groove.r0"), buf<int>(c, "err"), B);
    LAUNCH(c, "k_groove_scale", k_groove_scale, dim3(B), dim3(256), buf<double>(c, "groove.xraw"), buf<int>(c, "groove.npk"),
           buf<double>(c, "groove.stats"), B, buf<int>(c, "groove.slots"), buf<int>(c, "groove.nslot"), buf<float>(c, "groove.proba"));
    if ((rc = ensure(c, "rfc.nodes", N * 16, 4)) != SH_OK) return rc;
    int4* nodes = (int4*)c->bufs["rfc.nodes"].p;
    if (!c->packed_rfc) {
      LAUNCH(c, "k_rfc_pack", k_rfc_pack, dim3((unsigned)((N + 255) / 256)), dim3(256), feat, thr, ti, fi, lw, nodes, (int)N);
      c->packed_rfc = true;
    }
    LAUNCH(c, "k_groove_rfc", k_groove_rfc, dim3((unsigned)(B * ((SH_GSLOTS + 63) / 64))), dim3(64), buf<double>(c, "groove.xraw"), buf<int>(c, "groove.slots"), buf<int>(c, "groove.nslot"),
           buf<double>(c, "groove.stats"), nodes, roots, c->rfc_trees, buf<double>(c, "groove.xs"), buf<float>(c, "groove.proba"), B);
    LAUNCH(c, "k_groove_tail", k_groove_tail, dim3(B), dim3(256), buf<double>(c, "groove.ptheta"), buf<float>(c, "groove.proba"), buf<double>(c, "groove.bg_theta"), buf<int>(c, "err"),
           buf<double>(c, "prox.itr_centered_start"), buf<double>(c, "groove.r0"), buf<double>(c, "prox.zs"), buf<double>(c, "prox.centroids"), ga, c->params.groove_deg_window,
           buf<int>(c, "groove.local_idx"), buf<double>(c, "groove.points_obb"), buf<double>(c, "obb_transform"), buf<double>(c, "groove.axis_ct"), buf<double>(c, "groove.points_ct"));
  }
  if (mask & SH_STAGE_ANP) {
    if (!c->have_unet) return fail(c, SH_ERR_STATE, "sh_run: anatomic-neck stage needs sh_load_unet first");
    LAUNCH(c, "k_anp_rows", k_anp_rows, dim3(B * SH_ANP_ROWS), dim3(64), buf<double>(c, "prox.itr_start"),
           buf<double>(c, "groove.bg_theta"), buf<double>(c, "anp.raw"), buf<double>(c, "anp.t01"), buf<int>(c, "anp.roll"), B,
           buf<unsigned long long>(c, "anp.mm_enc"));
    const bool scale_in_net = (c->params.unet_dtype == SH_UNET_BF16 || c->params.unet_dtype == SH_UNET_F16) && unet16_starts_fused(c, SH_ANP_ROWS, SH_MPROX);
    if (!scale_in_net || c->keep_products)
      LAUNCH(c, "k_anp_scale", k_anp_scale, dim3(64, B), dim3(256), buf<double>(c, "anp.raw"), buf<unsigned long long>(c, "anp.mm_enc"), buf<float>(c, "anp.image"));
    if ((rc = unet_turn_enter(c)) != SH_OK) return rc;
    if (scale_in_net) { c->unet_raw = buf<double>(c, "anp.raw"); c->unet_mm = buf<unsigned long long>(c, "anp.mm_enc"); }
    rc = unet_dispatch(c, buf<float>(c, "anp.image"), buf<float>(c, "anp.logits"), B, SH_ANP_ROWS, SH_MPROX);
    c->unet_raw = nullptr; c->unet_mm = nullptr;
    (void)unet_turn_leave(c);
    if (rc != SH_OK) return rc;
    LAUNCH(c, "k_anp_edge_count", k_anp_edge_count, dim3(SH_ANP_ROWS / 8, B), dim3(512), buf<float>(c, "anp.logits"), buf<int>(c, "anp.rowcnt"), buf<unsigned long long>(c, "anp.maskbits"));
    LAUNCH(c, "k_anp_edges", k_anp_edges, dim3(SH_ANP_ROWS / 8, B), dim3(512), buf<unsigned long long>(c, "anp.maskbits"), buf<double>(c, "anp.raw"),
           buf<double>(c, "anp.t01"), buf<int>(c, "anp.roll"), buf<double>(c, "prox.zs"), buf<int>(c, "anp.rowcnt"), buf<double>(c, "anp.points_obb"), buf<int>(c, "anp.counts"),
           buf<int>(c, "err"));
    LAUNCH(c, "k_anp_plane", k_anp_plane, dim3(B), dim3(256), buf<double>(c, "anp.points_obb"), buf<int>(c, "anp.counts"),
           buf<double>(c, "anp.plane"), buf<int>(c, "err"), buf<unsigned long long>(c, "anp.ray_t"));
    LAUNCH(c, "k_rays_hit", k_rays_hit, dim3(SH_RAY_CHUNKS, B), dim3(256), buf<double>(c, "verts_obb"), buf<int>(c, "faces"), buf<long long>(c, "voff"),
           buf<long long>(c, "foff"), buf<double>(c, "anp.plane"), buf<unsigned long long>(c, "anp.ray_t"));
  }
  if (mask & SH_STAGE_TE) {
    if (c->side_pending) { HIPCHK(c, hipStreamWaitEvent(c->stream, c->side_join_ev, 0)); c->side_pending = false; }
    if (!te_rows_done && (rc = run_te_rows(c)) != SH_OK) return rc;
  }
  if (c->side_pending) { HIPCHK(c, hipStreamWaitEvent(c->stream, c->side_join_ev, 0)); c->side_pending = false; }
  const uint32_t need = SH_STAGE_GROOVE | SH_STAGE_ANP | SH_STAGE_CSYS | (c->params.bone_kind == SH_BONE_PROXIMAL ? 0u : (uint32_t)SH_STAGE_TE);
  const bool metrics = (mask & need) == need;
  if (metrics)
    LAUNCH(c, "k_sphere_partial", k_sphere_partial, dim3(SH_SPH_PARTS, B), dim3(256), buf<unsigned long long>(c, "anp.maskbits"), buf<double>(c, "anp.raw"),
           buf<double>(c, "anp.t01"), buf<int>(c, "anp.roll"), buf<double>(c, "prox.zs"), buf<double>(c, "anp.plane"), buf<double>(c, "metrics.partial"));
  {
    PackArgs A{};
    A.lm = buf<sh_landmarks>(c, "landmarks"); A.T_obb = buf<double>(c, "obb_transform"); A.zb = buf<double>(c, "z_bounds"); A.neck_z = buf<double>(c, "neck_z");
    A.neck_index = buf<int>(c, "neck_index"); A.flipped = buf<int>(c, "flipped"); A.canal_axis_ct = buf<double>(c, "canal.axis_ct"); A.te_axis_ct = buf<double>(c, "te.axis_ct");
    A.groove_axis_ct = buf<double>(c, "groove.axis_ct"); A.bg_theta = buf<double>(c, "groove.bg_theta"); A.groove_pts_ct = buf<double>(c, "groove.points_ct");
    A.plane = buf<double>(c, "anp.plane"); A.axes_obb = buf<double>(c, "anp.axes_obb"); A.anp_pts_obb = buf<double>(c, "anp.points_obb"); A.anp_counts = buf<int>(c, "anp.counts");
    A.err = buf<int>(c, "err"); A.mask = mask; A.B = B; A.bone_kind = (int)c->params.bone_kind;
    A.canal_cut = c->params.bone_kind == SH_BONE_PROXIMAL ? buf<double>(c, "pobb.cutoff") : (const double*)nullptr;
    A.cc0 = c->params.canal_cutoff[0]; A.cc1 = c->params.canal_cutoff[1];
    A.ray_t = buf<unsigned long long>(c, "anp.ray_t"); A.te_ends_ct = buf<double>(c, "te.ends_ct"); A.sphere_partial = buf<double>(c, "metrics.partial"); A.metrics = metrics ? 1 : 0;
    LAUNCH(c, "k_tail", k_tail, dim3(B), dim3(256), A);
  }
  if (mask & SH_STAGE_APPLY) {
    dim3 g((unsigned)std::min<long long>((c->maxV + 255) / 256, 1024), (unsigned)B);
    LAUNCH(c, "k_apply_csys", k_apply_csys, g, dim3(256), buf<sh_landmarks>(c, "landmarks"), buf<float>(c, "verts"), buf<long long>(c, "voff"), buf<double>(c, "verts_csys"));
  }
  return SH_OK;
}

#define SH_WINDOW (1 << 30)

static int join_prepared(sh_ctx* c) {
  if (!c->prep.active) return SH_OK;
  if (c->prep.th.joinable()) c->prep.th.join();
  c->prep.active = false;
  if (c->timing) {
    KTimer& h = c->timers["host.hull"]; h.ms += c->prep.hull_ms; h.n += 1;
    if (c->prep.d2h_ms > 0) { KTimer& a = c->timers["host.verts_d2h"]; a.ms += c->prep.d2h_ms; a.n += 1; }
  }
  return c->prep.rc;
}

static void start_prepare(sh_ctx* c) {
  sh_ctx::Prepared& p = c->prep;
  p.active = true; p.slot = c->hslot; p.B = c->B; p.gen = c->batch_gen; p.rc = SH_OK; p.bad_mesh = -1; p.d2h_ms = p.hull_ms = 0; p.err.clear();
  p.uploaded = false; p.staged = false;
  const HullPre hp = hullpre_ptrs(c);
  struct Dst { void* p[6]; } dst = {{buf<double>(c, "hull.hv"), buf<double>(c, "hull.normals"), buf<int>(c, "hull.edges"), buf<int>(c, "hull.nv"), buf<int>(c, "hull.nf"), buf<int>(c, "hull.ne")}};
  const bool can_upload = c->obb_done_ev != nullptr;
  p.th = std::thread([c, hp, dst, can_upload]() {
    sh_ctx::Prepared& q = c->prep;
    if (hipSetDevice(c->device) != hipSuccess) { q.rc = SH_ERR_HIP; return; }
    if (!c->copy_stream && hipStreamCreateWithFlags(&c->copy_stream, hipStreamNonBlocking) != hipSuccess) { q.rc = SH_ERR_HIP; return; }
    {
      auto t0 = std::chrono::steady_clock::now();
      if (fetch_hull_points(c, hp, c->copy_stream) != hipSuccess) { q.rc = SH_ERR_HIP; return; }
      q.d2h_ms = std::chrono::duration<double, std::milli>(std::chrono::steady_clock::now() - t0).count();
    }
    q.rc = hull_host_phase(c, c->hull_in, q.slot, 0, q.B, &q.bad_mesh, &q.hull_ms, &q.err, true);
    if (q.rc == SH_OK && can_upload) {
      if (hipStreamWaitEvent(c->copy_stream, c->obb_done_ev, 0) == hipSuccess && hull_upload(c, q.slot, q.B, dst.p, c->copy_stream) == hipSuccess &&
          hipStreamSynchronize(c->copy_stream) == hipSuccess)
        q.uploaded = true;
    }
  });
}

int sh_set_overlap(sh_ctx* c, int on) {
  if (!c) return SH_ERR_ARG;
  c->overlap = on != 0;
  return SH_OK;
}

int sh_set_unet_turns(sh_ctx* c, int on) {
  if (!c) return SH_ERR_ARG;
  c->unet_turn = on != 0;
  if (!c->unet_turn) unet_turn_forget(c);
  return SH_OK;
}

int sh_discard_prepared(sh_ctx* c) {
  if (!c) return SH_ERR_ARG;
  (void)join_prepared(c);
  c->prep.gen = ~0ull;
  return SH_OK;
}

#define SH_REC_HEAD offsetof(sh_landmarks, anp_points)
#define SH_REC_TAIL (sizeof(sh_landmarks) - SH_REC_HEAD - sizeof(((sh_landmarks*)0)->anp_points))
static inline size_t rec_bytes_rows(int rows) { return rows > 0 ? SH_REC_HEAD + SH_REC_TAIL + (size_t)rows * 24 : sizeof(sh_landmarks); }

__global__ void __launch_bounds__(256)
k_wire_records(const sh_landmarks* __restrict__ lm, unsigned char* __restrict__ dst, int R, size_t rec) {
  const int b = blockIdx.x, tid = threadIdx.x;
  const unsigned long long* src = (const unsigned long long*)(lm + b);
  unsigned long long* d = (unsigned long long*)(dst + (size_t)b * rec);
  constexpr int HEAD = (int)(SH_REC_HEAD / 8), TAIL = (int)(SH_REC_TAIL / 8), PTS = (int)(sizeof(((sh_landmarks*)0)->anp_points) / 8);
  for (int i = tid; i < HEAD; i += 256) d[i] = src[i];
  for (int i = tid; i < TAIL; i += 256) d[HEAD + i] = src[HEAD + PTS + i];
  int n = lm[b].n_anp;
  n = n < 0 ? 0 : (n > R ? R : n);
  for (int i = tid; i < 3 * R; i += 256) d[HEAD + TAIL + i] = i < 3 * n ? src[HEAD + i] : 0ull;
}

static int emit_records(sh_ctx* c, void* dst, int b0, int n, int rows, size_t rec) {
  const sh_landmarks* src = (const sh_landmarks*)c->bufs["landmarks"].p + b0;
  if (rows <= 0) { HIPCHK(c, hipMemcpyAsync((char*)dst + (size_t)b0 * rec, src, (size_t)n * rec, hipMemcpyDeviceToDevice, c->stream)); return SH_OK; }
  LAUNCH(c, "k_wire_records", k_wire_records, dim3(n), dim3(256), src, (unsigned char*)dst + (size_t)b0 * rec, rows, rec);
  return SH_OK;
}

__global__ void k_anp_points_ct(const double* __restrict__ pts_obb, const double* __restrict__ T_obb, int b, int n, double* __restrict__ out) {
  double Ti[16];
  inv_transform(T_obb + 16 * b, Ti);
  for (int i = blockIdx.x * blockDim.x + threadIdx.x; i < n; i += gridDim.x * blockDim.x) {
    const double* p = pts_obb + ((size_t)b * SH_ANP_CAP + i) * 3;
    xform_pt(Ti, p[0], p[1], p[2], out + 3 * (size_t)i);
  }
}

static void discard_staged(sh_ctx* c) {
  sh_ctx::StageSide& S = c->stg;
  if (!S.active) return;
  if (c->prep.staged) { (void)join_prepared(c); c->prep.gen = ~0ull; c->prep.staged = false; }
  (void)hipEventSynchronize(S.ready_ev);
  S.active = false;
}

#define SH_COPY_THREADS 4
static hipError_t staged_h2d(void* dev, void* pinned, const void* src, size_t n, hipStream_t st) {
  const size_t chunk = (size_t)4 << 20;
  const size_t nch = (n + chunk - 1) / chunk;
  if (nch == 0) return hipSuccess;
  std::atomic<size_t> next(0);
  std::atomic<int> err((int)hipSuccess);
  auto work = [&]() {
    for (;;) {
      const size_t k = next.fetch_add(1);
      if (k >= nch) break;
      const size_t o = k * chunk, m = std::min(chunk, n - o);
      memcpy((char*)pinned + o, (const char*)src + o, m);
      const hipError_t e = hipMemcpyAsync((char*)dev + o, (char*)pinned + o, m, hipMemcpyHostToDevice, st);
      if (e != hipSuccess) err.store((int)e);
    }
  };
  std::vector<std::thread> th;
  for (int t = 1; t < SH_COPY_THREADS && (size_t)t < nch; ++t) th.emplace_back(work);
  work();
  for (auto& t : th) t.join();
  return (hipError_t)err.load();
}

static bool is_pinned_host(const void* p) {
  hipPointerAttribute_t at{};
  const bool pinned = hipPointerGetAttributes(&at, p) == hipSuccess && at.type == hipMemoryTypeHost;
  (void)hipGetLastError();
  return pinned;
}

static int stage_common_alloc(sh_ctx* c, int B, long long sumV_cap, long long sumF_cap, size_t flag_ints) {
  sh_ctx::StageSide& S = c->stg;
  int rc;
  if (!c->copy_stream) HIPCHK(c, hipStreamCreateWithFlags(&c->copy_stream, hipStreamNonBlocking));
  if (!S.ready_ev) HIPCHK(c, hipEventCreateWithFlags(&S.ready_ev, hipEventDisableTiming));
  if (S.h_flag_cap < flag_ints) {
    if (S.h_flag) (void)hipHostFree(S.h_flag);
    S.h_flag = nullptr; S.h_flag_cap = 0;
    HIPCHK(c, hipHostMalloc((void**)&S.h_flag, flag_ints * 4));
    S.h_flag_cap = flag_ints;
  }
  if (S.h_kept_cap < sumV_cap) {
    if (S.h_kept) (void)hipHostFree(S.h_kept);
    S.h_kept = nullptr; S.h_kept_cap = 0;
    HIPCHK(c, hipHostMalloc((void**)&S.h_kept, (size_t)sumV_cap * 12));
    S.h_kept_cap = sumV_cap;
  }
  if (S.h_koff_cap < B + 1) {
    if (S.h_koff) (void)hipHostFree(S.h_koff);
    S.h_koff = nullptr; S.h_koff_cap = 0;
    HIPCHK(c, hipHostMalloc((void**)&S.h_koff, (size_t)(B + 1) * 8));
    S.h_koff_cap = B + 1;
  }
#define ENSS(name, bytes, elem) do { if ((rc = ensure(c, name, (size_t)(bytes), elem)) != SH_OK) return rc; c->bufs[name].per_mesh = 0; } while (0)
  ENSS("verts.s", sumV_cap * 12, 4);
  ENSS("faces.s", sumF_cap * 12, 4);
  ENSS("voff.s", (size_t)(B + 1) * 8, 8);
  ENSS("foff.s", (size_t)(B + 1) * 8, 8);
  ENSS("stage.flag", 64, 4);
  ENSS("hullpre.ext.s", (size_t)B * SH_HP_NDIR * 4, 4);
  ENSS("hullpre.planes.s", (size_t)B * SH_HP_MAXPL * 4 * 8, 8);
  ENSS("hullpre.npl.s", (size_t)B * 4, 4);
  ENSS("hullpre.nkept.s", (size_t)B * 4, 4);
  ENSS("hullpre.pval.s", (size_t)B * SH_HP_PARTS * SH_HP_NDIR * 8, 8);
  ENSS("hullpre.pidx.s", (size_t)B * SH_HP_PARTS * SH_HP_NDIR * 4, 4);
  ENSS("hullpre.pcnt.s", (size_t)B * SH_HP_PARTS * 4, 4);
  ENSS("hullpre.poff.s", (size_t)B * SH_HP_PARTS * 8, 8);
  ENSS("hullpre.koff.s", (size_t)(B + 1) * 8, 8);
  ENSS("hullpre.kept.s", (size_t)sumV_cap * 12, 4);
#undef ENSS
  return SH_OK;
}

static HullPre hullpre_ptrs_staged(sh_ctx* c) {
  return HullPre{(const float*)c->bufs["verts.s"].p, (const long long*)c->bufs["voff.s"].p, (int*)c->bufs["hullpre.ext.s"].p, (double*)c->bufs["hullpre.planes.s"].p,
                 (int*)c->bufs["hullpre.npl.s"].p, (float*)c->bufs["hullpre.kept.s"].p, (int*)c->bufs["hullpre.nkept.s"].p, (long long*)c->bufs["hullpre.koff.s"].p,
                 (double*)c->bufs["hullpre.pval.s"].p, (int*)c->bufs["hullpre.pidx.s"].p, (int*)c->bufs["hullpre.pcnt.s"].p, (long long*)c->bufs["hullpre.poff.s"].p};
}

struct StlPhase { bool on = false; int tsize = 0; long long maxc = 0; void *corners, *coff, *table, *slot, *vid, *fpos, *voff_d, *foff_d, *verts_d, *faces_d; hipEvent_t counted = nullptr; };

static void start_prepare_staged(sh_ctx* c, bool hulls, const StlPhase stl, std::function<int(std::string*)> phase0) {
  sh_ctx::Prepared& p = c->prep;
  sh_ctx::StageSide& S = c->stg;
  p.active = true; p.staged = true; p.slot = c->hslot; p.B = S.B; p.gen = hulls ? c->batch_gen + 1 : ~0ull; p.rc = SH_OK; p.bad_mesh = -1; p.d2h_ms = p.hull_ms = 0; p.err.clear();
  p.uploaded = false;
  const HullPre hp = hullpre_ptrs_staged(c);
  struct Dst { void* p[6]; } dst = {{c->bufs["hull.hv"].p, c->bufs["hull.normals"].p, c->bufs["hull.edges"].p, c->bufs["hull.nv"].p, c->bufs["hull.nf"].p, c->bufs["hull.ne"].p}};
  const size_t nB = (size_t)S.B;
  const bool can_upload = c->obb_done_ev != nullptr && dst.p[0] && c->bufs["hull.hv"].bytes >= nB * c->hcap.v * 24 && c->bufs["hull.normals"].bytes >= nB * c->hcap.f * 24 &&
                          c->bufs["hull.edges"].bytes >= nB * c->hcap.e * 16 && c->bufs["hull.nv"].bytes >= nB * 4 && c->bufs["hull.nf"].bytes >= nB * 4 && c->bufs["hull.ne"].bytes >= nB * 4;
  const int B = S.B;
  p.th = std::thread([c, hp, dst, can_upload, hulls, stl, B, phase0]() {
    sh_ctx::Prepared& q = c->prep;
    sh_ctx::StageSide& S = c->stg;
    auto meta = [&](int rc, const char* msg) {
      { std::lock_guard<std::mutex> lk(S.m); S.meta_rc = rc; if (msg) S.meta_err = msg; S.meta_ready = true; }
      S.cv.notify_all();
    };
    if (hipSetDevice(c->device) != hipSuccess) { q.rc = SH_ERR_HIP; meta(SH_ERR_HIP, "hipSetDevice"); return; }
    const bool dbg = c->sw.debug;
    const auto tt0 = std::chrono::steady_clock::now();
    auto since = [&]() { return std::chrono::duration<double, std::milli>(std::chrono::steady_clock::now() - tt0).count(); };
    double t_p0 = 0, t_meta = 0, t_pts = 0;
    {
      std::string et;
      const int rc0 = phase0(&et);
      if (rc0 != SH_OK) { q.rc = rc0; meta(rc0, et.c_str()); return; }
      if (!stl.on) meta(SH_OK, nullptr);
      t_p0 = since();
    }
    long long sumV = S.sumV;
    if (stl.on) {
      if (hipEventSynchronize(stl.counted) != hipSuccess) { q.rc = SH_ERR_HIP; meta(SH_ERR_HIP, "sh_stage_stl: the parse kernels failed"); return; }
      const int* counts = S.h_flag + 16;
      const int* nonfin = S.h_flag + 16 + 2 * B;
      S.voff.assign(B + 1, 0); S.foff.assign(B + 1, 0);
      long long maxV = 0, maxF = 0;
      for (int b = 0; b < B; ++b) {
        if (nonfin[b]) { q.rc = SH_ERR_ARG; meta(SH_ERR_ARG, "sh_stage_stl: a file holds NaN / infinite coordinates"); return; }
        if (counts[2 * b] < 4 || counts[2 * b + 1] < 4) { q.rc = SH_ERR_ARG; meta(SH_ERR_ARG, "sh_stage_stl: a mesh has fewer than 4 vertices/faces after merging"); return; }
        S.voff[b + 1] = S.voff[b] + counts[2 * b];
        S.foff[b + 1] = S.foff[b] + counts[2 * b + 1];
        maxV = std::max<long long>(maxV, counts[2 * b]); maxF = std::max<long long>(maxF, counts[2 * b + 1]);
      }
      S.maxV = maxV; S.maxF = maxF; S.sumV = S.voff[B]; S.sumF = S.foff[B];
      sumV = S.sumV;
      hipStream_t st = c->copy_stream;
      bool ok = hipMemcpyAsync(stl.voff_d, S.voff.data(), (size_t)(B + 1) * 8, hipMemcpyHostToDevice, st) == hipSuccess &&
                hipMemcpyAsync(stl.foff_d, S.foff.data(), (size_t)(B + 1) * 8, hipMemcpyHostToDevice, st) == hipSuccess;
      if (ok) {
        const dim3 gc((unsigned)std::min<long long>((stl.maxc + 255) / 256, 1024), (unsigned)B);
        hipLaunchKernelGGL(k_stl_emit, gc, dim3(256), 0, st, (const float*)stl.corners, (const long long*)stl.coff, (const int2*)stl.table, stl.tsize, (const int*)stl.slot,
                           (const int*)stl.vid, (const int*)stl.fpos, (const long long*)stl.voff_d, (const long long*)stl.foff_d, (float*)stl.verts_d, (int*)stl.faces_d);
        ok = hipGetLastError() == hipSuccess && hipEventRecord(S.ready_ev, st) == hipSuccess;
      }
      if (!ok) { q.rc = SH_ERR_HIP; meta(SH_ERR_HIP, "sh_stage_stl: enqueueing the merge failed"); return; }
// ... 791 lines not shown
```

Baseline: 9108.

## Fuse groove row peak analysis into the polar resample kernel

Moves the per-row groove peak detection into a shared device function and calls it at the end of the polar resample kernels for the groove rows, so those rows are processed while still in LDS. The separate k_groove_rows launch and the global re-read of the resampled rows are skipped, and the canal stage is moved earlier so its axis is available. The groove shared-memory layout is unioned to reduce LDS, and the small resample kernel gains a launch-bounds occupancy hint. The cost is extra LDS, registers and a tail of divergent work in the resample kernel, which may lower its occupancy.

```diff
diff --git a/shoulder_amd/csrc/k_groove.h b/shoulder_amd/csrc/k_groove.h
--- a/shoulder_amd/csrc/k_groove.h
+++ b/shoulder_amd/csrc/k_groove.h
@@ -1,200 +1,17 @@
 #pragma once
 #include "k_stages.h"
+#include "k_groove_row.h"
 
 namespace sh {
 
-#define SH_GSLOTS (SH_GROOVE_NROWS * SH_MAXPEAK)
-
-__global__ void k_groove_rows(const double* __restrict__ itr_cs , const double* __restrict__ prox_zs,
-                              const double* __restrict__ canal_axis_ct, int row0,
-                              double* __restrict__ xraw, double* __restrict__ ptheta, int* __restrict__ npk,
-                              double* __restrict__ r0, int* __restrict__ err, int B) {
-  __shared__ double s_bufA[SH_MPROX], s_bufB[SH_MPROX];
-  double* const s_r = s_bufA; double* const s_filt = s_bufA;
-  double* const s_neg = s_bufB; double* const s_roll = s_bufB;
-  __shared__ int s_cand[SH_PEAK_CAP];
-  __shared__ Peak s_pk[SH_PEAK_CAP];
-  __shared__ int s_pass[SH_PEAK_CAP];
-  __shared__ int s_ncand;
+__global__ void k_groove_rows(const double* __restrict__ itr_cs , const GrooveRowOut G) {
+  __shared__ GrooveRowLds S;
   const int M = SH_MPROX;
   const int gid = blockIdx.x, lane = threadIdx.x;
   const int b = gid / SH_GROOVE_NROWS, i = gid % SH_GROOVE_NROWS;
-  const double* row = itr_cs + ((size_t)b * SH_NPROX + row0 + i) * 2 * M;
-  const double* zs = prox_zs + (size_t)b * SH_NPROX + row0;
-  for (int k = lane; k < M; k += 64) s_r[k] = row[M + k];
-  if (lane == 0) s_ncand = 0;
-  __syncthreads();
-  double acc = 0.0;
-  if (lane < 32) {
-    const int leaf = lane >> 3, k = lane & 7;
-    acc = s_r[128 * leaf + k];
-    for (int q = 1; q < 16; ++q) acc += s_r[128 * leaf + 8 * q + k];
-  }
-  acc = acc + __shfl_down(acc, 1);
-  acc = acc + __shfl_down(acc, 2);
-  acc = acc + __shfl_down(acc, 4);
-  acc = acc + __shfl_down(acc, 8);
-  acc = acc + __shfl_down(acc, 16);
-  const double mean = __shfl(acc, 0) / (double)M;
-  for (int k = lane; k < M; k += 64) s_neg[k] = -1.0 * (s_r[k] - mean);
-  __syncthreads();
-  for (int k = 5 + lane; k < M - 5; k += 64) s_filt[k] = savgol10_1_at(s_neg, k);
-  if (lane == 0) savgol10_1_edges(s_neg, M, s_filt);
-  __syncthreads();
-  double bv = 1e300;
-  int bi = 0x7fffffff;
-  for (int k = lane; k < M; k += 64) if (s_filt[k] < bv) { bv = s_filt[k]; bi = k; }
-  for (int off = 32; off > 0; off >>= 1) {
-    double ov = __shfl_down(bv, off);
-    int oi = __shfl_down(bi, off);
-    if (ov < bv || (ov == bv && oi < bi)) { bv = ov; bi = oi; }
-  }
-  const int amin = __shfl(bi, 0);
-  double* r0row = r0 + (size_t)gid * M;
-  for (int k = lane; k < M; k += 64) r0row[k] = -s_neg[k];
-  __syncthreads();
-  for (int k = lane; k < M; k += 64) { int src = k + amin; if (src >= M) src -= M; s_roll[k] = s_filt[src]; }
-  __syncthreads();
-  for (int k = 1 + lane; k < M - 1; k += 64)
-    if (s_roll[k - 1] < s_roll[k]) {
-      int resume;
-      int pk = local_maximum_at(s_roll, M, k, &resume);
-      if (pk >= 0) { int s = atomicAdd(&s_ncand, 1); if (s < SH_PEAK_CAP) s_cand[s] = pk; }
-    }
-  __syncthreads();
-  int nc = s_ncand < SH_PEAK_CAP ? s_ncand : SH_PEAK_CAP;
-  if (lane == 0)
-    for (int a = 1; a < nc; ++a) { int v = s_cand[a]; int q = a - 1; while (q >= 0 && s_cand[q] > v) { s_cand[q + 1] = s_cand[q]; --q; } s_cand[q + 1] = v; }
-  __syncthreads();
-  static_assert(SH_MPROX == 512, "8 samples per lane");
-  __shared__ int s_lb[SH_PEAK_CAP], s_rb[SH_PEAK_CAP];
-  __shared__ double s_lmin[SH_PEAK_CAP], s_rmin[SH_PEAK_CAP];
-  {
-    double xr[8];
-#pragma unroll
-    for (int q = 0; q < 8; ++q) xr[q] = s_roll[8 * lane + q];
-    for (int cnd = 0; cnd < nc; ++cnd) {
-      const int pk = s_cand[cnd];
-      const double v = s_roll[pk];
-      int L = -1, R = M;
-#pragma unroll
-      for (int q = 0; q < 8; ++q) { const int k = 8 * lane + q; if (k < pk && xr[q] > v) L = k; }
-#pragma unroll
-      for (int q = 7; q >= 0; --q) { const int k = 8 * lane + q; if (k > pk && xr[q] > v) R = k; }
-      for (int off = 32; off > 0; off >>= 1) { L = max(L, __shfl_xor(L, off)); R = min(R, __shfl_xor(R, off)); }
-      double lm = v, rm = v;
-#pragma unroll
-      for (int q = 0; q < 8; ++q) {
-        const int k = 8 * lane + q;
-        if (k > L && k <= pk) lm = fmin(lm, xr[q]);
-        if (k >= pk && k < R) rm = fmin(rm, xr[q]);
-      }
-      for (int off = 32; off > 0; off >>= 1) { lm = fmin(lm, __shfl_xor(lm, off)); rm = fmin(rm, __shfl_xor(rm, off)); }
-      int lb = -1, rb = M;
-#pragma unroll
-      for (int q = 0; q < 8; ++q) { const int k = 8 * lane + q; if (k > L && k <= pk && xr[q] == lm) lb = k; }
-#pragma unroll
-      for (int q = 7; q >= 0; --q) { const int k = 8 * lane + q; if (k >= pk && k < R && xr[q] == rm) rb = k; }
-      for (int off = 32; off > 0; off >>= 1) { lb = max(lb, __shfl_xor(lb, off)); rb = min(rb, __shfl_xor(rb, off)); }
-      if (lane == 0) { s_lb[cnd] = lb; s_rb[cnd] = rb; s_lmin[cnd] = lm; s_rmin[cnd] = rm; }
-    }
-  }
-  __syncthreads();
-  if (lane < nc) {
-    const double* x = s_roll;
-    const int pk = s_cand[lane], lb = s_lb[lane], rb = s_rb[lane];
-    const double left_min = s_lmin[lane], right_min = s_rmin[lane];
-    bool ok = x[pk] >= -10.0;
-    const double prom = x[pk] - (left_min > right_min ? left_min : right_min);
-    ok = ok && prom >= 0.6;
-    if (ok) {
-      const double h = x[pk] - prom * 0.5;
-      int k = pk;
-      while (lb < k && h < x[k]) --k;
-      double lip = (double)k;
-      if (x[k] < h) lip += (h - x[k]) / (x[k + 1] - x[k]);
-      k = pk;
-      while (k < rb && h < x[k]) ++k;
-      double rip = (double)k;
-      if (x[k] < h) rip -= (h - x[k]) / (x[k - 1] - x[k]);
-      const double w = rip - lip;
-      ok = w >= 0.1;
-      if (ok) { s_pk[lane].idx = pk; s_pk[lane].prominence = prom; s_pk[lane].width = w; s_pk[lane].width_height = h; }
-    }
-    s_pass[lane] = ok ? 1 : 0;
-  }
-  __syncthreads();
-  __shared__ int s_np;
-  __shared__ double s_th[SH_MAXPEAK], s_d[SH_MAXPEAK][SH_MAXPEAK];
-  __shared__ int s_pidx[SH_MAXPEAK];
-  if (lane == 0) {
-    int np_ = 0;
-    for (int a = 0; a < nc; ++a) if (s_pass[a]) s_pk[np_++] = s_pk[a];
-    if (np_ > SH_MAXPEAK) {
-      bool keep[SH_PEAK_CAP];
-      for (int k = 0; k < np_; ++k) keep[k] = false;
-      for (int q = 0; q < SH_MAXPEAK; ++q) {
-        int bq = -1;
-        for (int k = 0; k < np_; ++k)
-          if (!keep[k] && (bq < 0 || s_pk[k].prominence > s_pk[bq].prominence)) bq = k;
-        keep[bq] = true;
-      }
-      int w = 0;
-      for (int k = 0; k < np_; ++k) if (keep[k]) s_pk[w++] = s_pk[k];
-      np_ = SH_MAXPEAK;
-    }
-    s_np = np_;
-  }
-  __syncthreads();
-  const int np_ = s_np;
-  if (lane < np_) {
-    const int idx = (s_pk[lane].idx + amin) % M;
-    s_pidx[lane] = idx;
-    s_th[lane] = row[idx];
-  }
-  double zmax = -1e300, zmin = 1e300;
-  for (int k = lane; k < SH_GROOVE_NROWS; k += 64) { zmax = fmax(zmax, zs[k]); zmin = fmin(zmin, zs[k]); }
-  for (int off = 32; off > 0; off >>= 1) { zmax = fmax(zmax, __shfl_xor(zmax, off)); zmin = fmin(zmin, __shfl_xor(zmin, off)); }
-  __syncthreads();
-  {
-    const int k = lane >> 3, j = lane & 7;
-    if (k < np_ && j < np_) s_d[k][j] = wrapped_abs_diff(s_th[k], s_th[j]);
-  }
-  __syncthreads();
-  if (lane < np_) {
-    const int k = lane;
-    double near = 0.0, next = 0.0;
-    if (np_ > 1) {
-      double a[SH_MAXPEAK];
-      int na = 0;
-      for (int j = 0; j < np_; ++j) {
-        double d = s_d[k][j];
-        if (rint(d * 100.0) / 100.0 != 0.0) a[na++] = d;
-      }
-      for (int p = 1; p < na; ++p) { double v = a[p]; int q = p - 1; while (q >= 0 && a[q] > v) { a[q + 1] = a[q]; --q; } a[q + 1] = v; }
-      near = na > 0 ? a[0] : nan("");
-      if (np_ > 2) next = na > 1 ? a[1] : nan("");
-    }
-    double rng = zmax - zmin;
-    if (rng == 0.0) rng = 1.0;
-    const double sc = 1.0 / rng;
-    const double z_scaled = zs[i] * sc + (0.0 - zmin * sc);
-    const double* ax = canal_axis_ct + 6 * b;
-    double cu[3] = {ax[0] - ax[3], ax[1] - ax[4], ax[2] - ax[5]};
-    const double n = norm3(cu);
-    cu[0] /= n; cu[1] /= n; cu[2] /= n;
-    const double z = zs[i], th = s_th[k];
-    const double rad = row[M + s_pidx[k]];
-    const double px = rad * cos(th), py = rad * sin(th);
-    const double dx = px - cu[0] * z, dy = py - cu[1] * z;
-    double* X = xraw + ((size_t)b * SH_GSLOTS + (size_t)i * SH_MAXPEAK + k) * 9;
-    X[0] = rad; X[1] = near; X[2] = next; X[3] = z_scaled; X[4] = s_pk[k].prominence; X[5] = s_pk[k].width;
-    X[6] = s_pk[k].width_height; X[7] = sqrt(dx * dx + dy * dy); X[8] = (double)np_ / 7.0;
-    ptheta[(size_t)b * SH_GSLOTS + (size_t)i * SH_MAXPEAK + k] = th;
-    for (int q = 0; q < 9; ++q) if (X[q] != X[q]) atomicCAS(&err[b], 0, SH_ERR_GEOMETRY_DEV);
-  }
-  if (lane == 0) npk[gid] = np_;
-  (void)B;
+  const double* row = itr_cs + ((size_t)b * SH_NPROX + G.row0 + i) * 2 * M;
+  for (int k = lane; k < M; k += 64) S.bufA[k] = row[M + k];
+  groove_row(S, row, b, i, G);
 }
 
 __global__ void __launch_bounds__(256)
diff --git a/shoulder_amd/csrc/k_groove_row.h b/shoulder_amd/csrc/k_groove_row.h
--- /dev/null
+++ b/shoulder_amd/csrc/k_groove_row.h
@@ -0,0 +1,217 @@
+#pragma once
+#include "sh_scalar.h"
+
+namespace sh {
+
+#define SH_GSLOTS (SH_GROOVE_NROWS * SH_MAXPEAK)
+
+struct GrooveRowLds {
+  union {
+    double bufA[SH_MPROX];
+    struct {
+      Peak pk[SH_PEAK_CAP];
+      double lmin[SH_PEAK_CAP], rmin[SH_PEAK_CAP];
+      int cand[SH_PEAK_CAP], pass[SH_PEAK_CAP], lb[SH_PEAK_CAP], rb[SH_PEAK_CAP];
+    };
+  };
+  double bufB[SH_MPROX];
+  double th[SH_MAXPEAK], d[SH_MAXPEAK][SH_MAXPEAK];
+  int pidx[SH_MAXPEAK];
+  int ncand, np;
+};
+static_assert(sizeof(Peak) * SH_PEAK_CAP + 2 * 8 * SH_PEAK_CAP + 4 * 4 * SH_PEAK_CAP <= 8 * SH_MPROX, "the peaks fit into the first row buffer");
+
+struct GrooveRowOut {
+  int row0;
+  const double* prox_zs; const double* canal_axis_ct;
+  double* xraw; double* ptheta; int* npk; double* r0; int* err;
+};
+
+__device__ inline void groove_row(GrooveRowLds& S, const double* row, int b, int i, const GrooveRowOut& G) {
+  const int M = SH_MPROX;
+  const int lane = threadIdx.x;
+  const bool act = lane < 64;
+  const size_t gid = (size_t)b * SH_GROOVE_NROWS + i;
+  const double* zs = G.prox_zs + (size_t)b * SH_NPROX + G.row0;
+  double* const s_r = S.bufA; double* const s_filt = S.bufA;
+  double* const s_neg = S.bufB; double* const s_roll = S.bufB;
+  __syncthreads();
+  int amin = 0;
+  if (act) {
+    double acc = 0.0;
+    if (lane < 32) {
+      const int leaf = lane >> 3, k = lane & 7;
+      acc = s_r[128 * leaf + k];
+      for (int q = 1; q < 16; ++q) acc += s_r[128 * leaf + 8 * q + k];
+    }
+    acc = acc + __shfl_down(acc, 1);
+    acc = acc + __shfl_down(acc, 2);
+    acc = acc + __shfl_down(acc, 4);
+    acc = acc + __shfl_down(acc, 8);
+    acc = acc + __shfl_down(acc, 16);
+    const double mean = __shfl(acc, 0) / (double)M;
+    for (int k = lane; k < M; k += 64) s_neg[k] = -1.0 * (s_r[k] - mean);
+  }
+  __syncthreads();
+  if (act) {
+    for (int k = 5 + lane; k < M - 5; k += 64) s_filt[k] = savgol10_1_at(s_neg, k);
+    if (lane == 0) savgol10_1_edges(s_neg, M, s_filt);
+  }
+  __syncthreads();
+  if (act) {
+    double bv = 1e300;
+    int bi = 0x7fffffff;
+    for (int k = lane; k < M; k += 64) if (s_filt[k] < bv) { bv = s_filt[k]; bi = k; }
+    for (int off = 32; off > 0; off >>= 1) {
+      double ov = __shfl_down(bv, off);
+      int oi = __shfl_down(bi, off);
+      if (ov < bv || (ov == bv && oi < bi)) { bv = ov; bi = oi; }
+    }
+    amin = __shfl(bi, 0);
+    double* r0row = G.r0 + gid * M;
+    for (int k = lane; k < M; k += 64) r0row[k] = -s_neg[k];
+  }
+  __syncthreads();
+  if (act) for (int k = lane; k < M; k += 64) { int src = k + amin; if (src >= M) src -= M; s_roll[k] = s_filt[src]; }
+  if (lane == 0) S.ncand = 0;
+  __syncthreads();
+  if (act)
+    for (int k = 1 + lane; k < M - 1; k += 64)
+      if (s_roll[k - 1] < s_roll[k]) {
+        int resume;
+        int pk = local_maximum_at(s_roll, M, k, &resume);
+        if (pk >= 0) { int s = atomicAdd(&S.ncand, 1); if (s < SH_PEAK_CAP) S.cand[s] = pk; }
+      }
+  __syncthreads();
+  const int nc = S.ncand < SH_PEAK_CAP ? S.ncand : SH_PEAK_CAP;
+  if (lane == 0)
+    for (int a = 1; a < nc; ++a) { int v = S.cand[a]; int q = a - 1; while (q >= 0 && S.cand[q] > v) { S.cand[q + 1] = S.cand[q]; --q; } S.cand[q + 1] = v; }
+  __syncthreads();
+  static_assert(SH_MPROX == 512, "8 samples per lane");
+  if (act) {
+    double xr[8];
+#pragma unroll
+    for (int q = 0; q < 8; ++q) xr[q] = s_roll[8 * lane + q];
+    for (int cnd = 0; cnd < nc; ++cnd) {
+      const int pk = S.cand[cnd];
+      const double v = s_roll[pk];
+      int L = -1, R = M;
+#pragma unroll
+      for (int q = 0; q < 8; ++q) { const int k = 8 * lane + q; if (k < pk && xr[q] > v) L = k; }
+#pragma unroll
+      for (int q = 7; q >= 0; --q) { const int k = 8 * lane + q; if (k > pk && xr[q] > v) R = k; }
+      for (int off = 32; off > 0; off >>= 1) { L = max(L, __shfl_xor(L, off)); R = min(R, __shfl_xor(R, off)); }
+      double lm = v, rm = v;
+#pragma unroll
+      for (int q = 0; q < 8; ++q) {
+        const int k = 8 * lane + q;
+        if (k > L && k <= pk) lm = fmin(lm, xr[q]);
+        if (k >= pk && k < R) rm = fmin(rm, xr[q]);
+      }
+      for (int off = 32; off > 0; off >>= 1) { lm = fmin(lm, __shfl_xor(lm, off)); rm = fmin(rm, __shfl_xor(rm, off)); }
+      int lb = -1, rb = M;
+#pragma unroll
+      for (int q = 0; q < 8; ++q) { const int k = 8 * lane + q; if (k > L && k <= pk && xr[q] == lm) lb = k; }
+#pragma unroll
+      for (int q = 7; q >= 0; --q) { const int k = 8 * lane + q; if (k >= pk && k < R && xr[q] == rm) rb = k; }
+      for (int off = 32; off > 0; off >>= 1) { lb = max(lb, __shfl_xor(lb, off)); rb = min(rb, __shfl_xor(rb, off)); }
+      if (lane == 0) { S.lb[cnd] = lb; S.rb[cnd] = rb; S.lmin[cnd] = lm; S.rmin[cnd] = rm; }
+    }
+  }
+  __syncthreads();
+  if (lane < nc) {
+    const double* x = s_roll;
+    const int pk = S.cand[lane], lb = S.lb[lane], rb = S.rb[lane];
+    const double left_min = S.lmin[lane], right_min = S.rmin[lane];
+    bool ok = x[pk] >= -10.0;
+    const double prom = x[pk] - (left_min > right_min ? left_min : right_min);
+    ok = ok && prom >= 0.6;
+    if (ok) {
+      const double h = x[pk] - prom * 0.5;
+      int k = pk;
+      while (lb < k && h < x[k]) --k;
+      double lip = (double)k;
+      if (x[k] < h) lip += (h - x[k]) / (x[k + 1] - x[k]);
+      k = pk;
+      while (k < rb && h < x[k]) ++k;
+      double rip = (double)k;
+      if (x[k] < h) rip -= (h - x[k]) / (x[k - 1] - x[k]);
+      const double w = rip - lip;
+      ok = w >= 0.1;
+      if (ok) { S.pk[lane].idx = pk; S.pk[lane].prominence = prom; S.pk[lane].width = w; S.pk[lane].width_height = h; }
+    }
+    S.pass[lane] = ok ? 1 : 0;
+  }
+  __syncthreads();
+  if (lane == 0) {
+    int np_ = 0;
+    for (int a = 0; a < nc; ++a) if (S.pass[a]) S.pk[np_++] = S.pk[a];
+    if (np_ > SH_MAXPEAK) {
+      bool keep[SH_PEAK_CAP];
+      for (int k = 0; k < np_; ++k) keep[k] = false;
+      for (int q = 0; q < SH_MAXPEAK; ++q) {
+        int bq = -1;
+        for (int k = 0; k < np_; ++k)
+          if (!keep[k] && (bq < 0 || S.pk[k].prominence > S.pk[bq].prominence)) bq = k;
+        keep[bq] = true;
+      }
+      int w = 0;
+      for (int k = 0; k < np_; ++k) if (keep[k]) S.pk[w++] = S.pk[k];
+      np_ = SH_MAXPEAK;
+    }
+    S.np = np_;
+  }
+  __syncthreads();
+  const int np_ = S.np;
+  if (lane < np_) {
+    const int idx = (S.pk[lane].idx + amin) % M;
+    S.pidx[lane] = idx;
+    S.th[lane] = row[idx];
+  }
+  double zmax = -1e300, zmin = 1e300;
+  if (act) {
+    for (int k = lane; k < SH_GROOVE_NROWS; k += 64) { zmax = fmax(zmax, zs[k]); zmin = fmin(zmin, zs[k]); }
+    for (int off = 32; off > 0; off >>= 1) { zmax = fmax(zmax, __shfl_xor(zmax, off)); zmin = fmin(zmin, __shfl_xor(zmin, off)); }
+  }
+  __syncthreads();
+  if (act) {
+    const int k = lane >> 3, j = lane & 7;
+    if (k < np_ && j < np_) S.d[k][j] = wrapped_abs_diff(S.th[k], S.th[j]);
+  }
+  __syncthreads();
+  if (lane < np_) {
+    const int k = lane;
+    double near = 0.0, next = 0.0;
+    if (np_ > 1) {
+      double a[SH_MAXPEAK];
+      int na = 0;
+      for (int j = 0; j < np_; ++j) {
+        double d = S.d[k][j];
+        if (rint(d * 100.0) / 100.0 != 0.0) a[na++] = d;
+      }
+      for (int p = 1; p < na; ++p) { double v = a[p]; int q = p - 1; while (q >= 0 && a[q] > v) { a[q + 1] = a[q]; --q; } a[q + 1] = v; }
+      near = na > 0 ? a[0] : nan("");
+      if (np_ > 2) next = na > 1 ? a[1] : nan("");
+    }
+    double rng = zmax - zmin;
+    if (rng == 0.0) rng = 1.0;
+    const double sc = 1.0 / rng;
+    const double z_scaled = zs[i] * sc + (0.0 - zmin * sc);
+    const double* ax = G.canal_axis_ct + 6 * b;
+    double cu[3] = {ax[0] - ax[3], ax[1] - ax[4], ax[2] - ax[5]};
+    const double n = norm3(cu);
+    cu[0] /= n; cu[1] /= n; cu[2] /= n;
+    const double z = zs[i], th = S.th[k];
+    const double rad = row[M + S.pidx[k]];
+    const double px = rad * cos(th), py = rad * sin(th);
+    const double dx = px - cu[0] * z, dy = py - cu[1] * z;
+    double* X = G.xraw + ((size_t)b * SH_GSLOTS + (size_t)i * SH_MAXPEAK + k) * 9;
+    X[0] = rad; X[1] = near; X[2] = next; X[3] = z_scaled; X[4] = S.pk[k].prominence; X[5] = S.pk[k].width;
+    X[6] = S.pk[k].width_height; X[7] = sqrt(dx * dx + dy * dy); X[8] = (double)np_ / 7.0;
+    G.ptheta[(size_t)b * SH_GSLOTS + (size_t)i * SH_MAXPEAK + k] = th;
+    for (int q = 0; q < 9; ++q) if (X[q] != X[q]) atomicCAS(&G.err[b], 0, SH_ERR_GEOMETRY_DEV);
+  }
+  if (lane == 0) G.npk[gid] = np_;
+}
+
+}
diff --git a/shoulder_amd/csrc/k_ovf.h b/shoulder_amd/csrc/k_ovf.h
--- a/shoulder_amd/csrc/k_ovf.h
+++ b/shoulder_amd/csrc/k_ovf.h
@@ -324,8 +324,9 @@
 
 __global__ void __launch_bounds__(SH_RS_THREADS)
 k_resample_polar_huge(int N, int M, const int* __restrict__ ring_n, OvfPools P, OvfSet S, const double* __restrict__ centroids,
-                      double* __restrict__ ixy, double* __restrict__ itr_start, double* __restrict__ itr_cs, const RsWant W) {
+                      double* __restrict__ ixy, double* __restrict__ itr_start, double* __restrict__ itr_cs, const RsWant W, const GrooveRowOut G) {
   constexpr int NS = SH_MPROX / SH_RS_THREADS;
+  __shared__ GrooveRowLds gl;
   __shared__ int amin_idx;
   __shared__ double wmin[SH_RS_THREADS / 64];
   __shared__ int widx[SH_RS_THREADS / 64];
@@ -335,6 +336,7 @@
     const int kpl = pl % N;
     const bool want_st = W.keep_all || kpl >= W.st_lo, want_cs = W.keep_all || (kpl >= W.cs_lo && kpl < W.cs_hi);
     if (!want_st && !want_cs) continue;
+    const bool groove = G.row0 >= 0 && kpl >= G.row0 && kpl < G.row0 + SH_GROOVE_NROWS;
     const int L = ring_n[pl];
     const double* rp = P.ring + 2 * S.roff[pl];
     double* d = (double*)(P.work + S.woff[pl]);
@@ -411,10 +413,12 @@
         int dst = tid + u * SH_RS_THREADS - k0; if (dst < 0) dst += M;
         o[dst] = th[u];
         o[M + dst] = rr[u];
+        if (pass && groove) gl.bufA[dst] = rr[u];
       }
       __syncthreads();
     }
-  }
-}
-
-}
+    if (groove) { groove_row(gl, itr_cs + (size_t)pl * 2 * M, pl / N, kpl - G.row0, G); __syncthreads(); }
+  }
+}
+
+}
diff --git a/shoulder_amd/csrc/k_slices.h b/shoulder_amd/csrc/k_slices.h
--- a/shoulder_amd/csrc/k_slices.h
+++ b/shoulder_amd/csrc/k_slices.h
@@ -1,5 +1,6 @@
 #pragma once
 #include "sh_scalar.h"
+#include "k_groove_row.h"
 
 namespace sh {
 
@@ -576,10 +577,12 @@
 template <int CAP>
 __device__ inline void resample_polar_plane(const int pl, int N, int M, const int* __restrict__ ring_n, const double* __restrict__ ring,
                  const double* __restrict__ centroids, double* __restrict__ ixy,
-                 double* __restrict__ itr_start, double* __restrict__ itr_cs, const long long* __restrict__ ovf_roff, const RsWant W) {
+                 double* __restrict__ itr_start, double* __restrict__ itr_cs, const long long* __restrict__ ovf_roff, const RsWant W,
+                 const GrooveRowOut& G) {
   static_assert(SH_MPROX % SH_RS_THREADS == 0, "whole samples per lane");
   constexpr int NS = SH_MPROX / SH_RS_THREADS;
-  __shared__ double rx[CAP + 1], ry[CAP + 1], d[CAP + 1];
+  __shared__ union { struct { double rx[CAP + 1], ry[CAP + 1], d[CAP + 1]; } rs; GrooveRowLds g; } lds;
+  double* const rx = lds.rs.rx; double* const ry = lds.rs.ry; double* const d = lds.rs.d;
   __shared__ int amin_idx;
   __shared__ double wmin[SH_RS_THREADS / 64];
   __shared__ int widx[SH_RS_THREADS / 64];
@@ -590,6 +593,7 @@
   const int kpl = pl % N;
   const bool want_st = W.keep_all || kpl >= W.st_lo, want_cs = W.keep_all || (kpl >= W.cs_lo && kpl < W.cs_hi);
   if (!want_st && !want_cs) return;
+  const bool groove = G.row0 >= 0 && kpl >= G.row0 && kpl < G.row0 + SH_GROOVE_NROWS;
   const double* rp = ring + (size_t)pl * (SH_MAXSEG + 1) * 2;
   for (int q = tid; q <= L; q += SH_RS_THREADS) { rx[q] = rp[2 * q]; ry[q] = rp[2 * q + 1]; }
   __syncthreads();
@@ -676,26 +680,29 @@
       int dst = tid + u * SH_RS_THREADS - k0; if (dst < 0) dst += M;
       o[dst] = th[u];
       o[M + dst] = rr[u];
-    }
-    __syncthreads();
-  }
-}
-
-__global__ void __launch_bounds__(SH_RS_THREADS)
+      if (pass && groove) lds.g.bufA[dst] = rr[u];
+    }
+    __syncthreads();
+  }
+  if (groove) groove_row(lds.g, itr_cs + (size_t)pl * 2 * M, pl / N, kpl - G.row0, G);
+}
+
+__global__ void __launch_bounds__(SH_RS_THREADS, 8)
 k_resample_polar(int N, int M, const int* __restrict__ ring_n, const double* __restrict__ ring, const double* __restrict__ centroids,
-                 double* __restrict__ ixy, double* __restrict__ itr_start, double* __restrict__ itr_cs, const long long* __restrict__ ovf_roff, const RsWant W) {
-  resample_polar_plane<SH_SMALLSEG>(blockIdx.x, N, M, ring_n, ring, centroids, ixy, itr_start, itr_cs, ovf_roff, W);
+                 double* __restrict__ ixy, double* __restrict__ itr_start, double* __restrict__ itr_cs, const long long* __restrict__ ovf_roff, const RsWant W,
+                 const GrooveRowOut G) {
+  resample_polar_plane<SH_SMALLSEG>(blockIdx.x, N, M, ring_n, ring, centroids, ixy, itr_start, itr_cs, ovf_roff, W, G);
 }
 __global__ void __launch_bounds__(SH_RS_THREADS)
 k_resample_polar_large(int nplanes, int N, int M, const int* __restrict__ ring_n, const double* __restrict__ ring, const double* __restrict__ centroids,
                        double* __restrict__ ixy, double* __restrict__ itr_start, double* __restrict__ itr_cs, const int* __restrict__ nlarge,
-                       const long long* __restrict__ ovf_roff, const RsWant W) {
+                       const long long* __restrict__ ovf_roff, const RsWant W, const GrooveRowOut G) {
   if (*nlarge == 0) return;
   for (int pl = blockIdx.x; pl < nplanes; pl += gridDim.x) {
     if (ring_n[pl] <= SH_SMALLSEG || ovf_roff[pl] >= 0) continue;
-    resample_polar_plane<SH_MAXSEG>(pl, N, M, ring_n, ring, centroids, ixy, itr_start, itr_cs, ovf_roff, W);
-    __syncthreads();
-  }
-}
-
-}
+    resample_polar_plane<SH_MAXSEG>(pl, N, M, ring_n, ring, centroids, ixy, itr_start, itr_cs, ovf_roff, W, G);
+    __syncthreads();
+  }
+}
+
+}
diff --git a/shoulder_amd/csrc/shoulder_hip.hip b/shoulder_amd/csrc/shoulder_hip.hip
--- a/shoulder_amd/csrc/shoulder_hip.hip
+++ b/shoulder_amd/csrc/shoulder_hip.hip
@@ -1476,7 +1476,13 @@
   return SH_OK;
 }
 
-struct SliceSpec { const char* pfx; int kind, N; bool ring, resample; int select; bool total_area, decode_bounds; };
+static GrooveRowOut groove_row_out(sh_ctx* c, int row0) {
+  return GrooveRowOut{row0, buf<double>(c, "prox.zs"), buf<double>(c, "canal.axis_ct"), buf<double>(c, "groove.xraw"), buf<double>(c, "groove.ptheta"),
+                      buf<int>(c, "groove.npk"), buf<double>(c, "groove.r0"), buf<int>(c, "err")};
+}
+struct SliceSpec { const char* pfx; int kind, N; bool ring, resample; int select; bool total_area, decode_bounds;
+                   bool groove;
+                 };
 static int run_slice_sets(sh_ctx* c, const SliceSpec* specs, int nspec) {
   const int B = c->Bwin;
   if (nspec < 1 || nspec > 2) return fail(c, SH_ERR_STATE, "run_slice_sets: one or two sets");
@@ -1542,13 +1548,14 @@
       RsWant want{c->keep_products ? 1 : 0, SH_ANP_ROW0, 0, 0};
       cutoff_range(SH_NPROX, c->params.groove_cutoff[0], c->params.groove_cutoff[1], &want.cs_lo, &want.cs_hi);
       if (c->b0 == 0) { c->rs_cs_lo = want.cs_lo; c->rs_cs_hi = want.cs_hi; c->rs_all = c->keep_products; c->rs_gen = c->batch_gen; }
+      const GrooveRowOut G = sp.groove ? groove_row_out(c, want.cs_lo) : GrooveRowOut{-1};
       LAUNCH(c, "k_resample_polar", k_resample_polar, dim3(B * S.N), dim3(SH_RS_THREADS), S.N, SH_MPROX, S.ring_n, S.ring,
-             S.centroids, buf<double>(c, "prox.ixy"), buf<double>(c, "prox.itr_start"), buf<double>(c, "prox.itr_centered_start"), (const long long*)OS[i].roff, want);
+             S.centroids, buf<double>(c, "prox.ixy"), buf<double>(c, "prox.itr_start"), buf<double>(c, "prox.itr_centered_start"), (const long long*)OS[i].roff, want, G);
       LAUNCH(c, "k_resample_polar_large", k_resample_polar_large, dim3(std::min(B * S.N, 512)), dim3(SH_RS_THREADS), B * S.N, S.N, SH_MPROX, S.ring_n, S.ring,
-             S.centroids, buf<double>(c, "prox.ixy"), buf<double>(c, "prox.itr_start"), buf<double>(c, "prox.itr_centered_start"), (const int*)S.nlarge, (const long long*)OS[i].roff, want);
+             S.centroids, buf<double>(c, "prox.ixy"), buf<double>(c, "prox.itr_start"), buf<double>(c, "prox.itr_centered_start"), (const int*)S.nlarge, (const long long*)OS[i].roff, want, G);
       if (ovf_on) {
         LAUNCH(c, "k_resample_polar_huge", k_resample_polar_huge, dim3(64), dim3(SH_RS_THREADS), S.N, SH_MPROX, (const int*)S.ring_n, OP, OS[i],
-               S.centroids, buf<double>(c, "prox.ixy"), buf<double>(c, "prox.itr_start"), buf<double>(c, "prox.itr_centered_start"), want);
+               S.centroids, buf<double>(c, "prox.ixy"), buf<double>(c, "prox.itr_start"), buf<double>(c, "prox.itr_centered_start"), want, G);
       }
     }
   }
@@ -1993,6 +2000,13 @@
     }
     if (rc != SH_OK) return rc;
   }
+  if (mask & SH_STAGE_CANAL) {
+    LAUNCH(c, "k_canal", k_canal, dim3(B), dim3(64), buf<double>(c, "full.centroids"), buf<double>(c, "full.zs"),
+           buf<double>(c, "z_bounds"), buf<double>(c, "obb_transform"), c->params.canal_cutoff[0], c->params.canal_cutoff[1],
+           c->params.bone_kind == SH_BONE_PROXIMAL ? buf<double>(c, "pobb.cutoff") : (const double*)nullptr,
+           buf<double>(c, "canal.points_obb"), buf<double>(c, "canal.axis_obb"), buf<double>(c, "canal.axis_ct"), buf<int>(c, "err"));
+  }
+  const bool groove_in_rs = (mask & SH_STAGE_PROXIMAL) && (mask & SH_STAGE_GROOVE) && c->have_rfc;
   if (mask & SH_STAGE_NECK) {
     const bool prox = c->params.bone_kind == SH_BONE_PROXIMAL;
     if (prox) {
@@ -2003,18 +2017,14 @@
              buf<double>(c, "neck_z"), buf<int>(c, "neck_index"), B, 0.70, 0.99, (double*)nullptr);
     }
     if (merge_env && (mask & SH_STAGE_PROXIMAL)) {
-      const SliceSpec sp[2] = {{"neckc", 3, 1, true, false, 1, false, false}, {"prox", 1, SH_NPROX, true, true, 0, false, false}};
+      const SliceSpec sp[2] = {{"neckc", 3, 1, true, false, 1, false, false, false}, {"prox", 1, SH_NPROX, true, true, 0, false, false, groove_in_rs}};
       if ((rc = run_slice_sets(c, sp, 2)) != SH_OK) return rc;
     } else if ((rc = run_slice_set(c, "neckc", 3, 1, true, false, 1)) != SH_OK) return rc;
   }
-  if (mask & SH_STAGE_CANAL) {
-    LAUNCH(c, "k_canal", k_canal, dim3(B), dim3(64), buf<double>(c, "full.centroids"), buf<double>(c, "full.zs"),
-           buf<double>(c, "z_bounds"), buf<double>(c, "obb_transform"), c->params.canal_cutoff[0], c->params.canal_cutoff[1],
-           c->params.bone_kind == SH_BONE_PROXIMAL ? buf<double>(c, "pobb.cutoff") : (const double*)nullptr,
-           buf<double>(c, "canal.points_obb"), buf<double>(c, "canal.axis_obb"), buf<double>(c, "canal.axis_ct"), buf<int>(c, "err"));
-  }
-  if ((mask & SH_STAGE_PROXIMAL) && !(merge_env && (mask & SH_STAGE_NECK)))
-    if ((rc = run_slice_set(c, "prox", 1, SH_NPROX, true, true)) != SH_OK) return rc;
+  if ((mask & SH_STAGE_PROXIMAL) && !(merge_env && (mask & SH_STAGE_NECK))) {
+    const SliceSpec sp{"prox", 1, SH_NPROX, true, true, 0, false, false, groove_in_rs};
+    if ((rc = run_slice_sets(c, &sp, 1)) != SH_OK) return rc;
+  }
   if (mask & SH_STAGE_GROOVE) {
     if (!c->have_rfc) return fail(c, SH_ERR_STATE, "sh_run: groove stage needs sh_load_rfc first");
     int ga, gb;
@@ -2026,9 +2036,8 @@
     const int* feat = (const int*)pp; const float* thr = (const float*)(pp + N * 4); const int* ti = (const int*)(pp + N * 8);
     const int* fi = (const int*)(pp + N * 12); const float* lw = (const float*)(pp + N * 16); const int* roots = (const int*)(pp + N * 20);
     const int rows = B * SH_GROOVE_NROWS;
-    LAUNCH(c, "k_groove_rows", k_groove_rows, dim3(rows), dim3(64), buf<double>(c, "prox.itr_centered_start"),
-           buf<double>(c, "prox.zs"), buf<double>(c, "canal.axis_ct"), ga, buf<double>(c, "groove.xraw"),
-           buf<double>(c, "groove.ptheta"), buf<int>(c, "groove.npk"), buf<double>(c, "groove.r0"), buf<int>(c, "err"), B);
+    if (!groove_in_rs)
+      LAUNCH(c, "k_groove_rows", k_groove_rows, dim3(rows), dim3(64), buf<double>(c, "prox.itr_centered_start"), groove_row_out(c, ga));
     LAUNCH(c, "k_groove_scale", k_groove_scale, dim3(B), dim3(256), buf<double>(c, "groove.xraw"), buf<int>(c, "groove.npk"),
            buf<double>(c, "groove.stats"), B, buf<int>(c, "groove.slots"), buf<int>(c, "groove.nslot"), buf<float>(c, "groove.proba"));
     if ((rc = ensure(c, "rfc.nodes", N * 16, 4)) != SH_OK) return rc;
```

Result: no change. 9069, median of 2 (-0.4%).
